# GAMES-UChile/mogptk

Measured on AMD Instinct MI355X. Metric: log-marginal-likelihood+grad evals/sec, MOSM C=4 N=8192; 1/2/4/8 GPU, higher is better.
Workload: dtype f64

## Files before the change

mogptk_amd/csrc/exact.hip:

```cpp
#include "mogp_model.h"
#include <cstdlib>
#include <limits>

using namespace mogp;

static int wait_stream(hipStream_t st) {
    static const bool spin = !(std::getenv("MOGP_SPIN_WAIT") && std::atoi(std::getenv("MOGP_SPIN_WAIT")) == 0);
    if (!spin) { HIP_TRY(hipStreamSynchronize(st)); return 0; }
    for (;;) {
        const hipError_t e = hipStreamQuery(st);
        if (e == hipSuccess) return 0;
        if (e != hipErrorNotReady) return hip_fail(e, "hipStreamQuery", __FILE__, __LINE__);
    }
}

static hipEvent_t prof_event(mogp_model* m, int idx) {
    if (!m->profiling) return nullptr;
    while ((int)m->ev.size() <= idx) { hipEvent_t e; if (hipEventCreate(&e) != hipSuccess) return nullptr; m->ev.push_back(e); }
    return m->ev[idx];
}

static void kinv_block_ranges(mogp_model* m) {
    std::vector<int> blk;
    tile_blocks(m->sx.off, m->C, blk);
    const int nblk = (int)blk.size() / 2, D = m->D;
    m->blk_cen.assign((size_t)D * nblk, 0.0); m->blk_half.assign((size_t)D * nblk, 0.0);
    for (int b = 0; b < nblk; ++b)
        for (int d = 0; d < D; ++d) {
            const double* x = m->sx.xs.data() + (size_t)d * m->sx.Mpad + blk[2 * b];
            double lo = x[0], hi = x[0];
            for (int i = 1; i < blk[2 * b + 1]; ++i) { lo = std::fmin(lo, x[i]); hi = std::fmax(hi, x[i]); }
            m->blk_cen[(size_t)d * nblk + b] = 0.5 * (lo + hi); m->blk_half[(size_t)d * nblk + b] = 0.5 * (hi - lo);
        }
}

static int kinv_plan(mogp_model* m, bool want) {
    static const bool full = std::getenv("MOGP_FULL_INVERSE") && std::atoi(std::getenv("MOGP_FULL_INVERSE")) != 0;
    m->kinv_sparse = false; m->kinv_fraction = 1.0;
    if (!want || full || m->sh_n > 1 || m->tiles.empty() || m->radial) return 0;
    const int nb = m->nb, D = m->D, T = m->T, W = m->Wt;
    const int64_t ld = m->Npad;
    if (m->blk_cen.empty()) kinv_block_ranges(m);
    const int nblk = (int)(m->blk_cen.size() / std::max(D, 1));
    std::vector<char> need((size_t)nb * nb, 0);
    for (const GTile& t : m->tiles) {
        const double* tab = m->table.data() + (size_t)t.pair * T * W;
        bool read = false;
        for (int k = 0; k < T && !read; ++k) {
            const double* row = tab + (size_t)k * W;
            double emin = 0.0;
            for (int d = 0; d < D; ++d) {
                const double sd = (m->blk_cen[(size_t)d * nblk + t.rb] - m->blk_cen[(size_t)d * nblk + t.cb]) + row[2 + 2 * D + d];
                const double mu = std::fmax(0.0, std::fabs(sd) - m->blk_half[(size_t)d * nblk + t.rb] - m->blk_half[(size_t)d * nblk + t.cb]);
                emin += row[2 + d] * mu * mu;
            }
            read = !(0.5 * emin > 52.0);
        }
        if (!read) continue;
        const int i0 = t.r0 / MOGP_TILE, i1 = (t.r0 + t.nr - 1) / MOGP_TILE, j0 = t.c0 / MOGP_TILE, j1 = (t.c0 + t.nc - 1) / MOGP_TILE;
        for (int i = i0; i <= i1; ++i) for (int j = j0; j <= j1; ++j) if (j <= i) need[(size_t)i * nb + j] = 1;
    }
    for (int i = 0; i < nb; ++i) need[(size_t)i * nb + i] = 1;
    std::vector<GemmTask> acc, lau;
    std::vector<int> prefix(nb + 1, 0);
    for (int i = 0; i < nb; ++i) {
        for (int j = 0; j <= i; ++j) {
            if (!need[(size_t)i * nb + j]) continue;
            GemmTask a;
            a.a_off = (int64_t)i * MOGP_TILE; a.b_off = (int64_t)j * MOGP_TILE; a.c_off = (int64_t)i * MOGP_TILE * ld + (int64_t)j * MOGP_TILE;
            a.kt = 4 * MOGP_TILE / 16; a.pad = i + 1;
            acc.push_back(a);
            GemmTask l;
            l.a_off = (int64_t)i * MOGP_TILE * ld + (int64_t)i * MOGP_TILE; l.b_off = (int64_t)i * MOGP_TILE * ld + (int64_t)j * MOGP_TILE;
            l.c_off = a.c_off; l.kt = (int)((ld - (int64_t)i * MOGP_TILE) / 16); l.pad = 0;
            lau.push_back(l);
        }
        prefix[i + 1] = (int)acc.size();
    }
    const double frac = (double)acc.size() / ((double)nb * (nb + 1) / 2);
    m->kinv_fraction = frac;
    if (frac > 0.85) return 0;
    const bool same = acc.size() == m->kinv_acc_tasks.size() && (acc.empty() || std::memcmp(acc.data(), m->kinv_acc_tasks.data(), acc.size() * sizeof(GemmTask)) == 0);
    if (!same || m->d_kinv_acc.n < acc.size()) {
        int rc;
        if ((rc = m->d_kinv_acc.ensure(std::max<size_t>(acc.size(), 1)))) return rc;
        if ((rc = m->d_kinv_lauum.ensure(std::max<size_t>(lau.size(), 1)))) return rc;
        HIP_TRY(hipMemcpyAsync(m->d_kinv_acc.p, acc.data(), acc.size() * sizeof(GemmTask), hipMemcpyHostToDevice, m->st));
        HIP_TRY(hipMemcpyAsync(m->d_kinv_lauum.p, lau.data(), lau.size() * sizeof(GemmTask), hipMemcpyHostToDevice, m->st));
        HIP_TRY(hipStreamSynchronize(m->st));
        m->kinv_acc_tasks.swap(acc); m->kinv_lauum_tasks.swap(lau);
    }
    m->kinv_prefix.swap(prefix);
    m->kinv_sparse = true;
    return 0;
}

static int pin_ensure(mogp_model* m, size_t n) {
    if (n <= m->h_pin_n) return 0;
    if (m->h_pin) { hipError_t e = hipHostFree(m->h_pin); (void)e; m->h_pin = nullptr; m->h_pin_n = 0; }
    HIP_TRY(hipHostMalloc(reinterpret_cast<void**>(&m->h_pin), n * sizeof(double), hipHostMallocDefault));
    m->h_pin_n = n;
    return 0;
}
struct PinLayout {
    size_t nzz, logdet = 0, zz, info, moments, diagG, pivots, total;
    PinLayout(int nb, int64_t Npad, int C, int T, int Wt) : nzz((size_t)((Npad + 3) / 4)) {
        zz = (size_t)nb; info = zz + nzz; moments = info + 1; diagG = moments + (size_t)(C * (C + 1) / 2) * T * Wt; pivots = diagG + C; total = pivots + 2;
    }
    explicit PinLayout(const mogp_model* m) : PinLayout(m->nb, m->Npad, m->C, m->T, m->Wt) {}
};

namespace mogp {
int begin_call(mogp_model* m, int64_t* info, bool one_gpu) {
    m->mean_w = nullptr;
    if (int rc = use_device(m->ctx)) return rc;
    if (info) *info = 0;
    if (one_gpu) one_gpu_call(m);
    return 0;
}

int exact_begin(mogp_model* m, const double* noise_var, const double* data_var, double jitter, GramArgs& ga, double& jabs) {
    const int C = m->C;
    const int64_t N = m->N, Npad = m->Npad;
    if (m->T <= 0) return fail(MOGP_EINVAL, "mogp_model_set_terms must be called before an evaluation");
    if (!noise_var) return fail(MOGP_EINVAL, "noise_var is null");
    { int r__ = ensure_system(m); if (r__) return r__; }
    m->have_W = m->have_Kinv = false;
    m->gemm_ev_used = 0; m->gemm_launches = 0; m->gemm_flops = 0.0;

    double dsum = 0.0;
    if (!m->point_diag.empty()) {
        for (int c = 0; c < C; ++c)
            for (int k = m->sx.off[c]; k < m->sx.off[c + 1]; ++k) dsum += m->point_diag[k] + noise_var[c];
    } else if (m->radial && m->point_kinds) {
        dsum = table_diag_points(m, m->sx);
        for (int c = 0; c < C; ++c) dsum += (double)(m->sx.off[c + 1] - m->sx.off[c]) * noise_var[c];
    } else
    for (int c = 0; c < C; ++c) dsum += (double)(m->sx.off[c + 1] - m->sx.off[c]) * (table_diag(m, c) + noise_var[c]);
    if (data_var) {
        std::vector<double> dv(Npad, 0.0);
        for (int64_t pos = 0; pos < N; ++pos) { dv[pos] = data_var[m->sx.perm[pos]]; dsum += dv[pos]; }
        { int r__ = m->d_dvar.ensure(Npad); if (r__) return r__; }
        HIP_TRY(hipMemcpyAsync(m->d_dvar.p, dv.data(), Npad * sizeof(double), hipMemcpyHostToDevice, m->st));
    }
    jabs = jitter * dsum / (double)N;
    HIP_TRY(hipMemcpyAsync(m->d_noise.p, noise_var, C * sizeof(double), hipMemcpyHostToDevice, m->st));
    static const unsigned long long big = std::numeric_limits<unsigned long long>::max();
    HIP_TRY(hipMemcpyAsync(m->d_info.p, &big, sizeof(big), hipMemcpyHostToDevice, m->st));
    int rc;
    if ((rc = mark(m, 0))) return rc;
    ga = GramArgs{};
    ga.tiles = m->d_tiles.p; ga.xr = m->d_x.p; ga.xc = m->d_x.p; ga.ldxr = ga.ldxc = Npad; ga.nrows = ga.ncols = N;
    if ((rc = m->ph_xx.prepare(m->sx.off, m->sx.off, C, m->T, Npad, Npad, m->st, ga.ph))) return rc;
    ga.table = m->d_table.p; ga.T = m->T; ga.D = m->D; ga.C = C; ga.W = m->Wt;
    ga.out = m->k.A.p; ga.ldo = Npad; ga.noise = m->d_noise.p; ga.dvar = data_var ? m->d_dvar.p : nullptr;
    ga.jitter_abs = jabs; ga.mirror = 0;
    if (m->radial) { ga.kind = m->d_kind.p; ga.shape = m->d_shape.p; }
    return 0;
}
}

namespace mogp { int chain_fallback(mogp_model* m) {
    if (m->flow_ran) {
        m->no_flow = true; m->flow_ran = false;
        m->flow_timeouts++;
        m->flow_retry_at = m->n_fact + m->flow_backoff;
        m->flow_backoff = std::min(m->flow_backoff * 4, 16384);
        for (hipStream_t q : {m->st, m->st2, m->st3, m->st4, m->ctx->st5, m->st_priv}) if (q) HIP_TRY(hipStreamSynchronize(q));
        static bool said_flow = false;
        if (!said_flow) {
            said_flow = true;
            unsigned code = 0;
            if (m->k.flow_flags.p && m->k.flow_cur && m->k.flow_cur->base_err > 0) { hipError_t e = hipMemcpy(&code, m->k.flow_flags.p + m->k.flow_cur->base_err, sizeof(code), hipMemcpyDeviceToHost); (void)e; }
            fprintf(stderr, "mogp: the dataflow kernel timed out (wait 0x%x; GPU shared with another process?); using the stream schedule for the next %d evaluations (said once)\n", code, (int)(m->flow_retry_at - m->n_fact));
            fprintf(stderr, "mogp: the host enqueued that evaluation in %.0f us (longest so far %.0f us)\n", m->flow_enqueue_us, m->flow_enqueue_us_max);
        }
        if (std::getenv("MOGP_FLOW_DEBUG")) { fprintf(stderr, "mogp: dataflow time-out %d of this model\n", m->flow_timeouts); flow_debug_dump(m); }
        return 0;
    }
    if (m->no_chain) return fail(MOGP_EHIP, "chain kernel: a hand-off timed out although the model is on the launch-per-step chain");
    m->no_chain = true;
    for (hipStream_t q : {m->st, m->st2, m->st3, m->st4, m->ctx->st5, m->st_priv}) if (q) HIP_TRY(hipStreamSynchronize(q));
    static bool said = false;
    if (!said) { said = true; fprintf(stderr, "mogp: the persistent chain kernel timed out (GPU shared with another process?); using the launch-per-step chain\n"); }
    return 0;
} }

template <typename F> static int retry_on_streams(mogp_model* m, int rc, F again) {
    if (rc != MOGP_RETRY_NO_CHAIN) return rc;
    if ((rc = chain_fallback(m))) return rc;
    return again();
}

namespace mogp { int report_not_pd(unsigned long long hinfo, int64_t* info) {
    if (info) *info = (int64_t)hinfo;
    return fail(MOGP_ENOTPD, "linalg.cholesky: The factorization could not be completed because the input is not "
                             "positive-definite (the leading minor of order " + std::to_string(hinfo) + " is not positive-definite).");
} }

static int factorize_finish(mogp_model* m, const GramArgs& ga, double* lml, int64_t* info) {
    const int64_t N = m->N, Npad = m->Npad;
    const PinLayout pl(m);
    const unsigned long long big = std::numeric_limits<unsigned long long>::max();
    unsigned long long hinfo = 0;
    std::memcpy(&hinfo, m->h_pin + pl.info, sizeof(hinfo));
    int rc;
    if (hinfo == MOGP_INFO_CHAIN_TIMEOUT) return MOGP_RETRY_NO_CHAIN;
    static const bool fake = std::getenv("MOGP_FAKE_K") && std::atoi(std::getenv("MOGP_FAKE_K")) > 1;
    if (hinfo != big && !fake) {
        if (info) *info = (int64_t)hinfo;
        int flag = 0;
        HIP_TRY(hipMemsetAsync(m->d_flag.p, 0, sizeof(int), m->st));
        if ((rc = launch_gram(ga, (int)m->tiles.size(), m->st))) return rc;
        if ((rc = launch_nonfinite_scan(m->k.A.p, Npad, N, m->d_flag.p, m->st))) return rc;
        HIP_TRY(hipMemcpyAsync(&flag, m->d_flag.p, sizeof(int), hipMemcpyDeviceToHost, m->st));
        HIP_TRY(hipStreamSynchronize(m->st));
        if (flag & 1) return fail(MOGP_ENONFINITE, "linalg.cholesky: kernel matrix has NaNs!");
        if (flag & 2) return fail(MOGP_ENONFINITE, "linalg.cholesky: kernel matrix has infinities!");
        return report_not_pd(hinfo, info);
    }
    m->pivot_min = m->h_pin[pl.pivots]; m->pivot_max = m->h_pin[pl.pivots + 1];
    double logdet = 0.0, zz = 0.0;
    for (int i = 0; i < m->nb; ++i) logdet += m->h_pin[pl.logdet + i];
    for (size_t i = 0; i < pl.nzz; ++i) zz += m->h_pin[pl.zz + i];
    if (lml) *lml = -0.5 * (double)N * std::log(2.0 * M_PI) - logdet - 0.5 * zz;
    m->have_W = !m->factor_only && !m->accurate_ran;
    return 0;
}

struct FactorPlan {
    enum Schedule { Fused, Phases, FactorOnly } schedule = Phases;
    bool defer = false;
    bool want_inverse = true;
    bool refine = false;
};

static int factorize(mogp_model* m, const double* noise_var, const double* data_var, double jitter, const FactorPlan& plan,
                     double* lml, double* jitter_abs, int64_t* info, GramArgs* ga_out = nullptr) {
    const bool fuse_inverse = plan.schedule == FactorPlan::Fused, factor_only = plan.schedule == FactorPlan::FactorOnly;
    const int64_t N = m->N, Npad = m->Npad;
    GramArgs ga{};
    double jabs = 0.0;
    int rc = exact_begin(m, noise_var, data_var, jitter, ga, jabs);
    if (rc) return rc;
    if (jitter_abs) *jitter_abs = jabs;
    m->n_fact++;
    if (m->no_flow && m->n_fact >= m->flow_retry_at) m->no_flow = false;
    m->factor_only = factor_only;
    ga.ev0 = prof_event(m, 7); ga.ev1 = prof_event(m, 8);
    m->strip.attach(ga);
    static const bool split_on = !(std::getenv("MOGP_GRAM_SPLIT") && std::atoi(std::getenv("MOGP_GRAM_SPLIT")) == 0);
    const bool split = split_on && fuse_inverse && flow_enabled(m, m->k) && !m->tiles_head.empty() && !m->tiles_tail.empty() && m->st2;
    if (split) {
        GramArgs gh = ga, gt = ga;
        gh.tiles = m->d_tiles_head.p; m->strip_head.attach(gh); gh.ev1 = nullptr;
        gt.tiles = m->d_tiles_tail.p; m->strip_tail.attach(gt); gt.ev0 = nullptr; gt.phases_ready = 1;
        if ((rc = launch_gram(gh, (int)m->tiles_head.size(), m->st))) return rc;
        if ((rc = launch_pad_identity(m->k.A.p, Npad, N, Npad, m->st))) return rc;
        if (!m->gram_ev) HIP_TRY(hipEventCreateWithFlags(&m->gram_ev, hipEventDisableTiming));
        HIP_TRY(hipEventRecord(m->gram_ev, m->st));
        HIP_TRY(hipStreamWaitEvent(m->st2, m->gram_ev, 0));
        if ((rc = launch_gram(gt, (int)m->tiles_tail.size(), m->st2))) return rc;
        if (!m->gram_tail_ev) HIP_TRY(hipEventCreateWithFlags(&m->gram_tail_ev, hipEventDisableTiming));
        HIP_TRY(hipEventRecord(m->gram_tail_ev, m->st2));
        m->k.tail_ready = m->gram_tail_ev;
    } else {
        if ((rc = launch_gram(ga, (int)m->tiles.size(), m->st))) return rc;
        if ((rc = launch_pad_identity(m->k.A.p, Npad, N, Npad, m->st))) return rc;
    }
    ga.ev0 = ga.ev1 = nullptr;
    if ((rc = mark(m, 1))) return rc;

    const PinLayout pl(m);
    if ((rc = pin_ensure(m, pl.total))) return rc;
    if ((rc = m->d_pivots.ensure(2))) return rc;
    if (m->accurate && (rc = m->acc_rhs.ensure((size_t)Npad * MOGP_TILE))) return rc;
    m->k.flow_used = false;
    m->flow_ran = false;
    m->k.want_vec = fuse_inverse;
    m->k.vec_y = m->d_y.p; m->k.vec_z = m->d_z.p; m->k.vec_zz = m->d_zz.p; m->k.vec_part = m->d_alpha.p + Npad;
    const bool accurate = m->accurate && plan.schedule == FactorPlan::Phases;
    m->accurate_ran = accurate;
    m->k.keep_L = m->k.refine_panels = plan.refine || accurate;
    if (factor_only && m->rhs_job && flow_enabled(m, m->k)) rc = spd_potri_flow(m, m->k, m->rhs_job);
    else rc = fuse_inverse ? spd_potri_fused(m, m->k) : spd_potrf(m, m->k);
    m->k.keep_L = m->k.refine_panels = false;
    m->k.want_vec = false; m->k.tail_ready = nullptr;
    if (rc) return rc;
    if ((rc = mark(m, 2))) return rc;
    if (accurate) {
        static const bool acc_aside = !(std::getenv("MOGP_ACC_ASIDE") && std::atoi(std::getenv("MOGP_ACC_ASIDE")) == 0);
        hipStream_t ms = (plan.want_inverse && m->st2u && acc_aside) ? m->st2u : m->st;
        if (plan.want_inverse) {
            if (ms != m->st) {
                while ((int)m->k.inv_ev.size() < 4) { hipEvent_t e; HIP_TRY(hipEventCreateWithFlags(&e, hipEventDisableTiming)); m->k.inv_ev.push_back(e); }
                HIP_TRY(hipEventRecord(m->k.inv_ev[0], m->st));
                HIP_TRY(hipStreamWaitEvent(ms, m->k.inv_ev[0], 0));
            }
            if ((rc = m->k.Wm.ensure((size_t)Npad * Npad))) return rc;
            HIP_TRY(hipMemsetAsync(m->k.Wm.p, 0, (size_t)Npad * Npad * sizeof(double), ms));
            if ((rc = launch_add_diag(m->k.Wm.p, Npad, Npad, 1.0, ms))) return rc;
            if ((rc = trsm_lower(m, m->k.A.p, Npad, m->nb, m->k.Wm.p, Npad, Npad, false, ms, true))) return rc;
            GemmArgs g{};
            g.A = m->k.Wm.p; g.lda = Npad; g.a_kmajor = 1; g.B = m->k.Wm.p; g.ldb = Npad; g.b_kmajor = 1;
            g.C = m->k.B.p; g.ldc = Npad; g.alpha = 1.0; g.beta = 0.0; g.mode = GM_LAUUM; g.mt = g.nt = m->nb; g.K = (int)Npad;
            if ((rc = gemm_call(m, g, gemm_flops(g, nullptr), ms))) return rc;
            if (ms != m->st) HIP_TRY(hipEventRecord(m->k.inv_ev[1], ms));
        }
        HIP_TRY(hipMemsetAsync(m->acc_rhs.p, 0, (size_t)Npad * MOGP_TILE * sizeof(double), m->st));
        if ((rc = launch_copy2d(m->acc_rhs.p, MOGP_TILE, m->d_y.p, 1, Npad, 1, 1.0, m->st))) return rc;
        if ((rc = trsm_lower(m, m->k.A.p, Npad, m->nb, m->acc_rhs.p, MOGP_TILE, MOGP_TILE, false))) return rc;
        if ((rc = launch_copy2d(m->d_z.p, 1, m->acc_rhs.p, MOGP_TILE, Npad, 1, 1.0, m->st))) return rc;
        HIP_TRY(hipMemsetAsync(m->d_zz.p, 0, pl.nzz * sizeof(double), m->st));
        if ((rc = launch_gemv_rows(m->d_z.p, Npad, 1, Npad, m->d_z.p, m->d_zz.p, m->st))) return rc;
        if ((rc = trsm_lower(m, m->k.A.p, Npad, m->nb, m->acc_rhs.p, MOGP_TILE, MOGP_TILE, true))) return rc;
        if ((rc = launch_copy2d(m->d_alpha.p, 1, m->acc_rhs.p, MOGP_TILE, Npad, 1, 1.0, m->st))) return rc;
        if (plan.want_inverse && ms != m->st) HIP_TRY(hipStreamWaitEvent(m->st, m->k.inv_ev[1], 0));
    } else if (plan.schedule == FactorPlan::Phases && (rc = spd_trtri(m, m->k))) return rc;
    if ((rc = mark(m, 3))) return rc;

    if (factor_only) {
        HIP_TRY(hipMemsetAsync(m->d_zz.p, 0, pl.nzz * sizeof(double), m->st));
    } else if (!accurate) {
        const double* Wp = fuse_inverse ? m->k.Wm.p : m->k.A.p;
        m->w_in_Wm = fuse_inverse;
        if (fuse_inverse && m->k.flow_used && m->k.vec_done) {
            if ((rc = launch_flow_alpha_sum(m->k, m->d_alpha.p, m->st))) return rc;
        } else {
            if ((rc = launch_trmv_lower(Wp, Npad, Npad, m->d_y.p, m->d_z.p, m->d_zz.p, m->st))) return rc;
            if ((rc = launch_trmv_lower_t(Wp, Npad, Npad, m->d_z.p, m->d_alpha.p, m->st))) return rc;
        }
    }
    if (fuse_inverse && (rc = spd_potri_fused_finish(m, m->k))) return rc;
    if ((rc = mark(m, 4))) return rc;
    {
        static const bool fault = std::getenv("MOGP_FLOW_FAULT") && std::atoi(std::getenv("MOGP_FLOW_FAULT")) != 0;
        static const unsigned long long timed_out = MOGP_INFO_CHAIN_TIMEOUT;
        if (fault && m->k.flow_used) HIP_TRY(hipMemcpyAsync(m->d_info.p, &timed_out, sizeof(timed_out), hipMemcpyHostToDevice, m->st));
    }

    const int nzz = (int)pl.nzz;
    if ((rc = launch_pivot_range(m->k.invd.p, N, m->d_pivots.p, m->st))) return rc;
    HIP_TRY(hipMemcpyAsync(m->h_pin + pl.pivots, m->d_pivots.p, 2 * sizeof(double), hipMemcpyDeviceToHost, m->st));
    HIP_TRY(hipMemcpyAsync(m->h_pin + pl.logdet, m->k.logdet.p, m->nb * sizeof(double), hipMemcpyDeviceToHost, m->st));
    static const int zz_piece = []() { const char* e = std::getenv("MOGP_D2H_CHUNK"); const int v = e ? std::atoi(e) : 2048; return v > 0 ? v : (1 << 30); }();
    for (int o = 0; o < nzz; o += zz_piece)
        HIP_TRY(hipMemcpyAsync(m->h_pin + pl.zz + o, m->d_zz.p + o, std::min(zz_piece, nzz - o) * sizeof(double), hipMemcpyDeviceToHost, m->st));
    HIP_TRY(hipMemcpyAsync(m->h_pin + pl.info, m->d_info.p, sizeof(unsigned long long), hipMemcpyDeviceToHost, m->st));
    if (ga_out) *ga_out = ga;
    if (plan.defer) return 0;
    HIP_TRY(hipStreamSynchronize(m->st));
    return factorize_finish(m, ga, lml, info);
}

namespace mogp { void collect_timing(mogp_model* m, int last_mark) {
    if (!m->profiling) return;
    auto el = [&](int a, int b) { float t = 0.f; if (hipEventElapsedTime(&t, m->ev[a], m->ev[b]) != hipSuccess) t = 0.f; return (double)t; };
    std::fill(m->ms, m->ms + MOGP_ST_COUNT, 0.0);
    m->ms[MOGP_ST_GRAM] = el(0, 1);
    m->ms[MOGP_ST_POTRF] = el(1, 2);
    m->ms[MOGP_ST_TRTRI] = el(2, 3);
    m->ms[MOGP_ST_SOLVE] = el(3, 4);
    if (last_mark >= 6) { m->ms[MOGP_ST_LAUUM] = el(4, 5); m->ms[MOGP_ST_MOMENTS] = el(5, 6); }
    m->ms[MOGP_ST_TOTAL] = el(0, last_mark);
    if ((int)m->ev.size() > 8) m->ms[MOGP_ST_GRAM_KERNEL] = el(7, 8);
    if (last_mark >= 6 && (int)m->ev.size() > 10) m->ms[MOGP_ST_MOMENT_KERNEL] = el(9, 10);
    double gsum = 0.0;
    for (size_t i = 0; i + 1 < m->gemm_ev_used; i += 2) {
        float t = 0.f;
        if (hipEventElapsedTime(&t, m->gemm_ev[i], m->gemm_ev[i + 1]) == hipSuccess) gsum += t;
    }
    m->ms[MOGP_ST_GEMM_KERNEL] = gsum;
}

int moment_pass_device(mogp_model* m, const double* kinv, double ksign) {
    const int C = m->C, D = m->D, W = m->Wt, T = m->T, P = C * (C + 1) / 2;
    const int64_t Npad = m->Npad;
    const int rm = m->sh_n > 1 ? m->sh_n : 0;
    const bool own = m->sh_n > 1 && m->own_n == m->sh_n && m->own_rank == m->sh_rank;
    int rc;
    MomentArgs ma{};
    ma.tiles = own ? m->d_tiles_own.p : m->d_tiles.p; ma.ntiles = (int)(own ? m->tiles_own.size() : m->tiles.size());
    ma.x = m->d_x.p; ma.ldx = Npad; ma.nrows = ma.ncols = m->N;
    if ((rc = m->ph_xx.prepare(m->sx.off, m->sx.off, C, T, Npad, Npad, m->st, ma.ph))) return rc;
    ma.table = m->d_table.p; ma.T = T; ma.D = D; ma.C = C; ma.W = W; ma.kinv = kinv; ma.kinv_sign = ksign; ma.ld = Npad; ma.alpha = m->d_alpha.p;
    ma.row_mod = rm; ma.row_rem = m->sh_rank;
    if (m->radial) { ma.kind = m->d_kind.p; ma.shape = m->d_shape.p; }
    ma.partial = m->d_partial.p;
    ma.phases_ready = 1;
    ma.ev0 = prof_event(m, 9); ma.ev1 = prof_event(m, 10);
    if ((rc = launch_moments(ma, m->st))) return rc;
    if ((rc = launch_moment_reduce(m->d_partial.p, own ? m->d_pair_start_own.p : m->d_pair_start.p, P, T, W, D, m->d_moments.p, m->st))) return rc;
    if ((rc = launch_diagG(kinv, Npad, m->d_alpha.p, m->d_chan_off.p, C, m->d_diagG.p, m->st, ksign, rm, m->sh_rank))) return rc;
    if ((rc = mean_grad_enqueue(m, m->d_alpha.p, -1.0))) return rc;
    return mark(m, 6);
}

int moment_pass(mogp_model* m, const double* kinv, double ksign, double* moments, double* diagG) {
    const int C = m->C, W = m->Wt, T = m->T, P = C * (C + 1) / 2;
    int rc;
    if ((rc = moment_pass_device(m, kinv, ksign))) return rc;
    HIP_TRY(hipMemcpyAsync(moments, m->d_moments.p, (size_t)P * T * W * sizeof(double), hipMemcpyDeviceToHost, m->st));
    HIP_TRY(hipMemcpyAsync(diagG, m->d_diagG.p, C * sizeof(double), hipMemcpyDeviceToHost, m->st));
    HIP_TRY(hipStreamSynchronize(m->st));
    return 0;
}

int test_side(mogp_model* m, int64_t S, const double* Xs, const double* kss_diag, int64_t extra_rows, hipStream_t st, TestSide& ts, GramArgs& ga) {
    const int C = m->C, D = m->D;
    const int64_t Npad = m->Npad;
    SortedX& ss = ts.ss;
    int rc;
    if ((rc = sort_inputs(Xs, S, D, C, MOGP_TILE, ss))) return rc;
    const int64_t Spad = ts.Spad = ss.Mpad, Srow = Spad + extra_rows;
    std::vector<GTile> pt;
    build_rect_tiles(ss.off, m->sx.off, C, pt);
    ts.ntiles = (int)pt.size();
    if ((rc = m->d_xs.ensure((size_t)D * Spad))) return rc;
    if ((rc = m->d_Ksf.ensure((size_t)Srow * Npad))) return rc;
    if ((rc = m->d_mu.ensure(Spad))) return rc;
    if ((rc = m->d_kdiag.ensure(Spad))) return rc;
    if ((rc = m->d_ptiles.ensure(std::max<size_t>(pt.size(), 1)))) return rc;
    std::vector<double> kd(Spad, 0.0);
    const bool per_point = m->Wt > 2 + 3 * D || (m->radial && m->point_kinds);
    for (int c = 0; c < C; ++c)
        for (int pos = ss.off[c]; pos < ss.off[c + 1]; ++pos) kd[pos] = per_point ? kss_diag[ss.perm[pos]] : kss_diag[c];
    HIP_TRY(hipMemcpyAsync(m->d_xs.p, ss.xs.data(), (size_t)D * Spad * sizeof(double), hipMemcpyHostToDevice, st));
    HIP_TRY(hipMemcpyAsync(m->d_kdiag.p, kd.data(), Spad * sizeof(double), hipMemcpyHostToDevice, st));
    HIP_TRY(hipMemcpyAsync(m->d_ptiles.p, pt.data(), pt.size() * sizeof(GTile), hipMemcpyHostToDevice, st));
    HIP_TRY(hipMemsetAsync(m->d_Ksf.p, 0, (size_t)Srow * Npad * sizeof(double), st));
    ga = GramArgs{};
    ga.tiles = m->d_ptiles.p; ga.xr = m->d_xs.p; ga.ldxr = Spad; ga.xc = m->d_x.p; ga.ldxc = Npad; ga.nrows = S; ga.ncols = m->N;
    if ((rc = m->ph_sx.prepare(ss.off, m->sx.off, C, m->T, Spad, Npad, st, ga.ph))) return rc;
    ga.table = m->d_table.p; ga.T = m->T; ga.D = D; ga.C = C; ga.W = m->Wt; ga.out = m->d_Ksf.p; ga.ldo = Npad;
    ga.noise = nullptr; ga.dvar = nullptr; ga.jitter_abs = 0.0; ga.mirror = 0;
    if (m->radial) { ga.kind = m->d_kind.p; ga.shape = m->d_shape.p; }
    return 0;
}
}

extern "C" {

int mogp_exact_eval(mogp_model* m, const double* noise_var, const double* data_var, double jitter, int flags,
                    double* lml, double* moments, double* diagG, double* trG, double* jitter_abs, int64_t* info) {
    if (!m) return fail(MOGP_EINVAL, "mogp_exact_eval: model is null");
    int rc;
    if ((rc = begin_call(m, info, true))) return rc;
    static const std::string grad_path = []() { const char* e = std::getenv("MOGP_GRAD_PATH"); return std::string(e ? e : ""); }();
    const bool sweep = grad_path == "sweep" && (flags & MOGP_EVAL_GRAD);
    const bool grad = (flags & MOGP_EVAL_GRAD) != 0;
    GramArgs ga{};
    if ((rc = ensure_system(m))) return rc;
    if ((rc = kinv_plan(m, grad && !sweep && !m->accurate))) return rc;
    const int fused_max = flow_enabled(m, m->k) ? 112 : 80;
    const bool fused = !sweep && grad && !m->accurate && (grad_path == "fused" || (grad_path != "phases" && m->nb <= fused_max));
    auto again = [&]() { return mogp_exact_eval(m, noise_var, data_var, jitter, flags, lml, moments, diagG, trG, jitter_abs, info); };
    FactorPlan plan;
    plan.schedule = fused ? FactorPlan::Fused : FactorPlan::Phases; plan.defer = grad; plan.want_inverse = grad;
    if (sweep) {
        m->pivot_min = m->pivot_max = 0.0;
        if ((rc = eval_sweep(m, noise_var, data_var, jitter, lml, jitter_abs, info))) return retry_on_streams(m, rc, again);
    }
    else if ((rc = factorize(m, noise_var, data_var, jitter, plan, lml, jitter_abs, info, &ga))) return retry_on_streams(m, rc, again);
    if (!grad) { collect_timing(m, 4); return MOGP_OK; }
    if (!moments || !diagG || !trG) return fail(MOGP_EINVAL, "mogp_exact_eval: gradient outputs are null");

    const int C = m->C, W = m->Wt, T = m->T, P = C * (C + 1) / 2;

    if (!sweep && !fused && !m->accurate_ran && (rc = spd_lauum(m, m->k))) return rc;
    const double* kinv = sweep ? m->k.A.p : m->k.B.p;
    const double ksign = sweep ? -1.0 : 1.0;
    if ((rc = mark(m, 5))) return rc;
    if (sweep) {
        if ((rc = moment_pass(m, kinv, ksign, moments, diagG))) return rc;
    } else {
        if ((rc = moment_pass_device(m, kinv, ksign))) return rc;
        const PinLayout pl(m);
        HIP_TRY(hipMemcpyAsync(m->h_pin + pl.moments, m->d_moments.p, (size_t)P * T * W * sizeof(double), hipMemcpyDeviceToHost, m->st));
        HIP_TRY(hipMemcpyAsync(m->h_pin + pl.diagG, m->d_diagG.p, C * sizeof(double), hipMemcpyDeviceToHost, m->st));
        if ((rc = wait_stream(m->st))) return rc;
        if ((rc = factorize_finish(m, ga, lml, info))) return retry_on_streams(m, rc, again);
        std::memcpy(moments, m->h_pin + pl.moments, (size_t)P * T * W * sizeof(double));
        std::memcpy(diagG, m->h_pin + pl.diagG, C * sizeof(double));
    }
    double tr = 0.0;
    for (int c = 0; c < C; ++c) tr += diagG[c];
    *trG = tr;
    m->have_Kinv = true;
    m->kinv_in_A = sweep;
    mean_grad_collect(m);
    collect_timing(m, 6);
    return MOGP_OK;
}

static int predict_core(mogp_model* m, const double* noise_var, const double* data_var, double jitter,
                        const double* kss_diag, int64_t S, const double* Xs, int full,
                        double* mu, double* var, int64_t* info, const double* mean_w) {
    int rc;
    if ((rc = begin_call(m, info, true))) return rc;
    const int C = m->C, nb = m->nb;
    const int64_t Npad = m->Npad;
    hipStream_t sv = m->st3 ? m->st3 : m->st;
    for (auto& e : m->pred_ev) if (!e) HIP_TRY(hipEventCreateWithFlags(&e, hipEventDisableTiming));
    HIP_TRY(hipEventRecord(m->pred_ev[0], m->st));
    HIP_TRY(hipStreamWaitEvent(sv, m->pred_ev[0], 0));
    TestSide ts; GramArgs ga{};
    if ((rc = test_side(m, S, Xs, kss_diag, MOGP_TILE, sv, ts, ga))) return rc;
    const SortedX& ss = ts.ss;
    const int64_t Spad = ts.Spad, Srow = Spad + MOGP_TILE;
    if ((rc = m->d_Vt.ensure((size_t)Srow * Npad))) return rc;
    if ((rc = m->d_var.ensure(Spad))) return rc;
    HIP_TRY(hipMemcpyAsync(m->d_Ksf.p + Spad * Npad, m->d_y.p, Npad * sizeof(double), hipMemcpyDeviceToDevice, sv));
    if ((rc = launch_gram(ga, ts.ntiles, sv))) return rc;
    if (mean_w) {
        std::vector<double> hw(Npad, 0.0);
        for (int64_t pos = 0; pos < m->N; ++pos) hw[pos] = mean_w[m->sx.perm[pos]];
        if ((rc = m->d_z.ensure(Npad))) return rc;
        HIP_TRY(dev_upload(m->d_z.p, hw.data(), Npad * sizeof(double)));
        if ((rc = launch_gemv_rows(m->d_Ksf.p, Npad, Spad, Npad, m->d_z.p, m->d_mu.p, sv))) return rc;
    }

    if ((rc = ensure_system(m))) return rc;
    const char* fpe = std::getenv("MOGP_FLOW_PREDICT");
    int fp_lo = 48, fp_hi = 160;
    if (fpe && std::strchr(fpe, ':')) { fp_lo = std::atoi(fpe); fp_hi = std::atoi(std::strchr(fpe, ':') + 1); }
    else if (fpe) fp_hi = std::atoi(fpe);
    const bool acc = m->accurate;
    const bool as_flow = !acc && fp_hi > 0 && nb >= fp_lo && nb <= fp_hi && Srow / MOGP_TILE <= 4096 && flow_enabled(m, m->k) && !m->kinv_sparse;
    FlowRhs job{m->d_Ksf.p, m->d_Vt.p, (int)(Srow / MOGP_TILE), nullptr};
    if (as_flow) {
        HIP_TRY(hipEventRecord(m->pred_ev[1], sv));
        job.ready = m->pred_ev[1];
        m->rhs_job = &job;
    }
    GramArgs gaK{};
    FactorPlan plan;
    plan.schedule = FactorPlan::FactorOnly; plan.defer = true; plan.refine = acc;
    rc = factorize(m, noise_var, data_var, jitter, plan, nullptr, nullptr, info, &gaK);
    m->rhs_job = nullptr;
    if (rc) return rc;
    const bool flowed = as_flow && m->k.flow_used;

    if (!flowed) {
        constexpr int OB = 4, KD = OB * MOGP_TILE;
        const int nouter = (nb + OB - 1) / OB, mt = (int)(Srow / MOGP_TILE);
        Spd& w = m->k;
        const bool streamed = g_outer == OB && (int)w.sync_ev.size() >= 2 * nouter;
        if (!streamed) {
            HIP_TRY(hipEventRecord(m->pred_ev[1], m->st));
            HIP_TRY(hipStreamWaitEvent(sv, m->pred_ev[1], 0));
        }
        if (w.Wd.n < (size_t)nouter * KD * KD) {
            if ((rc = w.Wd.ensure((size_t)nouter * KD * KD))) return rc;
            HIP_TRY(hipMemsetAsync(w.Wd.p, 0, (size_t)nouter * KD * KD * sizeof(double), sv));
        }
        for (int kb = 0; kb < nouter; ++kb) {
            const int k0 = kb * OB, nk = std::min(OB, nb - k0), k1 = k0 + nk, rem = nb - k1;
            const int64_t c0 = (int64_t)k0 * MOGP_TILE;
            if (streamed) HIP_TRY(hipStreamWaitEvent(sv, w.sync_ev[2 * kb], 0));
            double* Wk = w.Wd.p + (int64_t)kb * KD * KD;
            if ((rc = launch_wkk(w.A.p + c0 * (Npad + 1), Npad, w.invd.p + (int64_t)k0 * MOGP_TILE * MOGP_TILE, nk, Wk, KD, sv))) return rc;
            GemmArgs g{};
            g.A = m->d_Ksf.p + c0; g.lda = Npad; g.a_kmajor = 0; g.B = Wk; g.ldb = KD; g.b_kmajor = 0;
// ... 82 lines not shown
```

mogptk_amd/csrc/flow.hip:

```cpp
#include "mogp_model.h"
#include <unistd.h>
#include <chrono>
#include <set>

#include <cstdio>
#include <cstdlib>

namespace mogp {

typedef double d4_t __attribute__((ext_vector_type(4)));
typedef double d2_t __attribute__((ext_vector_type(2)));

#define FL_BK 16
#define FL_ROWK 18
#define FL_WTM 4
#define FL_WTN 2
#define FL_NWJ 4
#define FL_NWI 2
#define FL_NT 512
#define FL_COLK (MOGP_TILE + 16)
#define FL_OPER (MOGP_TILE * FL_ROWK)
#define FL_LDS_DOUBLES (2 * 2 * FL_OPER)
#define FL_LDS_BYTES (FL_LDS_DOUBLES * 8 + 16 + 3 * 64 * 4 + 16)
static_assert(MOGP_TILE * FL_ROWK == 16 * FL_COLK, "one LDS operand slot serves both layouts");
// ... 628 lines not shown
    }
    std::vector<const std::vector<FlowTask>*> order = {&q[Q_LOOK2], &q[Q_SEMI], &q[Q_INVCRIT], &vec};
    for (int d = 2; d < no + 3; ++d) {
        if (d < no && !into[d].empty()) order.push_back(&into[d]);
        if (d - 3 >= 0 && d - 3 < no && !trail[d - 3].empty()) order.push_back(&trail[d - 3]);
    }
    order.push_back(rhs_nt > 0 ? &rrest : &acc);
    for (size_t k = order.size(); k-- > 1;) if (order[k]->empty()) order.erase(order.begin() + (long)k);
    if ((int)order.size() > FLOW_MAXQ) {
        std::vector<FlowTask> rest;
        std::vector<const std::vector<FlowTask>*> tail(order.begin() + (FLOW_MAXQ - 2), order.end() - 1);
        for (auto* v : tail) rest.insert(rest.end(), v->begin(), v->end());
        std::stable_sort(rest.begin(), rest.end(), [](const FlowTask& x, const FlowTask& y) { return x.key < y.key; });
        p.folded = rest;
        order.erase(order.begin() + (FLOW_MAXQ - 2), order.end() - 1);
        order.insert(order.end() - 1, &p.folded);
    }
    p.nq = (int)order.size();
    for (int qi = 0; qi < p.nq; ++qi) {
        p.qbase[qi] = (int)p.tasks.size(); p.qsize[qi] = (int)order[qi]->size();
        p.tasks.insert(p.tasks.end(), order[qi]->begin(), order[qi]->end());
    }
    p.flops = 2.0 * MOGP_TILE * MOGP_TILE * FL_BK * tiles_k;
}

__global__ void k_alpha_sum(const double* __restrict__ part, int64_t npad, int no, int ob, double* __restrict__ out) {
    const int64_t col = (int64_t)blockIdx.x * blockDim.x + threadIdx.x;
    if (col >= npad) return;
    double s = 0.0;
    for (int r = (int)(col / MOGP_TILE) / ob; r < no; ++r) s += part[(int64_t)r * npad + col];
    out[col] = s;
}
int launch_flow_alpha_sum(const Spd& w, double* alpha, hipStream_t st) {
    const FlowPlan& p = w.flow_cur ? *w.flow_cur : w.flow;
    hipLaunchKernelGGL(k_alpha_sum, dim3((unsigned)((w.Npad + 255) / 256)), dim3(256), 0, st, w.vec_part, w.Npad, p.nouter, p.ob, alpha);
    HIP_TRY(hipGetLastError());
    return 0;
}

bool flow_enabled(const mogp_model* m, const Spd& w) {
    const char* eo = std::getenv("MOGP_FLOW");
    const char* en = std::getenv("MOGP_FLOW_MIN");
    const int on = eo ? std::atoi(eo) : 1, nmin = en ? std::atoi(en) : 8;
    if (!on || (m->no_flow && m->n_fact < m->flow_retry_at) || !chain_enabled(m) || !m->ctx->st_priv) return false;
    if (m->kinv_sparse && &w == &m->k) return false;
    return w.nb >= nmin && w.nb <= 0xfff0;
}

int spd_potri_flow(mogp_model* m, Spd& w, const FlowRhs* rhs) {
    const int nb = w.nb, ob = 4;
    const int64_t ld = w.Npad;
    int rc;
    const auto host_t0 = std::chrono::steady_clock::now();
    hipStream_t crit = m->st, priv = m->st_priv, bulk = m->st2;
    if (w.Wm.n < (size_t)ld * ld) {
        if ((rc = w.Wm.ensure((size_t)ld * ld))) return rc;
        HIP_TRY(hipMemsetAsync(w.Wm.p, 0, (size_t)ld * ld * sizeof(double), crit));
    }
    if ((rc = w.Lm.ensure((size_t)ld * ld))) return rc;
    if (!rhs && (rc = w.Wt.ensure((size_t)ld * ld))) return rc;
    const bool replay = m->replay_flow && !rhs && &w == &m->k;
    FlowPlan& plan = rhs ? w.flow_rhs : replay ? w.flow_replay : w.flow;
    DevBuf<FlowTask>& d_tasks = rhs ? w.flow_tasks_rhs : replay ? w.flow_tasks_replay : w.flow_tasks;
    DevBuf<int>& d_qmeta = rhs ? w.flow_qmeta_rhs : replay ? w.flow_qmeta_replay : w.flow_qmeta;
    const int rhs_nt = rhs ? rhs->nt : 0;
    if (plan.nb != nb || plan.ob != ob || plan.rhs_nt != rhs_nt) {
        flow_build(nb, ob, plan, rhs_nt, replay);
        if ((rc = d_tasks.ensure(plan.tasks.size()))) return rc;
        if ((rc = d_qmeta.ensure(2 * FLOW_MAXQ))) return rc;
        int qm[2 * FLOW_MAXQ] = {0};
        for (int q = 0; q < plan.nq; ++q) { qm[2 * q] = plan.qbase[q]; qm[2 * q + 1] = plan.qsize[q]; }
        HIP_TRY(hipStreamSynchronize(crit));
        HIP_TRY(dev_upload(d_tasks.p, plan.tasks.data(), plan.tasks.size() * sizeof(FlowTask)));
        HIP_TRY(dev_upload(d_qmeta.p, qm, sizeof(qm)));
    }
    if ((rc = w.flow_flags.ensure((size_t)plan.nflags))) return rc;
    if (!w.flow_diag.p) {
        if ((rc = w.flow_diag.ensure(FLOW_DIAG_WORDS))) return rc;
        HIP_TRY(hipMemsetAsync(w.flow_diag.p, 0, FLOW_DIAG_WORDS * sizeof(unsigned), crit));
    }
    w.flow_cur = &plan;
    const FlowPlan& p = plan;
    const int nouter = p.nouter;
    if ((rc = w.chain_flags.ensure((size_t)(nouter + 1) * MOGP_CHAIN_FLAGS))) return rc;
    HIP_TRY(hipMemsetAsync(w.chain_flags.p, 0, (size_t)(nouter + 1) * MOGP_CHAIN_FLAGS * sizeof(unsigned), crit));
    HIP_TRY(hipMemsetAsync(w.flow_flags.p, 0, (size_t)p.nflags * sizeof(unsigned), crit));
    if (replay) {
        std::vector<unsigned> preset((size_t)p.nflags, 0u);
        for (const FlowPlan::Chain& c : p.chain) preset[c.done_idx] = c.expect;
        HIP_TRY(hipMemcpyAsync(w.flow_flags.p, preset.data(), preset.size() * sizeof(unsigned), hipMemcpyHostToDevice, crit));
        HIP_TRY(hipStreamSynchronize(crit));
    }
    if (!rhs && w.want_vec && w.vec_zz) HIP_TRY(hipMemsetAsync(w.vec_zz, 0, (size_t)((ld + 3) / 4) * sizeof(double), crit));
    static const bool want_trace = std::getenv("MOGP_FLOW_TRACE") && std::atoi(std::getenv("MOGP_FLOW_TRACE")) != 0;
    if (want_trace) {
        if ((rc = w.flow_trace.ensure(FLOW_TRACE_W * p.tasks.size() + 4 * (size_t)nouter))) return rc;
        HIP_TRY(hipMemsetAsync(w.flow_trace.p, 0, w.flow_trace.n * sizeof(unsigned long long), crit));
    }
    while ((int)w.inv_ev.size() < 4) {
        hipEvent_t e;
        HIP_TRY(hipEventCreateWithFlags(&e, hipEventDisableTiming));
        w.inv_ev.push_back(e);
    }
    hipEvent_t start = w.inv_ev[0], e_flow = w.inv_ev[1], e_chain = w.inv_ev[2];
    HIP_TRY(hipEventRecord(start, crit));
    HIP_TRY(hipStreamWaitEvent(bulk, start, 0));
    HIP_TRY(hipStreamWaitEvent(priv, start, 0));

    static std::atomic<unsigned long long> attr_done{0ull};
    static std::atomic<unsigned long long> attr_done_dbg{0ull};
    { int r__ = set_max_dynamic_lds(reinterpret_cast<const void*>(k_flow<false>), FL_LDS_BYTES, attr_done); if (r__) return r__; }
    { int r__ = set_max_dynamic_lds(reinterpret_cast<const void*>(k_flow<true>), FL_LDS_BYTES, attr_done_dbg); if (r__) return r__; }
    static const int wg_per_cu = std::getenv("MOGP_FLOW_WGS") ? std::max(1, std::atoi(std::getenv("MOGP_FLOW_WGS"))) : 2;
    int cus = (m->ctx->ncu > 0 ? m->ctx->ncu : 256) - m->ctx->ncu_reserved;
    { static const int drop = std::getenv("MOGP_FLOW_DROP_CUS") ? std::atoi(std::getenv("MOGP_FLOW_DROP_CUS")) : 16;
      if (drop > 0 && drop < cus) cus -= drop; }
    FlowArgs g{};
    g.bA = w.A.p; g.bL = w.Lm.p; g.bWt = rhs ? rhs->T : w.Wt.p; g.bWm = w.Wm.p; g.bB = rhs ? rhs->X : w.B.p; g.ld = ld;
    g.tasks = d_tasks.p; g.qmeta = d_qmeta.p; g.flags = w.flow_flags.p;
    g.nq = p.nq; g.ncas = FLOW_NCAS; g.base_heads = p.base_heads; g.base_err = p.base_err; g.info = m->d_info.p;
    g.trace = want_trace ? w.flow_trace.p : nullptr;
    g.diag = w.flow_diag.p;
    static const bool want_post = std::getenv("MOGP_FLOW_DEBUG") && std::atoi(std::getenv("MOGP_FLOW_DEBUG")) != 0;
    if (want_post) {
        const size_t nwg = (size_t)wg_per_cu * ((size_t)cus + (size_t)m->ctx->ncu_reserved);
        if ((rc = w.flow_post.ensure(nwg * FLOW_POST_W))) return rc;
        HIP_TRY(hipMemsetAsync(w.flow_post.p, 0, w.flow_post.n * sizeof(unsigned), bulk));
        g.post = w.flow_post.p;
        if ((rc = w.flow_done.ensure(p.tasks.size()))) return rc;
        HIP_TRY(hipMemsetAsync(w.flow_done.p, 0, p.tasks.size(), bulk));
        g.done = w.flow_done.p;
    }
    g.npad = ld;
    { const char* e = std::getenv("MOGP_FLOW_REFILL"); g.refill = e ? std::atoi(e) : 0; }
    { const char* e = std::getenv("MOGP_FLOW_CLAIM1"); g.claim_one = e ? std::atoi(e) : 0; }
    { const char* e = std::getenv("MOGP_FLOW_NHI"); g.nhi = e ? std::atoi(e) : 0; }
    { const char* e = std::getenv("MOGP_FLOW_NAP"); g.nap_max = e ? (unsigned)std::max(0, std::atoi(e)) : 4u; }
    { const char* e = std::getenv("MOGP_FLOW_NAP_CALM"); g.nap_calm = e ? (unsigned)std::max(0, std::atoi(e)) : 0u; if (g.nap_calm < g.nap_max) g.nap_calm = g.nap_max; }
    w.vec_done = false;
    if (!rhs && w.want_vec && w.vec_y && w.vec_z && w.vec_zz && w.vec_part) {
        g.vy = w.vec_y; g.vz = w.vec_z; g.vzz = w.vec_zz; g.vpart = w.vec_part;
        w.vec_done = true;
    }
    hipEvent_t pe0 = nullptr, pe1 = nullptr;
    if (m->profiling) {
        if (m->gemm_ev_used + 2 > m->gemm_ev.size())
            for (int i = 0; i < 64; ++i) { hipEvent_t e; HIP_TRY(hipEventCreate(&e)); m->gemm_ev.push_back(e); }
        pe0 = m->gemm_ev[m->gemm_ev_used++]; pe1 = m->gemm_ev[m->gemm_ev_used++];
        HIP_TRY(hipEventRecord(pe0, bulk));
    }
    if (rhs && rhs->ready) HIP_TRY(hipStreamWaitEvent(bulk, rhs->ready, 0));
    const bool dbg_kernel = g.post != nullptr || g.trace != nullptr;
    static_assert(sizeof(FlowArgs) <= 512, "Spd::flow_args slots");
    if ((rc = w.flow_args.ensure(1024))) return rc;
    if (w.flow_args_h.size() != 2048) w.flow_args_h.assign(2048, (char)0xff);
    auto upload = [&](size_t slot, const FlowArgs& a, hipStream_t st) -> int {
        char* held = w.flow_args_h.data() + slot;
        char* fresh_ = w.flow_args_h.data() + 1024 + slot;
        std::memset(fresh_, 0, 512);
        std::memcpy(fresh_, &a, sizeof(a));
        if (std::memcmp(held, fresh_, 512) == 0) return 0;
        HIP_TRY(hipStreamSynchronize(st));
        HIP_TRY(dev_upload(w.flow_args.p + slot, fresh_, 512));
        std::memcpy(held, fresh_, 512);
        return 0;
    };
    if ((rc = upload(0, g, bulk))) return rc;
    const FlowArgs* d_g = reinterpret_cast<const FlowArgs*>(w.flow_args.p);
    FlowHot hot{};
    hot.bA = g.bA; hot.bL = g.bL; hot.bWt = g.bWt; hot.bWm = g.bWm; hot.bB = g.bB; hot.ld = g.ld; hot.tasks = g.tasks; hot.qmeta = g.qmeta; hot.flags = g.flags;
    hot.nq = g.nq; hot.ncas = g.ncas; hot.base_heads = g.base_heads; hot.base_err = g.base_err; hot.nap_max = g.nap_max; hot.nap_calm = g.nap_calm;
    if (dbg_kernel) hipLaunchKernelGGL(k_flow<true>, dim3(wg_per_cu * cus), dim3(FL_NT), FL_LDS_BYTES, bulk, d_g, hot);
    else hipLaunchKernelGGL(k_flow<false>, dim3(wg_per_cu * cus), dim3(FL_NT), FL_LDS_BYTES, bulk, d_g, hot);
    HIP_TRY(hipGetLastError());
    if (pe1) HIP_TRY(hipEventRecord(pe1, bulk));
    HIP_TRY(hipEventRecord(e_flow, bulk));
    m->gemm_launches += 1;
    m->gemm_flops += p.flops;

    unsigned* ferr = w.flow_flags.p + p.base_err;
    for (int kb = 0; kb < nouter && !replay; ++kb) {
        const int k0 = kb * ob, k1 = std::min(k0 + ob, nb), nk = k1 - k0, na = std::min(ob, nb - k1);
        const FlowPlan::Chain& pc = p.chain[kb];
        ChainFlow cf{};
        cf.done_flag = w.flow_flags.p + pc.done_idx; cf.write_through = 1;
        cf.trace = want_trace ? w.flow_trace.p + FLOW_TRACE_W * p.tasks.size() + 4 * (size_t)kb : nullptr;
        cf.diag = w.flow_diag.p;
        if ((rc = launch_chain(w.A.p, ld, k0, nk, w.invd.p, w.logdet.p, m->d_info.p, 0, w.Wm.p + (int64_t)k0 * MOGP_TILE * (ld + 1), ld,
                               w.chain_flags.p + (size_t)kb * MOGP_CHAIN_FLAGS, ferr, priv, &cf))) return rc;
        if (na <= 0) continue;
        GemmArgs t1{};
        t1.A = w.A.p + (int64_t)k1 * MOGP_TILE * ld + (int64_t)k0 * MOGP_TILE; t1.lda = ld; t1.a_kmajor = 0;
        t1.B = w.Wm.p + (int64_t)k0 * MOGP_TILE * (ld + 1); t1.ldb = ld; t1.b_kmajor = 0;
        t1.C = w.Lm.p + (int64_t)k1 * MOGP_TILE * ld + (int64_t)k0 * MOGP_TILE; t1.ldc = ld; t1.alpha = 1.0; t1.beta = 0.0;
        t1.mode = GM_KHI_J; t1.small = 1; t1.mt = 2 * na; t1.nt = nk; t1.K = nk * MOGP_TILE;
        t1.fl_flags = w.flow_flags.p; t1.fl_nwait = pc.t1_nwait;
        for (int k = 0; k < pc.t1_nwait; ++k) { t1.fl_widx[k] = pc.t1_widx[k]; t1.fl_wval[k] = pc.t1_wval[k]; }
        static const unsigned hook_spins = std::getenv("MOGP_FLOW_HOOK_SPINS") ? (unsigned)std::atoll(std::getenv("MOGP_FLOW_HOOK_SPINS")) : 0u;
        t1.fl_spins = hook_spins; t1.fl_diag = w.flow_diag.p;
        t1.fl_wt = 1; t1.fl_sig = 1; t1.fl_sig_base = pc.t1_sig_base; t1.fl_sig_shift = 1; t1.fl_err = ferr; t1.sk_info = m->d_info.p;
        if ((rc = launch_gemm(t1, priv))) return rc;
        if (kb == 0 && w.tail_ready) HIP_TRY(hipStreamWaitEvent(priv, w.tail_ready, 0));
        GemmArgs t2{};
        t2.A = t1.C; t2.lda = ld; t2.a_kmajor = 0; t2.B = t1.C; t2.ldb = ld; t2.b_kmajor = 0;
        t2.C = w.A.p + (int64_t)k1 * MOGP_TILE * (ld + 1); t2.ldc = ld; t2.alpha = -1.0; t2.beta = 1.0;
        t2.mode = GM_RECT_LOWER; t2.small = 2; t2.mt = 2 * na; t2.nt = 2 * na; t2.K = nk * MOGP_TILE;
        t2.fl_flags = w.flow_flags.p; t2.fl_nwait = pc.t2_wval ? 1 : 0; t2.fl_widx[0] = pc.t2_widx; t2.fl_wval[0] = pc.t2_wval;
        t2.fl_err = ferr; t2.sk_info = m->d_info.p; t2.fl_spins = hook_spins; t2.fl_diag = w.flow_diag.p;
        if ((rc = launch_gemm(t2, priv))) return rc;
        m->gemm_flops += gemm_flops(t1, nullptr) + gemm_flops(t2, nullptr);
    }
    static const bool tail_on = !(std::getenv("MOGP_FLOW_TAIL") && std::atoi(std::getenv("MOGP_FLOW_TAIL")) == 0);
    if (tail_on && m->ctx->ncu_reserved > 0 && !replay) {
        if (rhs && rhs->ready) HIP_TRY(hipStreamWaitEvent(priv, rhs->ready, 0));
        g.post_base = wg_per_cu * cus;
        if ((rc = upload(512, g, priv))) return rc;
        const FlowArgs* d_g2 = reinterpret_cast<const FlowArgs*>(w.flow_args.p + 512);
        if (dbg_kernel) hipLaunchKernelGGL(k_flow<true>, dim3(wg_per_cu * m->ctx->ncu_reserved), dim3(FL_NT), FL_LDS_BYTES, priv, d_g2, hot);
        else hipLaunchKernelGGL(k_flow<false>, dim3(wg_per_cu * m->ctx->ncu_reserved), dim3(FL_NT), FL_LDS_BYTES, priv, d_g2, hot);
        HIP_TRY(hipGetLastError());
    }
    HIP_TRY(hipEventRecord(e_chain, priv));
    HIP_TRY(hipStreamWaitEvent(crit, e_flow, 0));
    HIP_TRY(hipStreamWaitEvent(crit, e_chain, 0));
    w.fused_last_inv = nullptr; w.fused_last_wt = nullptr;
    w.flow_used = true;
    m->flow_ran = true;
    m->flow_enqueue_us = std::chrono::duration<double, std::micro>(std::chrono::steady_clock::now() - host_t0).count();
    m->flow_enqueue_us_max = std::max(m->flow_enqueue_us_max, m->flow_enqueue_us);
    { const char* e = std::getenv("MOGP_FLOW_DEBUG");
      if (e && std::atoi(e) == 2 && &w == &m->k) { usleep(60000); fprintf(stderr, "mogp: dataflow state 60 ms after the evaluation was enqueued\n"); flow_debug_dump(m); } }
    return 0;
}

}

namespace mogp { void flow_debug_dump(mogp_model* m) {
    if (!m->k.flow_flags.p || !m->k.flow_cur) return;
    const FlowPlan& p = *m->k.flow_cur;
    std::vector<unsigned> fl((size_t)p.nflags);
    hipError_t e = hipMemcpy(fl.data(), m->k.flow_flags.p, fl.size() * sizeof(unsigned), hipMemcpyDeviceToHost); (void)e;
    std::vector<unsigned long long> tr;
    if (m->k.flow_trace.p && m->k.flow_trace.n >= FLOW_TRACE_W * p.tasks.size()) {
        tr.resize(FLOW_TRACE_W * p.tasks.size());
        e = hipMemcpy(tr.data(), m->k.flow_trace.p, tr.size() * sizeof(unsigned long long), hipMemcpyDeviceToHost); (void)e;
    }
    fprintf(stderr, "  error word 0x%x\n", fl[p.base_err]);
    std::set<unsigned> holders;
    for (int q = 0; q < p.nq; ++q) {
        const unsigned h = fl[p.base_heads + q];
        const unsigned claimed = std::min<unsigned>(h, (unsigned)p.qsize[q]);
        unsigned done = 0, shown = 0;
        fprintf(stderr, "  queue %2d: head %u of %d", q, h, p.qsize[q]);
        for (unsigned hh = 0; hh < (unsigned)p.qsize[q]; ++hh) {
            const size_t ti = (size_t)p.qbase[q] + hh;
            const FlowTask& t = p.tasks[ti];
            const bool fin = !tr.empty() && tr[FLOW_TRACE_W * ti + 4] != 0;
            if (fin) { ++done; continue; }
            if (tr.empty() && hh + 4 < claimed) continue;
            if (hh > claimed || shown >= 6) continue;
            ++shown;
            fprintf(stderr, "\n      %s task %u key %u C(buf %d %d,%d) A(buf %d %d,%d) B(buf %d %d,%d) kt %d var %d:", hh < claimed ? "CLAIMED" : "head   ", hh, t.key,
                    t.cbuf, t.cr, t.cc, t.abuf, t.ar, t.ac, t.bbuf, t.br, t.bc, t.kt, t.var);
            for (int d = 0; d < t.ndep; ++d) fprintf(stderr, " flag[%u]=%u/%u", t.dep[d], fl[t.dep[d]], (unsigned)t.need[d]);
            if (!tr.empty()) {
                const unsigned long long w5 = tr[FLOW_TRACE_W * ti + 5];
                if (w5 >> 63) { fprintf(stderr, "  (HELD by wg %llu%s)", w5 & 0xffff, tr[FLOW_TRACE_W * ti + 1] ? ": STARTED, not finished" : ""); holders.insert((unsigned)(w5 & 0xffff)); }
                else fprintf(stderr, "  (taken by wg %llu: %s)", w5 & 0xffff, tr[FLOW_TRACE_W * ti + 1] ? "running" : "not started");
            }
        }
        if (!tr.empty()) fprintf(stderr, "\n      finished %u", done);
        fprintf(stderr, "\n");
    }
    if (!tr.empty() && !holders.empty()) {
        unsigned long long t0 = ~0ull, tmax = 0;
        for (size_t i = 0; i < p.tasks.size(); ++i) {
            const unsigned long long s1 = tr[FLOW_TRACE_W * i + 1];
            if (s1) { t0 = std::min(t0, s1); tmax = std::max(tmax, std::max(s1, tr[FLOW_TRACE_W * i + 4])); }
        }
        fprintf(stderr, "  last time stamp of the evaluation: %.1f us after its first task\n", (double)(tmax - t0) / 100.0);
        int shown = 0;
        for (unsigned wg : holders) {
            size_t last = (size_t)-1, held = 0;
            for (size_t i = 0; i < p.tasks.size(); ++i) {
                const unsigned long long w5 = tr[FLOW_TRACE_W * i + 5];
                if ((unsigned)(w5 & 0xffff) != wg) continue;
                if (w5 >> 63) { ++held; if (!tr[FLOW_TRACE_W * i + 1]) continue; }
                if (tr[FLOW_TRACE_W * i + 1] && (last == (size_t)-1 || tr[FLOW_TRACE_W * i + 1] > tr[FLOW_TRACE_W * last + 1])) last = i;
            }
            if (shown++ >= 24) break;
            if (last == (size_t)-1) { fprintf(stderr, "  holder wg %u: holds %zu, has started NO task\n", wg, held); continue; }
            const FlowTask& t = p.tasks[last];
            fprintf(stderr, "  holder wg %u (xcc %llu): holds %zu; its last task %zu var %d kt %d: looked %.1f taken %.1f k loop %.1f .. %.1f signalled %.1f us%s\n", wg,
                    (tr[FLOW_TRACE_W * last + 5] >> 16) & 0xff, held, last, t.var, t.kt,
                    (double)((long long)(tr[FLOW_TRACE_W * last + 0] - t0)) / 100.0, (double)((long long)(tr[FLOW_TRACE_W * last + 1] - t0)) / 100.0,
                    (double)((long long)(tr[FLOW_TRACE_W * last + 2] - t0)) / 100.0, (double)((long long)(tr[FLOW_TRACE_W * last + 3] - t0)) / 100.0,
                    tr[FLOW_TRACE_W * last + 4] ? (double)((long long)(tr[FLOW_TRACE_W * last + 4] - t0)) / 100.0 : -1.0, tr[FLOW_TRACE_W * last + 4] ? "" : "  <- NOT FINISHED");
        }
    }
    if (!tr.empty()) {
        unsigned long long t0 = ~0ull;
        for (size_t i = 0; i < p.tasks.size(); ++i) if (tr[FLOW_TRACE_W * i + 1] && tr[FLOW_TRACE_W * i + 1] < t0) t0 = tr[FLOW_TRACE_W * i + 1];
        std::map<long, std::pair<int, std::set<unsigned>>> win;
        for (size_t i = 0; i < p.tasks.size(); ++i) {
            const unsigned long long en = tr[FLOW_TRACE_W * i + 4];
            if (!en) continue;
            auto& w = win[(long)((en - t0) / 500000ull)];
            ++w.first; w.second.insert((unsigned)(tr[FLOW_TRACE_W * i + 5] & 0xffff));
        }
        for (auto& kv : win) fprintf(stderr, "  %4ld ms: %6d tasks done by %3zu workgroups\n", kv.first * 5, kv.second.first, kv.second.second.size());
    }
    if (m->k.flow_post.p) {
        std::vector<unsigned> po(m->k.flow_post.n);
        e = hipMemcpy(po.data(), m->k.flow_post.p, po.size() * sizeof(unsigned), hipMemcpyDeviceToHost); (void)e;
// ... 140 lines not shown
```

mogptk_amd/csrc/gram.hip:

```cpp
#include "mogp_internal.h"

#include <algorithm>
#include <vector>
#include <cstdlib>

#ifdef MOGP_GRAM_DEBUG
#define GRAM_DBG(a, bit) ((a).dbg & (bit))
#else
#define GRAM_DBG(a, bit) 0
#endif

namespace mogp {

typedef double d2_t __attribute__((ext_vector_type(2)));

__device__ __forceinline__ double frac_turn(double p) { return p - rint(p); }

#define GT_SKIP (-1)
#define GT_GENERAL 0
#define GT_SKIP_EXPONENT 50.0
#define GT_DEGREE(zmax) ((zmax) <= 1.19e-3 ? 4 : (zmax) <= 4.93e-3 ? 5 : (zmax) <= 0.0139 ? 6 : (zmax) <= 0.0308 ? 7 : (zmax) <= 0.0578 ? 8 : (zmax) <= 0.0968 ? 9 : \
                         (zmax) <= 0.149 ? 10 : (zmax) <= 0.2147 ? 11 : (zmax) <= 0.294 ? 12 : 14)
#define GT_DEGREE_CASES(X) X(4) X(5) X(6) X(7) X(8) X(9) X(10) X(11) X(12) X(14)

__device__ __forceinline__ double fast_exp(double x) {
    const double n = rint(x * 1.44269504088896338700e+00);
    double r = fma(-n, 6.93147180369123816490e-01, x);
    r = fma(-n, 1.90821492927058770002e-10, r);
    double p = 1.6059043836821613e-10;
    p = fma(p, r, 2.08767569878681e-09);
    p = fma(p, r, 2.505210838544172e-08);
    p = fma(p, r, 2.755731922398589e-07);
    p = fma(p, r, 2.7557319223985893e-06);
    p = fma(p, r, 2.48015873015873e-05);
    p = fma(p, r, 1.984126984126984e-04);
    p = fma(p, r, 1.388888888888889e-03);
    p = fma(p, r, 8.333333333333333e-03);
    p = fma(p, r, 4.1666666666666664e-02);
    p = fma(p, r, 1.6666666666666666e-01);
    p = fma(p, r, 0.5);
    p = fma(p, r, 1.0);
    p = fma(p, r, 1.0);
    return ldexp(p, (int)n);
}

template <int N>
__device__ __forceinline__ double exp_taylor(double z) {
    constexpr double c[15] = {1.0, 1.0, 0.5, 1.6666666666666666e-01, 4.1666666666666664e-02, 8.333333333333333e-03,
                              1.388888888888889e-03, 1.984126984126984e-04, 2.48015873015873e-05, 2.7557319223985893e-06,
                              2.755731922398589e-07, 2.505210838544172e-08, 2.08767569878681e-09, 1.6059043836821613e-10,
                              1.1470745597729725e-11};
    double p = c[N];
#pragma unroll
    for (int k = N - 1; k >= 0; --k) p = fma(p, z, c[k]);
    return p;
}

struct PhaseArgs {
    const double* x; int64_t ld; const int* off; const double* table; int T, D, C, W, role; double* cs; double* sn;
};
__global__ __launch_bounds__(256) void k_phase_table(PhaseArgs a) {
    const int64_t pt = (int64_t)blockIdx.x * 256 + threadIdx.x;
    if (pt >= a.off[a.C]) return;
    const int o = blockIdx.y, t = blockIdx.z, D = a.D, W = a.W;
    int c = 0;
    while (pt >= a.off[c + 1]) ++c;
    const int pair = a.role == 0 ? c * a.C + o : o * a.C + c;
    const double* row = a.table + ((size_t)pair * a.T + t) * W;
    double ph = a.role == 0 ? row[1] : 0.0;
    for (int d = 0; d < D; ++d) {
        const double m = row[2 + D + d], xv = a.x[(size_t)d * a.ld + pt];
        ph = a.role == 0 ? fma(m, xv + row[2 + 2 * D + d], ph) : fma(m, xv, ph);
    }
    double sn, cs;
    sincospi(2.0 * frac_turn(ph), &sn, &cs);
    const size_t idx = ((size_t)o * a.T + t) * a.ld + pt;
    a.cs[idx] = cs;
    a.sn[idx] = sn;
}

struct CentreArgs { const double* x; int64_t ld; const int* off; int C, D; double* cen; double* half; };
__global__ __launch_bounds__(64) void k_block_centres(CentreArgs a) {
    int b = blockIdx.x, c = 0;
    for (; c < a.C; ++c) {
        const int nb = (a.off[c + 1] - a.off[c] + MOGP_GT - 1) / MOGP_GT;
        if (b < nb) break;
        b -= nb;
    }
    if (c >= a.C) return;
    const int start = a.off[c] + b * MOGP_GT, n = min(MOGP_GT, a.off[c + 1] - start), lane = threadIdx.x;
    for (int d = 0; d < a.D; ++d) {
        const double v = a.x[(size_t)d * a.ld + start + (lane < n ? lane : 0)];
        double lo = v, hi = v;
#pragma unroll
        for (int off = 32; off > 0; off >>= 1) { lo = fmin(lo, __shfl_xor(lo, off, 64)); hi = fmax(hi, __shfl_xor(hi, off, 64)); }
        if (lane == 0) { a.cen[(size_t)d * a.ld + start] = 0.5 * (lo + hi); a.half[(size_t)d * a.ld + start] = 0.5 * (hi - lo); }
    }
}

size_t phase_ws_doubles(int C, int T, int64_t ldr, int64_t ldc) { return (size_t)2 * (C * T + MOGP_MAXD) * (size_t)(ldr + ldc); }

struct PhaseView {
    const double *rcs, *rsn, *ccs, *csn, *rcen, *rhalf, *ccen, *chalf;
};
__host__ __device__ static inline PhaseView phase_view(double* ws, int C, int T, int D, int64_t ldr, int64_t ldc) {
    PhaseView v;
    double* p = ws;
    v.rcs = p; p += (size_t)C * T * ldr; v.rsn = p; p += (size_t)C * T * ldr;
    v.ccs = p; p += (size_t)C * T * ldc; v.csn = p; p += (size_t)C * T * ldc;
    v.rcen = p; p += (size_t)D * ldr; v.rhalf = p; p += (size_t)D * ldr;
    v.ccen = p; p += (size_t)D * ldc; v.chalf = p;
    return v;
}

static int launch_phase_tables(const PhaseRef& ph, const double* xr, int64_t ldxr, int64_t nr, const double* xc, int64_t ldxc, int64_t nc,
                               const double* table, int T, int D, int C, int W, hipStream_t s) {
    if (!ph.ws || !ph.offr || !ph.offc) { set_error("Gram / moment launch without a phase workspace"); return -1; }
    const PhaseView v = phase_view(ph.ws, C, T, D, ldxr, ldxc);
    PhaseArgs a;
    a.table = table; a.T = T; a.D = D; a.C = C; a.W = W;
    a.x = xr; a.ld = ldxr; a.off = ph.offr; a.role = 0; a.cs = const_cast<double*>(v.rcs); a.sn = const_cast<double*>(v.rsn);
    if (nr > 0) hipLaunchKernelGGL(k_phase_table, dim3((unsigned)((nr + 255) / 256), C, T), dim3(256), 0, s, a);
    a.x = xc; a.ld = ldxc; a.off = ph.offc; a.role = 1; a.cs = const_cast<double*>(v.ccs); a.sn = const_cast<double*>(v.csn);
    if (nc > 0) hipLaunchKernelGGL(k_phase_table, dim3((unsigned)((nc + 255) / 256), C, T), dim3(256), 0, s, a);
    CentreArgs c;
    c.C = C; c.D = D;
    c.x = xr; c.ld = ldxr; c.off = ph.offr; c.cen = const_cast<double*>(v.rcen); c.half = const_cast<double*>(v.rhalf);
    if (nr > 0) hipLaunchKernelGGL(k_block_centres, dim3((unsigned)((nr + MOGP_GT - 1) / MOGP_GT + C)), dim3(64), 0, s, c);
    c.x = xc; c.ld = ldxc; c.off = ph.offc; c.cen = const_cast<double*>(v.ccen); c.half = const_cast<double*>(v.chalf);
    if (nc > 0) hipLaunchKernelGGL(k_block_centres, dim3((unsigned)((nc + MOGP_GT - 1) / MOGP_GT + C)), dim3(64), 0, s, c);
    HIP_TRY(hipGetLastError());
    return 0;
}

template <int DM>
struct TileLds {
    double cu[MOGP_TC][MOGP_GT], su[MOGP_TC][MOGP_GT], cw[MOGP_TC][MOGP_GT], sw[MOGP_TC][MOGP_GT];
    double V[MOGP_TC][DM], s[MOGP_TC][DM], M[MOGP_TC][DM], A[MOGP_TC];
    double Kp[MOGP_TC][DM];
    double L[MOGP_TC][DM], e[MOGP_TC][DM];
    int deg[MOGP_TC];
};
template <int DM>
struct TileCtx { double cr[DM], cc[DM], hr[DM], hc[DM]; };

template <int DM>
__device__ __forceinline__ void tile_centres(TileCtx<DM>& X, const GTile& tl, int D, const PhaseView& v, int64_t ldxr, int64_t ldxc) {
    for (int d = 0; d < D; ++d) {
        X.cr[d] = v.rcen[(size_t)d * ldxr + tl.r0]; X.hr[d] = v.rhalf[(size_t)d * ldxr + tl.r0];
        X.cc[d] = v.ccen[(size_t)d * ldxc + tl.c0]; X.hc[d] = v.chalf[(size_t)d * ldxc + tl.c0];
    }
}

template <int DM>
__device__ __forceinline__ void tile_context(TileCtx<DM>& X, double (&p)[4][DM], double (&q)[4][DM], const GTile& tl, int D,
                                             const PhaseView& v, const double* __restrict__ xr, int64_t ldxr,
                                             const double* __restrict__ xc, int64_t ldxc, int rg, int cg) {
    tile_centres<DM>(X, tl, D, v, ldxr, ldxc);
#pragma unroll
    for (int m = 0; m < 4; ++m)
        for (int d = 0; d < D; ++d) {
            p[m][d] = xr[(size_t)d * ldxr + tl.r0 + min(rg * 4 + m, tl.nr - 1)] - X.cr[d];
            q[m][d] = xc[(size_t)d * ldxc + tl.c0 + min(cg * 4 + m, tl.nc - 1)] - X.cc[d];
        }
}

constexpr int STAGE_ITEMS = MOGP_TC * MOGP_GT * 2 / 256;
template <int DM>
struct StageItem { double x[DM], cs, sn; };

template <int DM>
__device__ __forceinline__ void stage_item_load(StageItem<DM>& I, int which, int t, int pnt, const GTile& tl, int D, int C, int T, int t0,
                                                const PhaseView& v, const double* __restrict__ xr, int64_t ldxr,
                                                const double* __restrict__ xc, int64_t ldxc) {
    const int i = tl.pair / C, j = tl.pair - i * C;
    if (which == 0) {
        const int64_t g = tl.r0 + min(pnt, tl.nr - 1);
        const size_t k = ((size_t)j * T + t0 + t) * ldxr + g;
        I.cs = v.rcs[k]; I.sn = v.rsn[k];
        for (int d = 0; d < D; ++d) I.x[d] = xr[(size_t)d * ldxr + g];
    } else {
        const int64_t g = tl.c0 + min(pnt, tl.nc - 1);
        const size_t k = ((size_t)i * T + t0 + t) * ldxc + g;
        I.cs = v.ccs[k]; I.sn = v.csn[k];
        for (int d = 0; d < D; ++d) I.x[d] = xc[(size_t)d * ldxc + g];
    }
}

template <int DM, bool AMP, bool RAD = false>
__device__ __forceinline__ void stage_item_compute(TileLds<DM>& L, const StageItem<DM>& I, const TileCtx<DM>& X, const double* tab, int W,
                                                   int which, int t, int pnt, int D, int t0, const int* kinds = nullptr) {
    const double* row = tab + (size_t)(t0 + t) * W;
    const double A = row[0];
    if constexpr (RAD) {
        const int kd = kinds[t0 + t] & MOGP_KIND_MASK;
        const bool per = kd == MOGP_KIND_PERIODIC, dot = kd == MOGP_KIND_DOT;
        const int deg = (AMP && A == 0.0 && !dot) ? GT_SKIP : GT_GENERAL;
        if (pnt == 0 && which == 0) {
            L.deg[t] = deg; L.A[t] = A;
            for (int d = 0; d < D; ++d) {
                L.V[t][d] = row[2 + d]; L.M[t][d] = row[2 + D + d];
                L.s[t][d] = (X.cr[d] - X.cc[d]) + row[2 + 2 * D + d];
                L.Kp[t][d] = X.cr[d]; L.L[t][d] = X.cc[d];
            }
            L.e[t][0] = row[1];
        }
        if (deg == GT_SKIP) return;
        if (dot) return;
        const double f = (AMP && !per) ? A : 1.0;
        if (which == 0) { L.cu[t][pnt] = f * I.cs; L.su[t][pnt] = f * I.sn; }
        else { L.cw[t][pnt] = I.cs; L.sw[t][pnt] = I.sn; }
        return;
    }
    const bool env = W > 2 + 3 * D;
    double zmax = 0.0, es = 0.0, emin = 0.0, efac = 0.0, s[DM], V[DM], Lv[DM], er[DM], ec[DM];
// ... 1381 lines not shown
            c += fabs(s) >= fabs(x) ? (s - t) + x : (x - t) + s;
            s = t;
        }
        __syncthreads();
        red[part][pnt] = s; redc[part][pnt] = c;
        __syncthreads();
        if (part == 0 && pnt < n) {
            double hs = 0.0, hc = 0.0;
#pragma unroll
            for (int q = 0; q < 4; ++q) {
                const double x = red[q][pnt];
                const double t = hs + x;
                hc += fabs(hs) >= fabs(x) ? (hs - t) + x : (x - t) + hs;
                hs = t;
                hc += redc[q][pnt];
            }
            out[(size_t)d * ld + first + pnt] += hs + hc;
        }
    }
}

template <bool DENSE, bool ZG, bool ENV>
static int launch_moments_t(const MomentArgs& a, hipStream_t s) {
    switch (a.D) {
        case 1: hipLaunchKernelGGL((k_moments<1, DENSE, ZG, ENV>), dim3(a.ntiles), dim3(256), 0, s, a); break;
        case 2: hipLaunchKernelGGL((k_moments<2, DENSE, ZG, ENV>), dim3(a.ntiles), dim3(256), 0, s, a); break;
        case 3: hipLaunchKernelGGL((k_moments<3, DENSE, ZG, ENV>), dim3(a.ntiles), dim3(256), 0, s, a); break;
        default: hipLaunchKernelGGL((k_moments<0, DENSE, ZG, ENV>), dim3(a.ntiles), dim3(256), 0, s, a); break;
    }
    HIP_TRY(hipGetLastError());
    return 0;
}

int launch_moments(const MomentArgs& a0, hipStream_t s) {
    if (a0.ntiles <= 0) return 0;
    MomentArgs a = a0;
    if (a.W <= 0) a.W = 2 + 3 * a.D;
    const bool env = a.W > 2 + 3 * a.D;
    const double* xc = a.xc ? a.xc : a.x;
    const int64_t ldxc = a.xc ? a.ldxc : a.ldx;
    int rc = a.phases_ready ? 0 : launch_phase_tables(a.ph, a.x, a.ldx, a.nrows, xc, ldxc, a.xc ? a.ncols : a.nrows, a.table, a.T, a.D, a.C, a.W, s);
    if (rc) return rc;
    if (a.kind) {
        if (!a.shape) { set_error("launch_moments: kinds without shapes"); return -1; }
        if (a.G != nullptr || env) { set_error("launch_moments: radial profiles run in exact mode without an envelope only"); return -1; }
        if (a.ev0) HIP_TRY(hipEventRecord(a.ev0, s));
        switch (a.D) {
            case 1: hipLaunchKernelGGL((k_moments<1, false, false, false, true>), dim3(a.ntiles), dim3(256), 0, s, a); break;
            case 2: hipLaunchKernelGGL((k_moments<2, false, false, false, true>), dim3(a.ntiles), dim3(256), 0, s, a); break;
            case 3: hipLaunchKernelGGL((k_moments<3, false, false, false, true>), dim3(a.ntiles), dim3(256), 0, s, a); break;
            default: hipLaunchKernelGGL((k_moments<0, false, false, false, true>), dim3(a.ntiles), dim3(256), 0, s, a); break;
        }
        HIP_TRY(hipGetLastError());
        if (a.ev1) HIP_TRY(hipEventRecord(a.ev1, s));
        return 0;
    }
    if (a.G == nullptr) {
        if (a.ev0) HIP_TRY(hipEventRecord(a.ev0, s));
        static const bool mx_on = !(std::getenv("MOGP_MOM_X") && std::atoi(std::getenv("MOGP_MOM_X")) == 0);
        if (mx_on && !env && a.D == 1 && a.W == 5 && a.T <= 4 && a.row_mod <= 1 && a.xc == nullptr) {
            static const int ncu = []() { int dev = 0; hipDeviceProp_t pr; if (hipGetDevice(&dev) != hipSuccess || hipGetDeviceProperties(&pr, dev) != hipSuccess) return 256; return pr.multiProcessorCount; }();
            if (a.T <= 3) hipLaunchKernelGGL(k_moments_x<3>, dim3(std::min(a.ntiles, ncu)), dim3(512), 0, s, a);
            else hipLaunchKernelGGL(k_moments_x<4>, dim3(std::min(a.ntiles, ncu)), dim3(512), 0, s, a);
            HIP_TRY(hipGetLastError());
            rc = 0;
        } else
        rc = env ? launch_moments_t<false, false, true>(a, s) : launch_moments_t<false, false, false>(a, s);
        if (!rc && a.ev1) HIP_TRY(hipEventRecord(a.ev1, s));
        return rc;
    }
    if (a.gzr || a.gzc) {
        if (!a.gzp || !a.rblk || !a.cblk || a.nrb <= 0 || a.ncb <= 0) { set_error("launch_moments: the input-gradient pass needs its scratch and block tables"); return -1; }
        const size_t half = (size_t)a.nrb * a.ncb * a.D * MOGP_GT;
        HIP_TRY(hipMemsetAsync(a.gzp, 0, 2 * half * sizeof(double), s));
        if ((rc = env ? launch_moments_t<true, true, true>(a, s) : launch_moments_t<true, true, false>(a, s))) return rc;
        if (a.gzr) hipLaunchKernelGGL(k_gz_reduce, dim3(a.nrb), dim3(256), 0, s, a.gzp, a.ncb, a.D, a.rblk, a.gzr, a.ldgz);
        if (a.gzc) hipLaunchKernelGGL(k_gz_reduce, dim3(a.ncb), dim3(256), 0, s, a.gzp + half, a.nrb, a.D, a.cblk, a.gzc, a.ldgz);
        HIP_TRY(hipGetLastError());
        return 0;
    }
    return env ? launch_moments_t<true, false, true>(a, s) : launch_moments_t<true, false, false>(a, s);
}

__global__ __launch_bounds__(256) void k_moment_reduce(const double* __restrict__ partial, const int* __restrict__ pair_start,
                                                       int TW, int W, int D, int lower_pairs, double* __restrict__ out) {
    const int p = blockIdx.x, tw = blockIdx.y;
    const int b = pair_start[p], e = pair_start[p + 1];
    __shared__ double red[256];
    double s = 0.0;
    for (int t = b + threadIdx.x; t < e; t += 256) s += partial[(size_t)t * TW + tw];
    red[threadIdx.x] = s;
    __syncthreads();
    for (int off = 128; off > 0; off >>= 1) {
        if (threadIdx.x < off) red[threadIdx.x] += red[threadIdx.x + off];
        __syncthreads();
    }
    if (threadIdx.x == 0) {
        int i = (int)((sqrt(8.0 * (double)p + 1.0) - 1.0) * 0.5);
        while ((i + 1) * (i + 2) / 2 <= p) ++i;
        while (i * (i + 1) / 2 > p) --i;
        const bool diag = lower_pairs && (p - i * (i + 1) / 2) == i;
        const int w = tw % W;
        double v = red[0];
        if (diag && (w == 1 || (w >= 2 + D && w < 2 + 2 * D))) v = 0.0;
        out[(size_t)p * TW + tw] = v;
    }
}

int launch_moment_reduce(const double* partial, const int* pair_start, int npairs, int T, int W, int D, double* out, hipStream_t s, int lower_pairs) {
    hipLaunchKernelGGL(k_moment_reduce, dim3(npairs, T * W), dim3(256), 0, s, partial, pair_start, T * W, W, D, lower_pairs, out);
    HIP_TRY(hipGetLastError());
    return 0;
}

__global__ void k_diagG(const double* __restrict__ kinv, int64_t ld, const double* __restrict__ alpha,
                        const int* __restrict__ chan_off, double* __restrict__ out, double kinv_sign, int row_mod, int row_rem) {
    const int c = blockIdx.x;
    __shared__ double red[256];
    double s = 0.0;
    for (int64_t k = chan_off[c] + threadIdx.x; k < chan_off[c + 1]; k += 256)
        if (row_mod <= 1 || (int)((k / MOGP_TILE) % row_mod) == row_rem) s += 0.5 * (alpha[k] * alpha[k] - kinv_sign * kinv[k * ld + k]);
    red[threadIdx.x] = s;
    __syncthreads();
    for (int off = 128; off > 0; off >>= 1) {
        if (threadIdx.x < off) red[threadIdx.x] += red[threadIdx.x + off];
        __syncthreads();
    }
    if (threadIdx.x == 0) out[c] = red[0];
}

int launch_diagG(const double* kinv, int64_t ld, const double* alpha, const int* chan_off, int C, double* out, hipStream_t s,
                 double kinv_sign, int row_mod, int row_rem) {
    hipLaunchKernelGGL(k_diagG, dim3(C), dim3(256), 0, s, kinv, ld, alpha, chan_off, out, kinv_sign, row_mod, row_rem);
    HIP_TRY(hipGetLastError());
    return 0;
}

}
```

mogptk_amd/csrc/mogp_api.hip:

```cpp
#include "mogp_model.h"

#include <algorithm>
#include <cmath>
#include <cstring>
#include <cstdlib>

namespace mogp {

static thread_local std::string g_err;
void set_error(const std::string& msg) { g_err = msg; }
int hip_fail(hipError_t e, const char* what, const char* file, int line) {
    g_err = std::string("HIP error '") + hipGetErrorString(e) + "' in " + what + " (" + file + ":" + std::to_string(line) + ")";
    return MOGP_EHIP;
}
int launch_potrf_trtri_tile(double* A, int64_t ld, int t, double* invd, double* logdet, unsigned long long* info, hipStream_t s,
                            long long info_base = 0, int store_L = 0);

int fail(int code, const std::string& msg) { g_err = msg; return code; }

int sort_inputs(const double* X, int64_t M, int D, int C, int64_t pad_to, SortedX& o) {
    o.M = M;
    o.Mpad = round_up(std::max<int64_t>(M, 1), pad_to);
    o.perm.resize(M);
    o.off.assign(C + 1, 0);
// ... 558 lines not shown
        build_sym_tiles(m->sx.off, m->C, m->tiles, m->pair_start);
        if ((rc = m->d_tiles.ensure(m->tiles.size()))) return rc;
        if ((rc = m->d_pair_start.ensure(m->pair_start.size()))) return rc;
        HIP_TRY(dev_upload(m->d_tiles.p, m->tiles.data(), m->tiles.size() * sizeof(GTile)));
        if ((rc = m->strip.build(m->tiles))) return rc;
        for (const GTile& t : m->tiles) (t.c0 < 4 * MOGP_TILE ? m->tiles_head : m->tiles_tail).push_back(t);
        if (!m->tiles_head.empty() && !m->tiles_tail.empty()) {
            if ((rc = m->d_tiles_head.ensure(m->tiles_head.size()))) return rc;
            if ((rc = m->d_tiles_tail.ensure(m->tiles_tail.size()))) return rc;
            HIP_TRY(dev_upload(m->d_tiles_head.p, m->tiles_head.data(), m->tiles_head.size() * sizeof(GTile)));
            HIP_TRY(dev_upload(m->d_tiles_tail.p, m->tiles_tail.data(), m->tiles_tail.size() * sizeof(GTile)));
            if ((rc = m->strip_head.build(m->tiles_head))) return rc;
            if ((rc = m->strip_tail.build(m->tiles_tail))) return rc;
        }
        HIP_TRY(dev_upload(m->d_pair_start.p, m->pair_start.data(), m->pair_start.size() * sizeof(int)));
    }
    if ((rc = m->d_partial.ensure(m->tiles.size() * (size_t)std::max(m->T, 1) * (size_t)std::max(m->Wt, 1)))) return rc;
    if (m->k.Npad == m->Npad) return (m->k.owned_rows && !m->sh_owned) ? spd_make_whole(m->k) : 0;
    return spd_alloc(m->k, m->Npad, m->sh_owned ? m->ctx->device : -1);
} }

extern "C" {

static int ctx_streams(mogp_ctx* ctx) {
    if (ctx->streams_ready) return 0;
    int lo_prio = 0;
    {
        int lo = 0, hi = 0;
        HIP_TRY(hipDeviceGetStreamPriorityRange(&lo, &hi));
        lo_prio = lo;
        HIP_TRY(hipStreamCreateWithPriority(&ctx->st, hipStreamNonBlocking, hi));
        const char* er = std::getenv("MOGP_RESERVE_CUS");
        const int reserve = er ? std::atoi(er) : 2;
        hipDeviceProp_t prop;
        HIP_TRY(hipGetDeviceProperties(&prop, ctx->device));
        const int ncu = prop.multiProcessorCount;
        const bool masked = reserve > 0 && 16 * reserve < ncu;
        ctx->ncu = ncu; ctx->ncu_reserved = masked ? 8 * reserve : 0;
        ctx->chain_ok = !masked || 8 * reserve >= 13;
        if (masked) {
            std::vector<uint32_t> bulk((ncu + 31) / 32, 0u), priv((ncu + 31) / 32, 0u);
            for (int i = 0; i < ncu; ++i) (i < 8 * reserve ? priv : bulk)[i / 32] |= 1u << (i % 32);
            HIP_TRY(hipExtStreamCreateWithCUMask(&ctx->st_priv, (uint32_t)priv.size(), priv.data()));
            HIP_TRY(hipExtStreamCreateWithCUMask(&ctx->st2, (uint32_t)bulk.size(), bulk.data()));
            HIP_TRY(hipExtStreamCreateWithCUMask(&ctx->st3, (uint32_t)bulk.size(), bulk.data()));
            HIP_TRY(hipExtStreamCreateWithCUMask(&ctx->st4, (uint32_t)bulk.size(), bulk.data()));
        } else {
            HIP_TRY(hipStreamCreateWithPriority(&ctx->st2, hipStreamNonBlocking, (lo + hi) / 2));
            HIP_TRY(hipStreamCreateWithPriority(&ctx->st3, hipStreamNonBlocking, lo));
            HIP_TRY(hipStreamCreateWithPriority(&ctx->st4, hipStreamNonBlocking, lo));
        }
    }
    {
        hipDeviceProp_t prop;
        HIP_TRY(hipGetDeviceProperties(&prop, ctx->device));
        std::vector<uint32_t> all((prop.multiProcessorCount + 31) / 32, 0u);
        for (int i = 0; i < prop.multiProcessorCount; ++i) all[i / 32] |= 1u << (i % 32);
        if (ctx->st_priv) HIP_TRY(hipExtStreamCreateWithCUMask(&ctx->st2u, (uint32_t)all.size(), all.data()));
        else HIP_TRY(hipStreamCreateWithPriority(&ctx->st2u, hipStreamNonBlocking, lo_prio));
    }
    ctx->streams_ready = true;
    return 0;
}

int mogp_model_create(mogp_ctx* ctx, int64_t N, int D, int C, const double* X, const double* y, mogp_model** out) {
    if (!ctx || !X || !y || !out) return fail(MOGP_EINVAL, "mogp_model_create: null argument");
    *out = nullptr;
    if (N <= 0 || D <= 0 || D > MOGP_MAXD || C <= 0) return fail(MOGP_EINVAL, "mogp_model_create: need N > 0, 0 < D <= 8, C > 0");
    int rc;
    if ((rc = use_device(ctx))) return rc;
    mogp_model* m = new mogp_model();
    m->ctx = ctx; m->N = N; m->D = D; m->C = C;
    if ((rc = sort_inputs(X, N, D, C, MOGP_TILE, m->sx))) { delete m; return rc; }
    m->Npad = m->sx.Mpad;
    m->nb = (int)(m->Npad / MOGP_TILE);
    const int64_t Npad = m->Npad;
    const int nchunks = (int)((Npad + 511) / 512);
#define TRY_RC(x) do { int r__ = (x); if (r__) { mogp_model_destroy(m); return r__; } } while (0)
#define TRY_HIP(x) do { hipError_t e__ = (x); if (e__ != hipSuccess) { int r__ = hip_fail(e__, #x, __FILE__, __LINE__); mogp_model_destroy(m); return r__; } } while (0)
    TRY_RC(ctx_streams(ctx));
    m->st = ctx->st; m->st2 = ctx->st2; m->st2u = ctx->st2u; m->st3 = ctx->st3; m->st4 = ctx->st4; m->st_priv = ctx->st_priv;
    TRY_RC(m->d_x.ensure((size_t)D * Npad));
    TRY_RC(m->d_y.ensure(Npad));
    TRY_RC(m->d_noise.ensure(C));
    TRY_RC(m->d_z.ensure(Npad));
    TRY_RC(m->d_alpha.ensure((size_t)(1 + nchunks) * Npad));
    TRY_RC(m->d_zz.ensure((Npad + 3) / 4));
    TRY_RC(m->d_diagG.ensure(C));
    TRY_RC(m->d_info.ensure(2));
    TRY_RC(m->d_flag.ensure(1));
    TRY_RC(m->d_chan_off.ensure(C + 1));
    TRY_HIP(dev_upload(m->d_x.p, m->sx.xs.data(), (size_t)D * Npad * sizeof(double)));
    TRY_HIP(dev_upload(m->d_chan_off.p, m->sx.off.data(), (C + 1) * sizeof(int)));
    TRY_RC(mogp_model_set_y(m, y));
#undef TRY_RC
#undef TRY_HIP
    *out = m;
    return MOGP_OK;
}

int mogp_model_destroy(mogp_model* m) {
    if (!m) return MOGP_OK;
    if (m->ctx) { hipError_t e = hipSetDevice(m->ctx->device); (void)e; }
    if (m->st) { hipError_t e = hipStreamSynchronize(m->st); (void)e; }
    for (auto e : m->ev) { hipError_t r = hipEventDestroy(e); (void)r; }
    for (auto e : m->gemm_ev) { hipError_t r = hipEventDestroy(e); (void)r; }
    for (auto& e : m->pred_ev) if (e) { hipError_t r = hipEventDestroy(e); (void)r; e = nullptr; }
    for (hipStream_t q : {m->st2, m->st2u, m->st3, m->st4, m->ctx->st5, m->st_priv}) if (q) { hipError_t e = hipStreamSynchronize(q); (void)e; }
    m->k.release(); m->ws.release(); m->ws_tail.release();
    for (int b = 0; b < 2; ++b) { m->swU[b].release(); m->swUr[b].release(); m->swXr[b].release(); }
    for (auto e : m->sw_ev) { hipError_t r = hipEventDestroy(e); (void)r; }
    for (auto e : m->sh_prof) { hipError_t r = hipEventDestroy(e); (void)r; }
    m->d_symv.release(); m->sh_send.release(); m->sh_recv.release(); m->sh_send1.release(); m->sh_recv1.release(); m->sh_fact.release();
    for (auto e : m->sh_ev) { hipError_t r = hipEventDestroy(e); (void)r; }
    if (m->tw) { m->tw->release(); delete m->tw; m->tw = nullptr; }
    m->oa.release();
    m->d_x.release(); m->d_y.release(); m->d_table.release(); m->d_kind.release(); m->d_shape.release();
    m->d_noise.release(); m->d_dvar.release(); m->d_z.release(); m->d_alpha.release(); m->d_zz.release();
    m->d_partial.release(); m->d_moments.release(); m->d_diagG.release(); m->d_tiles.release(); m->d_pair_start.release(); m->strip.release(); m->strip_own.release();
    m->d_tiles_head.release(); m->d_tiles_tail.release(); m->strip_head.release(); m->strip_tail.release();
    if (m->gram_ev) { hipError_t r = hipEventDestroy(m->gram_ev); (void)r; m->gram_ev = nullptr; }
    if (m->gram_tail_ev) { hipError_t r = hipEventDestroy(m->gram_tail_ev); (void)r; m->gram_tail_ev = nullptr; }
    m->d_chan_off.release(); m->d_flag.release(); m->d_info.release(); m->d_pivots.release(); m->acc_rhs.release();
    m->d_xs.release(); m->d_Ksf.release(); m->d_Vt.release(); m->d_mu.release(); m->d_var.release(); m->d_kdiag.release();
    m->d_Kss.release(); m->d_ptiles.release(); m->d_pred_tasks.release();
    m->ph_xx.release(); m->ph_sx.release(); m->ph_ss.release();
    if (m->h_pin) { hipError_t e = hipHostFree(m->h_pin); (void)e; m->h_pin = nullptr; }
    mean_release(m);

    delete m;
    return MOGP_OK;
}

int mogp_model_set_y(mogp_model* m, const double* y) {
    if (!m || !y) return fail(MOGP_EINVAL, "mogp_model_set_y: null argument");
    int rc;
    if ((rc = use_device(m->ctx))) return rc;
    std::vector<double> ys(m->Npad, 0.0);
    for (int64_t pos = 0; pos < m->N; ++pos) ys[pos] = y[m->sx.perm[pos]];
    if (m->mean_on) {
        HIP_TRY(dev_upload(m->d_y0.p, ys.data(), m->Npad * sizeof(double)));
        m->hy0 = ys;
        m->mean_g_valid = m->mean_g_pending = false;
        return mean_apply(m);
    }
    HIP_TRY(dev_upload(m->d_y.p, ys.data(), m->Npad * sizeof(double)));
    m->hy = ys;
    return MOGP_OK;
}

int mogp_model_set_terms_ex(mogp_model* m, int T, int width, const double* table) {
    if (!m || !table || T <= 0) return fail(MOGP_EINVAL, "mogp_model_set_terms: bad argument");
    if (width != 2 + 3 * m->D && width != 2 + 5 * m->D) return fail(MOGP_EINVAL, "mogp_model_set_terms: the row width must be 2 + 3 D or 2 + 5 D");
    int rc;
    if ((rc = use_device(m->ctx))) return rc;
    const int W = width;
    const size_t n = (size_t)m->C * m->C * T * W;
    for (size_t i = 0; i < n; ++i)
        if (!std::isfinite(table[i])) return fail(MOGP_ENONFINITE, "spectral term table has non-finite entries (kernel parameters diverged)");
    if (T != m->T) m->radial = m->point_kinds = false;
    m->T = T;
    m->Wt = W;
    if (m->tw) m->tw->pred_valid = false;
    m->table.assign(table, table + n);
    if ((rc = m->d_table.ensure(n))) return rc;
    if ((rc = m->d_moments.ensure((size_t)(m->C * (m->C + 1) / 2) * T * W))) return rc;
    HIP_TRY(hipMemcpyAsync(m->d_table.p, m->table.data(), n * sizeof(double), hipMemcpyHostToDevice, m->st));
    return MOGP_OK;
}

int mogp_model_set_terms(mogp_model* m, int T, const double* table) {
    if (!m) return fail(MOGP_EINVAL, "mogp_model_set_terms: bad argument");
    return mogp_model_set_terms_ex(m, T, 2 + 3 * m->D, table);
}

int mogp_model_set_kinds(mogp_model* m, int T, const int* kind, const double* shape) {
    if (!m) return fail(MOGP_EINVAL, "mogp_model_set_kinds: model is null");
    if (T != m->T || T <= 0) return fail(MOGP_EINVAL, "mogp_model_set_kinds: T must be that of the last mogp_model_set_terms");
    const size_t n = (size_t)m->C * m->C * T;
    bool any = false;
    if (const char* bad = check_kinds(kind, shape, m->C, m->D, T, &any)) return fail(MOGP_EINVAL, std::string("mogp_model_set_kinds: ") + bad);
    m->radial = false; m->point_kinds = false;
    if (!any) return MOGP_OK;
    if (m->Wt != 2 + 3 * m->D) return fail(MOGP_EINVAL, "mogp_model_set_kinds: radial profiles do not combine with enveloped term rows");
    m->hkind.assign(kind, kind + n);
    m->hshape.assign(shape, shape + n);
    for (size_t i = 0; i < n; ++i) m->point_kinds |= (kind[i] & MOGP_KIND_MASK) == MOGP_KIND_DOT;
    int rc;
    if ((rc = use_device(m->ctx))) return rc;
    if ((rc = m->d_kind.ensure(n))) return rc;
    if ((rc = m->d_shape.ensure(n))) return rc;
    HIP_TRY(hipMemcpyAsync(m->d_kind.p, kind, n * sizeof(int), hipMemcpyHostToDevice, m->st));
    HIP_TRY(hipMemcpyAsync(m->d_shape.p, shape, n * sizeof(double), hipMemcpyHostToDevice, m->st));
    m->radial = true;
    return MOGP_OK;
}

int mogp_model_set_point_diag(mogp_model* m, const double* kdiag) {
    if (!m) return fail(MOGP_EINVAL, "mogp_model_set_point_diag: model is null");
    m->point_diag.clear();
    if (kdiag) {
        m->point_diag.resize(m->N);
        for (int64_t pos = 0; pos < m->N; ++pos) m->point_diag[pos] = kdiag[m->sx.perm[pos]];
    }
    return MOGP_OK;
}

int mogp_gram(mogp_ctx* ctx, int C, int D, int T, const double* table, int64_t M1, const double* X1,
              int64_t M2, const double* X2, double* K_out) {
    return mogp_gram_ex(ctx, C, D, T, 2 + 3 * D, table, M1, X1, M2, X2, K_out);
}

int mogp_gram_ex(mogp_ctx* ctx, int C, int D, int T, int width, const double* table, int64_t M1, const double* X1,
                 int64_t M2, const double* X2, double* K_out) {
    return mogp_gram_kinds(ctx, C, D, T, width, table, nullptr, nullptr, M1, X1, M2, X2, K_out);
}

int mogp_gram_kinds(mogp_ctx* ctx, int C, int D, int T, int width, const double* table, const int* kind, const double* shape,
                    int64_t M1, const double* X1, int64_t M2, const double* X2, double* K_out) {
    if (!ctx || !table || !X1 || !K_out || M1 <= 0 || T <= 0 || C <= 0 || D <= 0 || D > MOGP_MAXD || (width != 2 + 3 * D && width != 2 + 5 * D))
        return fail(MOGP_EINVAL, "mogp_gram: bad argument");
    bool radial = false;
    if (const char* bad = check_kinds(kind, shape, C, D, T, &radial)) return fail(MOGP_EINVAL, std::string("mogp_gram_kinds: ") + bad);
    if (radial && width != 2 + 3 * D) return fail(MOGP_EINVAL, "mogp_gram_kinds: kinds need shapes and rows of width 2 + 3 D");
    int rc;
    if ((rc = use_device(ctx))) return rc;
    const bool sym = (X2 == nullptr);
    SortedX s1, s2;
    if ((rc = sort_inputs(X1, M1, D, C, 1, s1))) return rc;
    if (!sym && (rc = sort_inputs(X2, M2, D, C, 1, s2))) return rc;
    const SortedX& sc = sym ? s1 : s2;
    const int64_t R = s1.M, Cc = sc.M;
    std::vector<GTile> tiles;
    std::vector<int> ps;
    if (sym) build_sym_tiles(s1.off, C, tiles, ps); else build_rect_tiles(s1.off, s2.off, C, tiles);
    const int W = width;
    DevBuf<double> dx1, dx2, dtab, dout;
    DevBuf<GTile> dt;
    DevBuf<int> dkind;
    DevBuf<double> dshape;
    PhaseWs ph;
    auto cleanup = [&]() { dx1.release(); dx2.release(); dtab.release(); dout.release(); dt.release(); dkind.release(); dshape.release(); ph.release(); };
#define G_TRY(x) do { int r__ = (x); if (r__) { cleanup(); return r__; } } while (0)
#define G_HIP(x) do { hipError_t e__ = (x); if (e__ != hipSuccess) { cleanup(); return hip_fail(e__, #x, __FILE__, __LINE__); } } while (0)
    G_TRY(dx1.ensure((size_t)D * s1.Mpad));
    G_TRY(dtab.ensure((size_t)C * C * T * W));
    G_TRY(dout.ensure((size_t)R * Cc));
    G_TRY(dt.ensure(std::max<size_t>(tiles.size(), 1)));
    G_HIP(dev_upload(dx1.p, s1.xs.data(), (size_t)D * s1.Mpad * sizeof(double)));
// ... 180 lines not shown
```

mogptk_amd/csrc/mogp_internal.h:

```cpp
#pragma once
#include <hip/hip_runtime.h>
#include <stdint.h>
#include <atomic>
#include <string>
#include <vector>

#define MOGP_TILE 128
#define MOGP_GT 64
#define MOGP_TC 8
#define MOGP_MAXD 8

#define MOGP_KIND_GAUSS 0
#define MOGP_KIND_RQ 1
#define MOGP_KIND_MATERN12 2
#define MOGP_KIND_MATERN32 3
#define MOGP_KIND_MATERN52 4
#ifndef MOGP_KIND_PERIODIC
#define MOGP_KIND_PERIODIC 5
#endif
#ifndef MOGP_KIND_SINC
#define MOGP_KIND_SINC 6
#define MOGP_KIND_DOT 7
#define MOGP_DOT_DEGREE_MAX 8
#endif
#ifndef MOGP_KIND_TIMES
#define MOGP_KIND_TIMES (1 << 8)
#endif
#define MOGP_KIND_MASK 0xff
#define MOGP_GROUP_MAX 4

namespace mogp {
const char* check_kinds(const int* kind, const double* shape, int C, int D, int T, bool* any);
}

namespace mogp {

void set_error(const std::string& msg);
int hip_fail(hipError_t e, const char* what, const char* file, int line);
#define HIP_TRY(x)                                                        \
    do {                                                                  \
        hipError_t e__ = (x);                                             \
        if (e__ != hipSuccess) return mogp::hip_fail(e__, #x, __FILE__, __LINE__); \
    } while (0)

inline int set_max_dynamic_lds(const void* fn, int bytes, std::atomic<unsigned long long>& done) {
    int dev = 0;
    HIP_TRY(hipGetDevice(&dev));
    const unsigned long long bit = 1ull << (dev & 63);
    if (done.load(std::memory_order_acquire) & bit) return 0;
    HIP_TRY(hipFuncSetAttribute(fn, hipFuncAttributeMaxDynamicSharedMemorySize, bytes));
    done.fetch_or(bit, std::memory_order_release);
    return 0;
}

struct GTile {
    int r0, c0;
    int nr, nc;
    int pair;
    int flags;
    int rb, cb;
};
struct GSeg { int r0, c0, n, pair; int diag, pad[3]; };
enum { GT_MIRROR = 1,
       GT_DIAG = 2 };

struct PhaseRef {
    const int* offr = nullptr;
    const int* offc = nullptr;
    double* ws = nullptr;
};
size_t phase_ws_doubles(int C, int T, int64_t ldr, int64_t ldc);

struct GramArgs {
    const GTile* tiles;
    const double* xr;
    const double* xc;
    int64_t ldxr, ldxc;
    int64_t nrows, ncols;
    PhaseRef ph;
    const double* table;
    int T, D, C;
    int W;
    double* out;
    int64_t ldo;
    double* out2;
    const double* noise;
    const double* dvar;
    double jitter_abs;
    int mirror;
    hipEvent_t ev0, ev1;
    const GSeg* segs; int nsegs;
    const GTile* rest; int nrest;
    int dbg;
    int tab_lds;
    int phases_ready;
    const int* kind;
    const double* shape;
};

struct MomentArgs {
    const GTile* tiles;
    int ntiles;
    const double* x;
    int64_t ldx;
    const double* xc;
    int64_t ldxc;
    int64_t nrows, ncols;
    PhaseRef ph;
    const double* table;
    int T, D, C;
    int W;
    const double* kinv;
    int64_t ld;
    const double* alpha;
    double kinv_sign;
    int row_mod, row_rem;
    const double* G;
    int64_t ldg;
    const double* ru;
    const double* rw;
    double rcoef;
    int sym;
    double* gzr;
    double* gzc;
    int64_t ldgz;
    double* gzp;
    int nrb, ncb;
    const int* rblk;
    const int* cblk;
    double* partial;
    hipEvent_t ev0, ev1;
    int tab_lds;
    int phases_ready;
    const int* kind;
    const double* shape;
};

int launch_gram(const GramArgs& a, int ntiles, hipStream_t s);
void split_strip_tiles(const std::vector<GTile>& tiles, int maxrun, std::vector<GSeg>& segs, std::vector<GTile>& rest);
int launch_moments(const MomentArgs& a, hipStream_t s);
inline size_t gz_scratch_doubles(int nrb, int ncb, int D) { return (size_t)2 * nrb * ncb * D * MOGP_GT; }
void tile_blocks(const std::vector<int>& off, int C, std::vector<int>& blk);
int launch_moment_reduce(const double* partial, const int* pair_start, int npairs, int T, int W, int D, double* out, hipStream_t s,
                         int lower_pairs = 1);
int launch_diagG(const double* kinv, int64_t ld, const double* alpha, const int* chan_off, int C, double* out, hipStream_t s,
                 double kinv_sign = 1.0, int row_mod = 0, int row_rem = 0);

enum GemmMode { GM_RECT = 0,
                GM_LOWER = 1,
                GM_LAUUM = 2,
                GM_KHI_J = 3,
                GM_TASKS = 4,
                GM_RECT_LOWER = 5,
                GM_KHI_I = 6,
                GM_KLO_J = 7,
                GM_KLO_I = 8 };

struct GemmTask {
    int64_t a_off, b_off, c_off;
    int kt;
    int pad;
};

struct GemmArgs {
    const double* A; int64_t lda; int a_kmajor;
    const double* B; int64_t ldb; int b_kmajor;
    double* C; int64_t ldc;
    double alpha, beta;
    int mode, mt, nt, K;
    const GemmTask* tasks; int ntasks;
    int task_chunked;
    int small;
    int beta0_from;
    int ksplit; int64_t c_split;
    int ksplit_xcd;
    int col_major;
    int row_mod, row_rem, row_off, row_shift;
    int sk_hint;
    int sk_spans;
    double* sk_ws;
    unsigned* sk_flags;
    unsigned sk_epoch;
    unsigned long long* sk_info;
    unsigned* fl_flags; int fl_nwait; unsigned fl_widx[4]; unsigned fl_wval[4];
    int fl_wt, fl_sig; unsigned fl_sig_base; int fl_sig_shift; unsigned* fl_err; unsigned fl_spins; unsigned* fl_diag;
};
int launch_gemm(const GemmArgs& a, hipStream_t s);
double gemm_flops(const GemmArgs& a, const std::vector<GemmTask>* host_tasks);

int launch_potrf_tile(double* A, int64_t ld, int t, double* logdet, unsigned long long* info, hipStream_t s);
int launch_trtri_tiles(const double* A, int64_t ld, int t0, int nt, double* invd, hipStream_t s);
int launch_put_diag_tiles(double* A, int64_t ld, int nt, const double* invd, hipStream_t s);
int launch_wkk(const double* Ablk, int64_t ld, const double* invd, int nk, double* Wk, int64_t ldw, hipStream_t s);
#define MOGP_CHAIN_FLAGS 32
#define MOGP_INFO_CHAIN_TIMEOUT 0ull
struct ChainFlow {
    unsigned* wait_flag; unsigned wait_val;
    unsigned* done_flag;
    int write_through;
    unsigned long long* trace;
    unsigned* diag;
};
int launch_chain(double* A, int64_t ld, int t0, int nk, double* invd, double* logdet, unsigned long long* info, long long info_base,
                 double* Wk, int64_t ldw, unsigned* flags, unsigned* err, hipStream_t s, const ChainFlow* flow = nullptr);

#define FLOW_MAXQ 48
#define FLOW_NCAS 1
#define FLOW_TRACE_W 6
#define FLOW_POST_W 96
#define FLOW_KEY_STEP 1024
#define FLOW_NOSIG 0xffffffffu
struct FlowTask {
    uint16_t ar, ac, br, bc, cr, cc;
    uint8_t abuf, bbuf, cbuf, var;
    uint16_t kt, ndep;
    uint32_t dep[4];
    uint16_t need[4];
    uint32_t sig[2];
    uint32_t key;
    uint32_t pad[2];
};
static_assert(sizeof(FlowTask) == 64, "FlowTask layout");
enum { FLOW_DIAG_DEEP = 0, FLOW_DIAG_HEAD_STALE = 1, FLOW_DIAG_DEP_STALE = 2, FLOW_DIAG_WAIT_DEEP = 3, FLOW_DIAG_WAIT_STALE = 4, FLOW_DIAG_LAST = 5, FLOW_DIAG_WORDS = 8 };
struct FlowPlan {
    int nb = 0, ob = 0, nouter = 0, nq = 0, rhs_nt = 0;
    bool replay = false;
    std::vector<FlowTask> tasks;
    std::vector<FlowTask> folded;
    int qbase[FLOW_MAXQ] = {0}, qsize[FLOW_MAXQ] = {0};
// ... 29 lines not shown
```

mogptk_amd/csrc/mogp_model.h:

```cpp
#pragma once
#include "../../include/mogp_hip.h"
#include "mogp_internal.h"

#include <algorithm>
#include <cmath>
#include <cstring>
#include <string>
#include <map>
#include <vector>

namespace mogp {

inline int dev_fill_zero(void* p, size_t bytes) {
    HIP_TRY(hipMemset(p, 0, bytes));
    HIP_TRY(hipStreamSynchronize(nullptr));
    return 0;
}

inline hipError_t dev_upload(void* dst, const void* src, size_t bytes) {
    hipError_t e = hipMemcpy(dst, src, bytes, hipMemcpyHostToDevice);
    return e != hipSuccess ? e : hipStreamSynchronize(nullptr);
}

template <typename T>
struct DevBuf {
    T* p = nullptr;
    size_t n = 0;
    bool borrowed = false;
    int ensure(size_t count) {
        if (count <= n) return 0;
        if (borrowed) { set_error("DevBuf: a borrowed range cannot grow"); return -1; }
        if (p) { hipError_t e = hipFree(p); (void)e; p = nullptr; n = 0; }
        HIP_TRY(hipMalloc(reinterpret_cast<void**>(&p), count * sizeof(T)));
        n = count;
        return 0;
    }
    void release() { if (p && !borrowed) { hipError_t e = hipFree(p); (void)e; } p = nullptr; n = 0; borrowed = false; }
};

struct RowBacked {
    static constexpr size_t GRAN = (size_t)2 << 20;
    char* base = nullptr;
    size_t bytes = 0, gran = GRAN;
    int device = 0;
    std::vector<hipMemGenericAllocationHandle_t> handle;
    std::vector<char> have;
    size_t nbacked = 0;
    int reserve(size_t nbytes, int dev) {
        release();
        bytes = (nbytes + gran - 1) / gran * gran;
        void* q = nullptr;
        HIP_TRY(hipMemAddressReserve(&q, bytes, gran, nullptr, 0));
        base = static_cast<char*>(q); device = dev;
        have.assign(bytes / gran, 0);
        handle.resize(bytes / gran);
        return 0;
    }
    int back(size_t off, size_t len) {
        if (len == 0) return 0;
        if (!base || off + len > bytes) { set_error("RowBacked::back: outside the reserved range"); return -1; }
        const size_t g_lo = off / gran, g_hi = (off + len - 1) / gran;
        hipMemAllocationProp prop{};
        prop.type = hipMemAllocationTypePinned; prop.location.type = hipMemLocationTypeDevice; prop.location.id = device;
        hipMemAccessDesc acc{};
        acc.location.type = hipMemLocationTypeDevice; acc.location.id = device; acc.flags = hipMemAccessFlagsProtReadWrite;
        for (size_t g = g_lo; g <= g_hi;) {
            if (have[g]) { ++g; continue; }
            size_t e = g;
            for (; e <= g_hi && !have[e]; ++e) {
                HIP_TRY(hipMemCreate(&handle[e], gran, &prop, 0));
                hipError_t me = hipMemMap(base + e * gran, gran, 0, handle[e], 0);
                if (me == hipSuccess) me = hipMemSetAccess(base + e * gran, gran, &acc, 1);
                if (me != hipSuccess) { hipError_t x = hipMemUnmap(base + e * gran, gran); x = hipMemRelease(handle[e]); (void)x; HIP_TRY(me); }
                have[e] = 1; ++nbacked;
            }
            { int z__ = dev_fill_zero(base + g * gran, (e - g) * gran); if (z__) return z__; }
            g = e;
        }
        return 0;
    }
    size_t backed_bytes() const { return nbacked * gran; }
    void release() {
        for (size_t g = 0; g < have.size(); ++g)
            if (have[g]) {
                hipError_t e = hipMemUnmap(base + g * gran, gran); (void)e;
                e = hipMemRelease(handle[g]); (void)e;
            }
        have.clear(); handle.clear(); nbacked = 0;
        if (base) { hipError_t e = hipMemAddressFree(base, bytes); (void)e; }
        base = nullptr; bytes = 0;
    }
};

struct PhaseWs {
    DevBuf<double> ws;
    DevBuf<int> offr, offc;
    std::vector<int> hr, hc;
    int prepare(const std::vector<int>& r, const std::vector<int>& c, int C, int T, int64_t ldr, int64_t ldc, hipStream_t s, PhaseRef& out) {
        int rc;
        if ((rc = ws.ensure(phase_ws_doubles(C, T, ldr, ldc)))) return rc;
        if (hr != r) {
            if ((rc = offr.ensure(r.size()))) return rc;
            hr = r;
            HIP_TRY(hipMemcpyAsync(offr.p, hr.data(), hr.size() * sizeof(int), hipMemcpyHostToDevice, s));
        }
        if (hc != c) {
            if ((rc = offc.ensure(c.size()))) return rc;
            hc = c;
            HIP_TRY(hipMemcpyAsync(offc.p, hc.data(), hc.size() * sizeof(int), hipMemcpyHostToDevice, s));
        }
        out.offr = offr.p; out.offc = offc.p; out.ws = ws.p;
        return 0;
    }
    void release() { ws.release(); offr.release(); offc.release(); hr.clear(); hc.clear(); }
};

struct SortedX {
    int64_t M = 0, Mpad = 0;
    std::vector<int64_t> perm;
    std::vector<int> off;
    std::vector<double> xs;
    bool identity = true;
};


int fail(int code, const std::string& msg);
static inline int64_t round_up(int64_t v, int64_t m) { return (v + m - 1) / m * m; }
int sort_inputs(const double* X, int64_t M, int D, int C, int64_t pad_to, SortedX& o);
void build_sym_tiles(const std::vector<int>& off, int C, std::vector<GTile>& tiles, std::vector<int>& pair_start);
void build_rect_tiles(const std::vector<int>& offr, const std::vector<int>& offc, int C, std::vector<GTile>& tiles,
                      std::vector<int>* pair_start = nullptr);

}

using namespace mogp;

enum { MOGP_COMM_NONE = 0, MOGP_COMM_RCCL = 1, MOGP_COMM_EXTERNAL = 2 };
struct mogp_comm {
    int kind = MOGP_COMM_NONE, rank = 0, n = 1;
    void* nccl = nullptr;
    mogp_allgather_cb allgather = nullptr;
    mogp_allreduce_cb allreduce = nullptr;
    void* user = nullptr;
};

struct mogp_ctx {
    int device = 0;
    mogp_comm comm;
    std::string name;
    hipStream_t st = nullptr, st2 = nullptr, st3 = nullptr, st4 = nullptr, st5 = nullptr, st_priv = nullptr, st2u = nullptr;
    bool streams_ready = false;
    bool chain_ok = true;
    struct SkWs { DevBuf<double> ws; DevBuf<unsigned> flags; unsigned epoch = 0; };
    std::map<hipStream_t, SkWs> sk;
    int ncu = 0, ncu_reserved = 0;
};

struct TrtriLevel {
    std::vector<GemmTask> h1, h2;
    DevBuf<GemmTask> d1, d2;
    double flops1 = 0, flops2 = 0;
};

#define MOGP_CHAIN_BOUND_TILES 160
#define MOGP_NPANEL 4
struct Spd {
    int64_t Npad = 0;
    int nb = 0;
    bool keep_L = false;
    bool refine_panels = false;
    DevBuf<double> pscr;
    DevBuf<double> A, B, invd, logdet;
    RowBacked Arows;
    bool owned_rows = false;
    DevBuf<double> Wm;
    std::vector<TrtriLevel> levels;
    std::vector<hipEvent_t> sync_ev;
    std::vector<hipEvent_t> row_ev;
    bool want_row_ev = false;
    std::vector<hipEvent_t> inv_ev;
    hipEvent_t fused_last_inv = nullptr, fused_last_wt = nullptr;
    DevBuf<double> Wd;
    DevBuf<double> Pb[MOGP_NPANEL];
    DevBuf<unsigned> chain_flags;
    DevBuf<double> Lm, Wt;
    FlowPlan flow;
    DevBuf<FlowTask> flow_tasks;
    DevBuf<int> flow_qmeta;
    FlowPlan flow_replay;
    DevBuf<FlowTask> flow_tasks_replay;
    DevBuf<int> flow_qmeta_replay;
    FlowPlan flow_rhs;
    DevBuf<FlowTask> flow_tasks_rhs;
    DevBuf<int> flow_qmeta_rhs;
    const FlowPlan* flow_cur = nullptr;
    DevBuf<unsigned> flow_flags;
    DevBuf<char> flow_args;
    std::vector<char> flow_args_h;
    DevBuf<unsigned char> flow_done;
    DevBuf<unsigned> flow_post;
    DevBuf<unsigned> flow_diag;
    DevBuf<unsigned long long> flow_trace;
    hipEvent_t tail_ready = nullptr;
    bool flow_used = false;
    bool want_vec = false, vec_done = false;
    const double* vec_y = nullptr; double* vec_z = nullptr; double* vec_zz = nullptr; double* vec_part = nullptr;
    void release() {
        for (auto& lv : levels) { lv.d1.release(); lv.d2.release(); }
        for (auto e : sync_ev) { hipError_t r = hipEventDestroy(e); (void)r; }
        for (auto e : row_ev) { hipError_t r = hipEventDestroy(e); (void)r; }
        row_ev.clear();
        for (auto e : inv_ev) { hipError_t r = hipEventDestroy(e); (void)r; }
        inv_ev.clear(); Wm.release(); Wd.release(); chain_flags.release(); for (auto& b : Pb) b.release();
        Lm.release(); Wt.release(); flow_tasks.release(); flow_qmeta.release(); flow_flags.release(); flow_args.release(); flow_args_h.clear(); flow_diag.release(); flow_post.release(); flow_done.release(); flow_trace.release(); flow = FlowPlan();
        flow_tasks_rhs.release(); flow_qmeta_rhs.release(); flow_rhs = FlowPlan(); flow_cur = nullptr;
        flow_tasks_replay.release(); flow_qmeta_replay.release(); flow_replay = FlowPlan();
        levels.clear(); sync_ev.clear();
        A.release(); B.release(); invd.release(); logdet.release(); pscr.release();
        Arows.release(); owned_rows = false;
    }
};

struct StripTiles {
    std::vector<mogp::GSeg> segs;
    std::vector<mogp::GTile> rest;
    mogp::DevBuf<mogp::GSeg> d_segs;
    mogp::DevBuf<mogp::GTile> d_rest;
    int build(const std::vector<mogp::GTile>& tiles);
    void attach(mogp::GramArgs& ga) const { ga.segs = d_segs.p; ga.nsegs = (int)segs.size(); ga.rest = d_rest.p; ga.nrest = (int)rest.size(); }
    void release() { d_segs.release(); d_rest.release(); }
};

struct TitsiasWork {
    int64_t Mpad = 0;
    Spd a, q;
    DevBuf<double> zx, B, v, GB, Qs, E, R, T1, GA, Hm;
    DevBuf<double> vec, scratch, gz, partial_uu, partial_uf, mom_uu, mom_uf, zero_noise;
    DevBuf<GTile> tiles_uu, tiles_uf;
    DevBuf<int> ps_uu, ps_uf;
    StripTiles strip_uf;
    std::vector<int> tile_key;
    size_t n_tuu = 0, n_tuf = 0;
    DevBuf<double> Kus, Aus, Bus;
    DevBuf<double> zero_col;
    DevBuf<double> kslices;
    DevBuf<double> red;
    const double* Wq = nullptr;
    SortedX pred_ss;
    bool pred_valid = false;
    hipEvent_t side_ev[2] = {nullptr, nullptr};
    hipEvent_t prod_ev[2] = {nullptr, nullptr};
    DevBuf<int> blk_z, blk_x;
    std::vector<int> hblk_z, hblk_x;
    DevBuf<double> gzp;
    SortedX sv_sz; bool sv_dense = false, sv_valid = false;
    DevBuf<double> kd_point;
    DevBuf<double> nvec;
    PhaseWs ph_zz, ph_zx, ph_zs;
    void release() {
        ph_zz.release(); ph_zx.release(); ph_zs.release();
        a.release(); q.release();
        zx.release(); B.release(); v.release(); GB.release(); Qs.release(); E.release(); R.release(); T1.release(); GA.release(); Hm.release();
        vec.release(); scratch.release(); gz.release(); partial_uu.release(); partial_uf.release(); mom_uu.release(); mom_uf.release();
        zero_noise.release(); tiles_uu.release(); tiles_uf.release(); ps_uu.release(); ps_uf.release(); strip_uf.release(); tile_key.clear();
        Kus.release(); Aus.release(); Bus.release(); zero_col.release(); kslices.release(); nvec.release(); kd_point.release(); red.release();
        blk_z.release(); blk_x.release(); gzp.release(); hblk_z.clear(); hblk_x.clear();
        for (auto& e : side_ev) if (e) { hipError_t r = hipEventDestroy(e); (void)r; e = nullptr; }
        for (auto& e : prod_ev) if (e) { hipError_t r = hipEventDestroy(e); (void)r; e = nullptr; }
    }
};

struct OaWork {
    mogp::DevBuf<double> K, Sc, Y, vec;
    bool valid = false;
    void release() { K.release(); Sc.release(); Y.release(); vec.release(); valid = false; }
};

struct FlowRhs { double* T; double* X; int nt; hipEvent_t ready; };
struct mogp_model {
    mogp_ctx* ctx = nullptr;
    int64_t N = 0, Npad = 0;
    int nb = 0, D = 0, C = 0, T = 0;
    int Wt = 0;
    std::vector<double> point_diag;
    SortedX sx;
    std::vector<GTile> tiles;
    std::vector<int> pair_start;
    std::vector<double> table;
    bool radial = false;
    mogp::DevBuf<int> d_kind;
    std::vector<int> hkind;
    mogp::DevBuf<double> d_shape;
    std::vector<double> hshape;
    bool point_kinds = false;
    hipStream_t st = nullptr;
    hipStream_t st2 = nullptr;
    hipStream_t st2u = nullptr;
    hipStream_t st3 = nullptr;
    hipStream_t st4 = nullptr;
    hipStream_t st_priv = nullptr;
    Spd k;
    Spd ws, ws_tail;
    DevBuf<double> swU[2], swUr[2];
    DevBuf<double> swXr[2];
    std::vector<hipEvent_t> sw_ev;
    int sh_rank = 0, sh_n = 1;
    bool sh_owned = false;
    int backed_rank = -1, backed_n = 0;
    std::vector<GTile> tiles_own;
    std::vector<int> pair_start_own;
    DevBuf<GTile> d_tiles_own;
    bool factor_only = false;
    hipEvent_t pred_ev[2] = {nullptr, nullptr};
    StripTiles strip, strip_own;
    std::vector<GTile> tiles_head, tiles_tail;
    DevBuf<GTile> d_tiles_head, d_tiles_tail;
    StripTiles strip_head, strip_tail;
    hipEvent_t gram_ev = nullptr, gram_tail_ev = nullptr;
    DevBuf<int> d_pair_start_own;
    int own_rank = -1, own_n = 0;
    DevBuf<double> sh_send, sh_recv;
    DevBuf<double> sh_send1, sh_recv1;
    DevBuf<double> sh_fact;
    bool sh_factor_once = false;
    bool sh_split = false;
    std::vector<hipEvent_t> sh_ev;
    std::vector<hipEvent_t> sh_prof;
    double sh_ms[6] = {0, 0, 0, 0, 0, 0};
    int sh_prof_blocks = 0;
    double sh_jabs = 0.0;
    bool sh_dvar = false;

    std::vector<double> hy;
    DevBuf<double> d_symv;
    DevBuf<double> d_x, d_y, d_table, d_noise, d_dvar, d_z, d_alpha, d_zz, d_partial, d_moments, d_diagG;
    DevBuf<GTile> d_tiles;
    std::vector<GemmTask> kinv_acc_tasks, kinv_lauum_tasks;
    std::vector<int> kinv_prefix;
    DevBuf<GemmTask> d_kinv_acc, d_kinv_lauum;
    std::vector<double> blk_cen, blk_half;
    bool kinv_sparse = false;
    double kinv_fraction = 1.0;
    DevBuf<int> d_pair_start, d_chan_off, d_flag;
    DevBuf<double> d_pivots;
    bool accurate = false, accurate_ran = false;
    DevBuf<double> acc_rhs;
    double pivot_min = 0.0, pivot_max = 0.0;
    DevBuf<unsigned long long> d_info;

    DevBuf<double> d_xs, d_Ksf, d_Vt, d_mu, d_var, d_kdiag, d_Kss;
    DevBuf<GTile> d_ptiles;
    DevBuf<GemmTask> d_pred_tasks;
    PhaseWs ph_xx, ph_sx, ph_ss;

    double* h_pin = nullptr;
    size_t h_pin_n = 0;

    bool profiling = false;
    std::vector<hipEvent_t> ev;
    std::vector<hipEvent_t> gemm_ev;
    size_t gemm_ev_used = 0;
    double ms[MOGP_ST_COUNT] = {0};
    int64_t gemm_launches = 0;
    double gemm_flops = 0.0;
    bool have_W = false, have_Kinv = false, kinv_in_A = false, w_in_Wm = false;
    bool flow_ran = false;
    const FlowRhs* rhs_job = nullptr;
    bool replay_flow = false;
    bool no_flow = false;
    long long n_fact = 0, flow_retry_at = 0;
    int flow_backoff = 64, flow_timeouts = 0;
    double flow_enqueue_us = 0.0, flow_enqueue_us_max = 0.0;
    bool no_chain = false;
    TitsiasWork* tw = nullptr;
    OaWork oa;

    bool mean_on = false, mean_g_valid = false, mean_g_pending = false;
    std::vector<double> mean_coef, mean_g, hy0;
    DevBuf<double> d_y0, d_mean_coef, d_mean_part, d_mean_g;
    double* h_mean_pin = nullptr;
    hipEvent_t mean_ev = nullptr;
    const double* mean_w = nullptr;
    double mean_w_scale = 0.0;
};


namespace mogp {
int use_device(mogp_ctx* c);
int gemm_call(mogp_model* m, const GemmArgs& g, double flops, hipStream_t st = nullptr);
int mark(mogp_model* m, int idx);
double table_diag(const mogp_model* m, int c);
double table_diag_points(const mogp_model* m, const SortedX& pts);
int mean_apply(mogp_model* m);
int mean_grad_enqueue(mogp_model* m, const double* w, double scale);
void mean_grad_collect(mogp_model* m);
void mean_release(mogp_model* m);
int spd_alloc(Spd& w, int64_t Npad, int owned_rows_device = -1);
int spd_make_whole(Spd& w);
inline GemmArgs make_gemm(const double* A, int64_t lda, int akm, const double* B, int64_t ldb, int bkm, double* C, int64_t ldc,
                          double alpha, int mode, int mt, int nt, int64_t K) {
    GemmArgs g{};
    g.A = A; g.lda = lda; g.a_kmajor = akm; g.B = B; g.ldb = ldb; g.b_kmajor = bkm; g.C = C; g.ldc = ldc;
    g.alpha = alpha; g.beta = 0.0; g.mode = mode; g.mt = mt; g.nt = nt; g.K = (int)K;
    return g;
}
int side_fork(mogp_model* m, TitsiasWork& t, hipStream_t* side);
int side_join(mogp_model* m, TitsiasWork& t, hipStream_t side);
int gz_prepare(mogp_model* m, TitsiasWork& t, const std::vector<int>& offz, int D);
void gz_attach(const TitsiasWork& t, MomentArgs& ma, bool zx);
int spd_check_info(mogp_model* m, const char* which, int64_t* info);
int spd_info_verdict(mogp_model* m, const char* which, unsigned long long hinfo, int64_t* info);
int sparse_timeout_check(mogp_model* m);
bool chain_enabled(const mogp_model* m);
int chain_fallback(mogp_model* m);
int spd_invert(mogp_model* m, Spd& w, const char* which, int64_t* info, const double** W, bool defer_check = false);
int mm_lower_splitk(mogp_model* m, TitsiasWork& t, const double* A, const double* B, double* out, int mt, int64_t Mpad, int64_t ldk, int64_t K,
                    double alpha = 1.0);
int launch_scale_cols(const double* in, double* out, int64_t ld, int64_t rows, int64_t n, const double* s, hipStream_t st);
int sparse_workspace(mogp_model* m, TitsiasWork& t, int64_t Mpad);
int sparse_tiles(mogp_model* m, TitsiasWork& t, const SortedX& sz, bool want_uf);
int sparse_kuu(mogp_model* m, int64_t M, const double* Z, double jitter, bool want_uf, SortedX& sz, double* jit, const char* need_grouped = nullptr);
int sparse_kuf(mogp_model* m, TitsiasWork& t, const SortedX& sz, hipStream_t stream, bool use_strips, double* out2);
int refined_apply(mogp_model* m, TitsiasWork& t, const double* P, const double* Q, const double* rhs, double* out);
int allreduce_vec_scalars(mogp_model* m, TitsiasWork& t, double* vec, int64_t n, double* hs, int k);
int adjoint_GA(mogp_model* m, TitsiasWork& t, double scale, hipStream_t stream);
int solve_with_rider(mogp_model* m, TitsiasWork& t, double* panel, const double* r, double* beta);
struct MomentSpec { const double* G; int64_t ldg; const double* ru; const double* rw; double rcoef; bool dz; };
int sparse_moments(mogp_model* m, TitsiasWork& t, const SortedX& sz, const MomentSpec* uf, const MomentSpec& uu, bool sharded, hipStream_t side);
int sparse_predict_panels(mogp_model* m, TitsiasWork& t, const SortedX& sz, int64_t S, const double* Xs, SortedX& ss);
int sparse_point_stats(mogp_model* m, TitsiasWork& t, const SortedX& pts, const double* a, const double* b, const double* mu_panel,
                       const double* mu_vec, double mu_div, const double* kdiag, double* mu, double* var);
int sparse_predict_finish(mogp_model* m, TitsiasWork& t, const SortedX& ss, const double* mu_panel, const double* mu_vec, double mu_div,
                          const double* kss_diag, double* mu, double* var);
#define MOGP_RETRY_NO_CHAIN 0x7e7e
extern int g_outer;
int begin_call(mogp_model* m, int64_t* info, bool one_gpu);
int exact_begin(mogp_model* m, const double* noise_var, const double* data_var, double jitter, GramArgs& ga, double& jabs);
int report_not_pd(unsigned long long hinfo, int64_t* info);
struct TestSide { SortedX ss; int64_t Spad = 0; int ntiles = 0; };
int test_side(mogp_model* m, int64_t S, const double* Xs, const double* kss_diag, int64_t extra_rows, hipStream_t st, TestSide& ts, GramArgs& ga);
inline void scatter_by_perm(const SortedX& ss, const double* sorted, double* out) { for (int64_t pos = 0; pos < ss.M; ++pos) out[ss.perm[pos]] = sorted[pos]; }
int moment_pass_device(mogp_model* m, const double* kinv, double ksign);
int moment_pass(mogp_model* m, const double* kinv, double ksign, double* moments, double* diagG);
void collect_timing(mogp_model* m, int last_mark);
int eval_sweep(mogp_model* m, const double* noise_var, const double* data_var, double jitter, double* lml, double* jitter_abs, int64_t* info);
void one_gpu_call(mogp_model* m);
int ensure_system(mogp_model* m);
int spd_potrf(mogp_model* m, Spd& w, long long info_base = 0);
int spd_potri_fused(mogp_model* m, Spd& w);
bool flow_enabled(const mogp_model* m, const Spd& w);
int launch_flow_alpha_sum(const Spd& w, double* alpha, hipStream_t st);
int spd_potri_flow(mogp_model* m, Spd& w, const FlowRhs* rhs = nullptr);
void flow_debug_dump(mogp_model* m);
int spd_potri_fused_finish(mogp_model* m, Spd& w);
int spd_trtri(mogp_model* m, Spd& w);
int spd_lauum(mogp_model* m, Spd& w);
int spd_sweep(mogp_model* m, Spd& w);
int sweep_prepare(mogp_model* m, Spd& w);
int sweep_nblocks(const Spd& w);
int sweep_block(mogp_model* m, Spd& w, int kb, hipEvent_t* prof = nullptr, hipEvent_t panel_ready = nullptr, hipEvent_t* stall = nullptr);
int sweep_finish(mogp_model* m, Spd& w);
int trsm_lower(mogp_model* m, const double* L, int64_t ldl, int nb, double* B, int64_t ldb, int64_t ncols, bool trans, hipStream_t st = nullptr, bool tri = false,
               const hipEvent_t* row_ready = nullptr);
int launch_transpose(double* dst, const double* src, int64_t ld, int64_t n, hipStream_t s);
int launch_sym_lower_avg(double* A, int64_t ld, int64_t n, double scale, hipStream_t s);
int comm_allgather(mogp_ctx* ctx, const double* send, double* recv, int64_t count, hipStream_t st);
int comm_allreduce(mogp_ctx* ctx, double* buf, int64_t count, hipStream_t st);
int shard_pack(mogp_model* m, Spd& w, int kb, double** send, double** recv, int64_t* count);
int shard_unpack(mogp_model* m, Spd& w, int kb);
int shard_pack_part(mogp_model* m, Spd& w, int kb, int part, DevBuf<double>& sendb, DevBuf<double>& recvb, int64_t* count, hipStream_t st);
int shard_unpack_part(mogp_model* m, Spd& w, int kb, int part, DevBuf<double>& recvb, hipStream_t st);
int shard_factor_bcast(mogp_model* m, Spd& w, Spd& s, int k0, int nk, bool mine, hipStream_t st);
}
```

mogptk_amd/csrc/potri.hip:

```cpp
#include "mogp_model.h"

#include <algorithm>
#include <chrono>
#include <cstdio>
#include <cstdlib>

using namespace mogp;

namespace mogp {
int launch_potrf_trtri_tile(double* A, int64_t ld, int t, double* invd, double* logdet, unsigned long long* info, hipStream_t s,
                            long long info_base = 0, int store_L = 0);
}

#define RC(x) do { int r__ = (x); if (r__) return r__; } while (0)
#define FZ_OB 4
#define FZ_KD (FZ_OB * MOGP_TILE)

namespace {

enum { EV_BLK = 0, EV_DIAG = 1, EV_PANEL = 2, EV_BULK = 3, EV_INV = 4, EV_REST = 5, EV_WROW = 6, EV_ACC = 7, EV_PER_BLOCK = 8 };

int intra_block_chain(mogp_model* m, Spd& w, double* Wk, int k0, int k1, hipStream_t q, int kb) {
    const int64_t ld = w.Npad;
    if (chain_enabled(m)) {
// ... 22 lines not shown
}

int panel_rows(mogp_model* m, Spd& w, double* P, const double* Wk, int k0, int nk, int r0, int nr, bool small, hipStream_t q) {
    const int64_t ld = w.Npad;
    GemmArgs g{};
    g.A = w.A.p + (int64_t)r0 * MOGP_TILE * ld + (int64_t)k0 * MOGP_TILE; g.lda = ld; g.a_kmajor = 0;
    g.B = Wk; g.ldb = FZ_KD; g.b_kmajor = 0;
    g.C = P + (int64_t)r0 * MOGP_TILE * FZ_KD; g.ldc = FZ_KD; g.alpha = 1.0; g.beta = 0.0;
    g.mode = GM_KHI_J; g.small = small ? 1 : 0; g.mt = small ? 2 * nr : nr; g.nt = nk; g.K = nk * MOGP_TILE;
    return gemm_call(m, g, gemm_flops(g, nullptr), q);
}

int inverse_step(mogp_model* m, Spd& w, const double* Wkk, int k0, int k1, const double* Lp, hipStream_t q, hipStream_t qacc, hipEvent_t w_row,
                 hipEvent_t w_final) {
    const int64_t ld = w.Npad;
    const int nk = k1 - k0, rem = w.nb - k1;
    const int64_t Kd = (int64_t)nk * MOGP_TILE, c0 = (int64_t)k0 * MOGP_TILE;
    double* Wrow = w.Wm.p + c0 * ld;
    double* Brow = w.B.p + c0 * ld;
    if (k0 > 0) {
        GemmArgs g{};
        g.A = Wkk; g.lda = FZ_KD; g.a_kmajor = 0; g.B = Wrow; g.ldb = ld; g.b_kmajor = 1;
        g.C = Brow; g.ldc = ld; g.alpha = 1.0; g.beta = 0.0;
        g.mode = GM_KHI_I; g.small = 1; g.mt = 2 * nk; g.nt = k0; g.K = (int)Kd;
        RC(gemm_call(m, g, gemm_flops(g, nullptr), q));
        RC(launch_copy2d(Wrow, ld, Brow, ld, Kd, c0, 1.0, q));
    }
    RC(launch_copy2d(Wrow + c0, ld, Wkk, FZ_KD, Kd, Kd, 1.0, q));
    if (w_final) HIP_TRY(hipEventRecord(w_final, q));
    HIP_TRY(hipEventRecord(w_row, q));
    if (rem > 0) {
        double* Wt = w.Wm.p + (int64_t)k1 * MOGP_TILE * ld;
        GemmArgs g{};
        g.A = Lp; g.lda = FZ_KD; g.a_kmajor = 0; g.B = Wkk; g.ldb = FZ_KD; g.b_kmajor = 1;
        g.C = Wt + c0; g.ldc = ld; g.alpha = -1.0; g.beta = 0.0;
        g.mode = GM_KLO_J; g.mt = rem; g.nt = nk; g.K = (int)Kd;
        RC(gemm_call(m, g, gemm_flops(g, nullptr), q));
        if (k0 > 0) {
            GemmArgs u{};
            u.A = Lp; u.lda = FZ_KD; u.a_kmajor = 0; u.B = Wrow; u.ldb = ld; u.b_kmajor = 1;
            u.C = Wt; u.ldc = ld; u.alpha = -1.0; u.beta = 1.0;
            u.mode = GM_RECT; u.mt = rem; u.nt = k0; u.K = (int)Kd;
            RC(gemm_call(m, u, gemm_flops(u, nullptr), q));
        }
    }
    HIP_TRY(hipStreamWaitEvent(qacc, w_row, 0));
    GemmArgs g{};
    g.A = Wrow; g.lda = ld; g.a_kmajor = 1; g.B = Wrow; g.ldb = ld; g.b_kmajor = 1;
    g.C = w.B.p; g.ldc = ld; g.alpha = 1.0; g.beta = 1.0;
    g.mode = GM_LOWER; g.mt = g.nt = k1; g.K = (int)Kd;
    g.beta0_from = k0 + 1;
    if (m->kinv_sparse && &w == &m->k && Kd == 4 * MOGP_TILE && k1 < (int)m->kinv_prefix.size()) {
        g.mode = GM_TASKS; g.tasks = m->d_kinv_acc.p; g.ntasks = m->kinv_prefix[k1]; g.task_chunked = 1; g.mt = g.nt = 0;
        return gemm_call(m, g, 2.0 * MOGP_TILE * MOGP_TILE * (double)Kd * g.ntasks, qacc);
    }
    return gemm_call(m, g, gemm_flops(g, nullptr), qacc);
}

}

namespace mogp {

int spd_potri_fused(mogp_model* m, Spd& w) {
    w.flow_used = false;
    if (flow_enabled(m, w)) return spd_potri_flow(m, w);
    const int nb = w.nb;
    const int64_t ld = w.Npad;
    const int nouter = (nb + FZ_OB - 1) / FZ_OB;
    const auto t_host0 = std::chrono::steady_clock::now();
    hipStream_t crit = m->st, priv = m->st_priv ? m->st_priv : m->st, bulk = m->st2, inv = m->st3;
    static const bool split_acc = !(std::getenv("MOGP_ACC_STREAM") && std::atoi(std::getenv("MOGP_ACC_STREAM")) == 0);
    hipStream_t acc = (m->st4 && split_acc) ? m->st4 : m->st3;

    if (w.Wm.n < (size_t)ld * ld) {
        RC(w.Wm.ensure((size_t)ld * ld));
        HIP_TRY(hipMemsetAsync(w.Wm.p, 0, (size_t)ld * ld * sizeof(double), crit));
    }
    for (auto& b : w.Pb) RC(b.ensure((size_t)ld * FZ_KD));
    if (w.Wd.n < (size_t)nouter * FZ_KD * FZ_KD) {
        RC(w.Wd.ensure((size_t)nouter * FZ_KD * FZ_KD));
        HIP_TRY(hipMemsetAsync(w.Wd.p, 0, (size_t)nouter * FZ_KD * FZ_KD * sizeof(double), crit));
    }
    RC(w.chain_flags.ensure((size_t)(nouter + 1) * MOGP_CHAIN_FLAGS));
    HIP_TRY(hipMemsetAsync(w.chain_flags.p, 0, (size_t)(nouter + 1) * MOGP_CHAIN_FLAGS * sizeof(unsigned), crit));
    auto Wk = [&](int kb) { return w.Wd.p + (int64_t)kb * FZ_KD * FZ_KD; };
    while ((int)w.inv_ev.size() < EV_PER_BLOCK * nouter + 2) {
        hipEvent_t e;
        HIP_TRY(hipEventCreateWithFlags(&e, hipEventDisableTiming));
        w.inv_ev.push_back(e);
    }
    auto ev = [&](int kb, int which) { return w.inv_ev[EV_PER_BLOCK * kb + which]; };
    hipEvent_t start = w.inv_ev[EV_PER_BLOCK * nouter], w_ready = w.inv_ev[EV_PER_BLOCK * nouter + 1];
    HIP_TRY(hipEventRecord(start, crit));

    auto geom = [&](int kb, int& k0, int& k1, int& nk, int& rem, int& na, int& k2) {
        k0 = kb * FZ_OB; k1 = std::min(k0 + FZ_OB, nb); nk = k1 - k0; rem = nb - k1; na = std::min(FZ_OB, rem); k2 = k1 + na;
    };
    auto chain = [&](int kb) -> int {
        int k0, k1, nk, rem, na, k2; geom(kb, k0, k1, nk, rem, na, k2);
        RC(intra_block_chain(m, w, Wk(kb), k0, k1, priv, kb));
        HIP_TRY(hipEventRecord(ev(kb, EV_BLK), priv));
        return 0;
    };
    auto next_diag = [&](int kb) -> int {
        int k0, k1, nk, rem, na, k2; geom(kb, k0, k1, nk, rem, na, k2);
        if (rem <= 0) return 0;
        double* P = w.Pb[kb % MOGP_NPANEL].p;
        if (kb >= MOGP_NPANEL) HIP_TRY(hipStreamWaitEvent(priv, ev(kb - MOGP_NPANEL, EV_INV), 0));
        if (kb >= 1) HIP_TRY(hipStreamWaitEvent(priv, ev(kb - 1, EV_BULK), 0));
        if (kb >= 1) HIP_TRY(hipStreamWaitEvent(priv, ev(kb - 1, EV_PANEL), 0));
        RC(panel_rows(m, w, P, Wk(kb), k0, nk, k1, na, true, priv));
        const double* Pn = P + (int64_t)k1 * MOGP_TILE * FZ_KD;
        GemmArgs u{};
        u.A = Pn; u.lda = FZ_KD; u.a_kmajor = 0; u.B = Pn; u.ldb = FZ_KD; u.b_kmajor = 0;
        u.C = w.A.p + (int64_t)k1 * MOGP_TILE * (ld + 1); u.ldc = ld; u.alpha = -1.0; u.beta = 1.0;
        u.mode = GM_RECT_LOWER; u.small = 2; u.mt = 2 * na; u.nt = 2 * na; u.K = nk * MOGP_TILE;
        RC(gemm_call(m, u, gemm_flops(u, nullptr), priv));
        HIP_TRY(hipEventRecord(ev(kb, EV_DIAG), priv));
        return 0;
    };
    HIP_TRY(hipStreamWaitEvent(priv, start, 0));
    RC(chain(0));
    RC(next_diag(0));
    for (int kb = 0; kb < nouter; ++kb) {
        int k0, k1, nk, rem, na, k2; geom(kb, k0, k1, nk, rem, na, k2);
        const int Kd = nk * MOGP_TILE;
        double* P = w.Pb[kb % MOGP_NPANEL].p;
        const double* Pn = P + (int64_t)k1 * MOGP_TILE * FZ_KD;
        const double* Pr = P + (int64_t)k2 * MOGP_TILE * FZ_KD;
        const int nr = rem - na, n1 = std::min(FZ_OB, std::max(nr, 0));
        if (kb + 1 < nouter) RC(chain(kb + 1));
        if (rem > 0) {
            HIP_TRY(hipStreamWaitEvent(crit, ev(kb, EV_DIAG), 0));
            if (nr > 0) RC(panel_rows(m, w, P, Wk(kb), k0, nk, k2, nr, false, crit));
            HIP_TRY(hipEventRecord(ev(kb, EV_REST), crit));
            if (nr > 0) {
                GemmArgs u{};
                u.A = Pr; u.lda = FZ_KD; u.a_kmajor = 0; u.B = Pn; u.ldb = FZ_KD; u.b_kmajor = 0;
                u.C = w.A.p + (int64_t)k2 * MOGP_TILE * ld + (int64_t)k1 * MOGP_TILE; u.ldc = ld; u.alpha = -1.0; u.beta = 1.0;
                u.mode = GM_RECT; u.mt = nr; u.nt = na; u.K = Kd;
                RC(gemm_call(m, u, gemm_flops(u, nullptr), crit));
            }
            HIP_TRY(hipEventRecord(ev(kb, EV_PANEL), crit));
        }
        if (nr > 0) {
            HIP_TRY(hipStreamWaitEvent(bulk, ev(kb, EV_REST), 0));
            GemmArgs u{};
            u.A = Pr; u.lda = FZ_KD; u.a_kmajor = 0; u.B = Pr; u.ldb = FZ_KD; u.b_kmajor = 0;
            u.C = w.A.p + (int64_t)k2 * MOGP_TILE * (ld + 1); u.ldc = ld; u.alpha = -1.0; u.beta = 1.0;
            u.mode = GM_RECT_LOWER; u.mt = nr; u.nt = n1; u.K = Kd;
            RC(gemm_call(m, u, gemm_flops(u, nullptr), bulk));
        }
        HIP_TRY(hipEventRecord(ev(kb, EV_BULK), bulk));
        if (kb + 1 < nouter) RC(next_diag(kb + 1));
        if (nr > n1) {
            const double* Pq = Pr + (int64_t)n1 * MOGP_TILE * FZ_KD;
            GemmArgs v{};
            v.A = Pq; v.lda = FZ_KD; v.a_kmajor = 0; v.B = Pq; v.ldb = FZ_KD; v.b_kmajor = 0;
            v.C = w.A.p + (int64_t)(k2 + n1) * MOGP_TILE * (ld + 1); v.ldc = ld; v.alpha = -1.0; v.beta = 1.0;
            v.mode = GM_LOWER; v.mt = v.nt = nr - n1; v.K = Kd;
            RC(gemm_call(m, v, gemm_flops(v, nullptr), bulk));
        }
        HIP_TRY(hipStreamWaitEvent(inv, ev(kb, EV_BLK), 0));
        if (rem > 0) HIP_TRY(hipStreamWaitEvent(inv, ev(kb, EV_REST), 0));
        RC(inverse_step(m, w, Wk(kb), k0, k1, P + (int64_t)k1 * MOGP_TILE * FZ_KD, inv, acc, ev(kb, EV_WROW), kb == nouter - 1 ? w_ready : nullptr));
        HIP_TRY(hipEventRecord(ev(kb, EV_INV), inv));
// ... 24 lines not shown
```

mogptk_amd/csrc/sweep.hip:

```cpp
#include "mogp_model.h"

#include <cstdlib>
#include <limits>

using namespace mogp;

#define RC(x) do { int r__ = (x); if (r__) return r__; } while (0)
#define SW_OB 4

static GemmArgs upd(const double* A, int64_t lda, int akm, const double* B, int64_t ldb, int bkm, double* C, int64_t ldc,
                    int mode, int mt, int nt, int64_t K, int small = 0) {
    GemmArgs g{};
    g.A = A; g.lda = lda; g.a_kmajor = akm; g.B = B; g.ldb = ldb; g.b_kmajor = bkm; g.C = C; g.ldc = ldc;
    g.alpha = -1.0; g.beta = 1.0; g.mode = mode; g.mt = mt; g.nt = nt; g.K = (int)K; g.small = small;
    return g;
}

namespace mogp {

int sweep_prepare(mogp_model* m, Spd& w) {
    const int nb = w.nb;
    const int64_t ld = w.Npad;
    const int nouter = (nb + SW_OB - 1) / SW_OB;
    RC(spd_alloc(m->ws, (int64_t)std::min(SW_OB, nb) * MOGP_TILE));
    if (nb % SW_OB && nb > SW_OB) RC(spd_alloc(m->ws_tail, (int64_t)(nb % SW_OB) * MOGP_TILE));
    for (int b = 0; b < 2; ++b) {
        RC(m->swU[b].ensure((size_t)ld * SW_OB * MOGP_TILE));
        RC(m->swUr[b].ensure((size_t)ld * SW_OB * MOGP_TILE));
        if (m->sh_owned) RC(m->swXr[b].ensure((size_t)ld * SW_OB * MOGP_TILE));
    }
    while ((int)m->sw_ev.size() < 2 * nouter) {
        hipEvent_t e;
        HIP_TRY(hipEventCreateWithFlags(&e, hipEventDisableTiming));
        m->sw_ev.push_back(e);
    }
    return 0;
}

int sweep_nblocks(const Spd& w) { return (w.nb + SW_OB - 1) / SW_OB; }

int sweep_block(mogp_model* m, Spd& w, int kb, hipEvent_t* prof, hipEvent_t panel_ready, hipEvent_t* stall) {
    const int nb = w.nb;
    const int64_t ld = w.Npad;
    const int rm = m->sh_n > 1 ? m->sh_n : 0, rr = m->sh_rank;
    const bool ow = m->sh_owned;
    auto owned = [&](int i) { return rm == 0 || i % rm == rr; };
    static const int force_masked = std::getenv("MOGP_SWEEP_MASKED") ? std::atoi(std::getenv("MOGP_SWEEP_MASKED")) : 0;
    hipStream_t q1 = m->st, q2 = (rm == 0 && !force_masked && w.nb > MOGP_CHAIN_BOUND_TILES && m->st2u) ? m->st2u : m->st2;
    double* A = w.A.p;
    const int k0 = kb * SW_OB, k1 = std::min(k0 + SW_OB, nb), nk = k1 - k0;
    const int64_t Kd = (int64_t)nk * MOGP_TILE;
    const int below = nb - k1;
    Spd& s = (nk == m->ws.nb) ? m->ws : m->ws_tail;
    double* Akk = A + (int64_t)k0 * MOGP_TILE * (ld + 1);
    double* Acol = A + (int64_t)k1 * MOGP_TILE * ld + (int64_t)k0 * MOGP_TILE;
    double* Arow = A + (int64_t)k0 * MOGP_TILE * ld;
    const bool chain = chain_enabled(m) && q2 == m->st2 && m->st_priv && m->ctx->comm.kind != MOGP_COMM_EXTERNAL;
    const bool once = rm > 0 && m->sh_factor_once;
    const bool mine = !once || (k0 % rm) == rr;
    if (chain && kb == 0) {
        const int nouter = (nb + SW_OB - 1) / SW_OB;
        RC(w.chain_flags.ensure((size_t)(nouter + 1) * MOGP_CHAIN_FLAGS));
        HIP_TRY(hipMemsetAsync(w.chain_flags.p, 0, (size_t)(nouter + 1) * MOGP_CHAIN_FLAGS * sizeof(unsigned), q1));
    }
    if (!mine) {
        HIP_TRY(hipMemsetAsync(s.B.p, 0, (size_t)Kd * Kd * sizeof(double), q1));
    } else if (chain) {
        const int nouter = (nb + SW_OB - 1) / SW_OB;
        if (s.Wm.n < (size_t)Kd * Kd) {
            RC(s.Wm.ensure((size_t)Kd * Kd));
            HIP_TRY(hipMemsetAsync(s.Wm.p, 0, (size_t)Kd * Kd * sizeof(double), q1));
        }
        double* cA = ow ? s.A.p - (int64_t)k0 * MOGP_TILE * (Kd + 1) : A;
        RC(launch_chain(cA, ow ? Kd : ld, k0, nk, w.invd.p, w.logdet.p, m->d_info.p, 0, s.Wm.p, Kd, w.chain_flags.p + (size_t)kb * MOGP_CHAIN_FLAGS,
                        w.chain_flags.p + (size_t)nouter * MOGP_CHAIN_FLAGS, q1));
        GemmArgs g{};
        g.A = s.Wm.p; g.lda = Kd; g.a_kmajor = 1; g.B = s.Wm.p; g.ldb = Kd; g.b_kmajor = 1;
        g.C = s.B.p; g.ldc = Kd; g.alpha = 1.0; g.beta = 0.0;
        g.mode = GM_LAUUM; g.mt = g.nt = nk; g.K = (int)Kd;
        RC(gemm_call(m, g, gemm_flops(g, nullptr), q1));
    } else {
        if (!ow) RC(launch_copy2d(s.A.p, Kd, Akk, ld, Kd, Kd, 1.0, q1));
        RC(spd_potrf(m, s, (long long)k0 * MOGP_TILE));
        HIP_TRY(hipMemcpyAsync(w.logdet.p + k0, s.logdet.p, nk * sizeof(double), hipMemcpyDeviceToDevice, q1));
        RC(spd_trtri(m, s));
        RC(spd_lauum(m, s));
    }
    if (mine) RC(launch_symmetrize(s.B.p, Kd, Kd, q1));
    if (once) RC(shard_factor_bcast(m, w, s, k0, nk, mine, q1));
    const double* P = s.B.p;
    if (stall) HIP_TRY(hipEventRecord(stall[0], q1));
    if (panel_ready) HIP_TRY(hipStreamWaitEvent(q1, panel_ready, 0));
    if (stall) HIP_TRY(hipEventRecord(stall[1], q1));
    double* Uc = m->swU[kb & 1].p;
    double* Ur = m->swUr[kb & 1].p;
    double* Xrow = ow ? m->swXr[kb & 1].p : Arow;
    if (!ow) {
        RC(launch_copy2d(Uc, Kd, Acol, ld, (int64_t)below * MOGP_TILE, Kd, 1.0, q1));
        RC(launch_copy2d(Ur, ld, Arow, ld, Kd, (int64_t)k0 * MOGP_TILE, 1.0, q1));
    }
    if (below > 0) {
        GemmArgs g = upd(Uc, Kd, 0, P, Kd, 0, Acol, ld, GM_RECT, 2 * below, nk, Kd, 1);
        g.alpha = 1.0; g.beta = 0.0;
        g.row_mod = rm; g.row_rem = rr; g.row_off = k1; g.row_shift = 1;
        RC(gemm_call(m, g, gemm_flops(g, nullptr), q1));
    }
    if (k0 > 0) {
        GemmArgs g = upd(P, Kd, 0, Ur, ld, 1, Xrow, ld, GM_RECT, nk, k0, Kd);
        g.alpha = 1.0; g.beta = 0.0;
        RC(gemm_call(m, g, gemm_flops(g, nullptr), q1));
    }
    if (!ow) RC(launch_copy2d(Akk, ld, P, Kd, Kd, Kd, -1.0, q1));
    else
        for (int i = k0; i < k1; ++i) {
            if (!owned(i)) continue;
            const int64_t r = (int64_t)(i - k0) * MOGP_TILE;
            if (k0 > 0) RC(launch_copy2d(A + (int64_t)i * MOGP_TILE * ld, ld, Xrow + r * ld, ld, MOGP_TILE, (int64_t)k0 * MOGP_TILE, 1.0, q1));
            RC(launch_copy2d(A + (int64_t)i * MOGP_TILE * ld + (int64_t)k0 * MOGP_TILE, ld, P + r * Kd, Kd, MOGP_TILE, Kd, -1.0, q1));
        }
    HIP_TRY(hipEventRecord(m->sw_ev[2 * kb], q1));
    if (prof) HIP_TRY(hipEventRecord(prof[0], q1));
    const int nk2 = std::min(SW_OB, below);
    if (kb > 0) HIP_TRY(hipStreamWaitEvent(q1, m->sw_ev[2 * (kb - 1) + 1], 0));
    if (nk2 > 0) {
        GemmArgs a1 = upd(Acol, ld, 0, Uc, Kd, 0, A + (int64_t)k1 * MOGP_TILE * (ld + 1), ld, GM_RECT_LOWER, below, nk2, Kd);
        a1.row_mod = rm; a1.row_rem = rr; a1.row_off = k1;
        RC(gemm_call(m, a1, gemm_flops(a1, nullptr), q1));
        if (k0 > 0) {
            GemmArgs b1 = upd(Acol, ld, 0, Ur, ld, 1, A + (int64_t)k1 * MOGP_TILE * ld, ld, GM_RECT, nk2, k0, Kd);
            b1.row_mod = rm; b1.row_rem = rr; b1.row_off = k1;
            RC(gemm_call(m, b1, gemm_flops(b1, nullptr), q1));
        }
    }
    if (prof) HIP_TRY(hipEventRecord(prof[1], q1));
    HIP_TRY(hipStreamWaitEvent(q2, m->sw_ev[2 * kb], 0));
    if (prof) HIP_TRY(hipEventRecord(prof[2], q2));
    const int rest = below - nk2;
    if (rest > 0) {
        const int64_t r0 = (int64_t)(k1 + nk2) * MOGP_TILE;
        const double* Xr2 = A + r0 * ld + (int64_t)k0 * MOGP_TILE;
        GemmArgs a2 = upd(Xr2, ld, 0, Uc + (int64_t)nk2 * MOGP_TILE * Kd, Kd, 0, A + r0 * (ld + 1), ld, GM_LOWER, rest, rest, Kd);
        a2.row_mod = rm; a2.row_rem = rr; a2.row_off = k1 + nk2;
        RC(gemm_call(m, a2, gemm_flops(a2, nullptr), q2));
        if (k0 > 0) {
            GemmArgs b2 = upd(Xr2, ld, 0, Ur, ld, 1, A + r0 * ld, ld, GM_RECT, rest, k0, Kd);
// ... 188 lines not shown
```

Measured before the change: 94.59.

## Trim per-evaluation launches, memsets and host syncs around the dataflow factorization

Several changes aim to cut per-evaluation host overhead and small launches. The dataflow flag and zz buffers are now zeroed after the results copy, off the critical path, so the next call can skip its memsets. Noise and info uploads are merged into one copy, and moments plus diagG come back in a single D2H transfer from a contiguous buffer. The host waits on an event instead of the whole stream. Moment reduction and diagG are fused into one kernel, block centres are cached across calls, and phase/centre kernels handle both sides in one launch. The cost is extra bookkeeping for clean-state validity, which could go stale if another path touches those flags.

Result: no change. 94.73 (median of 3 runs) (+0.2%).

```diff
diff --git a/mogptk_amd/csrc/exact.hip b/mogptk_amd/csrc/exact.hip
--- a/mogptk_amd/csrc/exact.hip
+++ b/mogptk_amd/csrc/exact.hip
@@ -4,13 +4,13 @@
 
 using namespace mogp;
 
-static int wait_stream(hipStream_t st) {
+static int wait_event(hipEvent_t ev) {
     static const bool spin = !(std::getenv("MOGP_SPIN_WAIT") && std::atoi(std::getenv("MOGP_SPIN_WAIT")) == 0);
-    if (!spin) { HIP_TRY(hipStreamSynchronize(st)); return 0; }
+    if (!spin) { HIP_TRY(hipEventSynchronize(ev)); return 0; }
     for (;;) {
-        const hipError_t e = hipStreamQuery(st);
+        const hipError_t e = hipEventQuery(ev);
         if (e == hipSuccess) return 0;
-        if (e != hipErrorNotReady) return hip_fail(e, "hipStreamQuery", __FILE__, __LINE__);
+        if (e != hipErrorNotReady) return hip_fail(e, "hipEventQuery", __FILE__, __LINE__);
     }
 }
 
@@ -103,9 +103,9 @@
     return 0;
 }
 struct PinLayout {
-    size_t nzz, logdet = 0, zz, info, moments, diagG, pivots, total;
+    size_t nzz, logdet = 0, zz, info, moments, diagG, pivots, flow_err, total;
     PinLayout(int nb, int64_t Npad, int C, int T, int Wt) : nzz((size_t)((Npad + 3) / 4)) {
-        zz = (size_t)nb; info = zz + nzz; moments = info + 1; diagG = moments + (size_t)(C * (C + 1) / 2) * T * Wt; pivots = diagG + C; total = pivots + 2;
+        zz = (size_t)nb; info = zz + nzz; moments = info + 1; diagG = moments + (size_t)(C * (C + 1) / 2) * T * Wt; pivots = diagG + C; flow_err = pivots + 2; total = flow_err + 1;
     }
     explicit PinLayout(const mogp_model* m) : PinLayout(m->nb, m->Npad, m->C, m->T, m->Wt) {}
 };
@@ -144,14 +144,21 @@
         HIP_TRY(hipMemcpyAsync(m->d_dvar.p, dv.data(), Npad * sizeof(double), hipMemcpyHostToDevice, m->st));
     }
     jabs = jitter * dsum / (double)N;
-    HIP_TRY(hipMemcpyAsync(m->d_noise.p, noise_var, C * sizeof(double), hipMemcpyHostToDevice, m->st));
     static const unsigned long long big = std::numeric_limits<unsigned long long>::max();
-    HIP_TRY(hipMemcpyAsync(m->d_info.p, &big, sizeof(big), hipMemcpyHostToDevice, m->st));
+    m->h_step.resize((size_t)C + 1);
+    std::memcpy(m->h_step.data(), noise_var, C * sizeof(double));
+    std::memcpy(m->h_step.data() + C, &big, sizeof(big));
+    HIP_TRY(hipMemcpyAsync(m->d_step.p, m->h_step.data(), ((size_t)C + 1) * sizeof(double), hipMemcpyHostToDevice, m->st));
     int rc;
     if ((rc = mark(m, 0))) return rc;
     ga = GramArgs{};
     ga.tiles = m->d_tiles.p; ga.xr = m->d_x.p; ga.xc = m->d_x.p; ga.ldxr = ga.ldxc = Npad; ga.nrows = ga.ncols = N;
     if ((rc = m->ph_xx.prepare(m->sx.off, m->sx.off, C, m->T, Npad, Npad, m->st, ga.ph))) return rc;
+    if (!m->ph_xx.centres_held(m->d_x.p, m->d_x.p, m->T, m->D)) {
+        if ((rc = launch_block_centres(ga.ph, m->d_x.p, Npad, N, m->d_x.p, Npad, N, C, m->T, m->D, m->st))) return rc;
+        m->ph_xx.centres_mark(m->d_x.p, m->d_x.p, m->T, m->D);
+    }
+    ga.ph.centres_ready = 1;
     ga.table = m->d_table.p; ga.T = m->T; ga.D = m->D; ga.C = C; ga.W = m->Wt;
     ga.out = m->k.A.p; ga.ldo = Npad; ga.noise = m->d_noise.p; ga.dvar = data_var ? m->d_dvar.p : nullptr;
     ga.jitter_abs = jabs; ga.mirror = 0;
@@ -171,7 +178,8 @@
         if (!said_flow) {
             said_flow = true;
             unsigned code = 0;
-            if (m->k.flow_flags.p && m->k.flow_cur && m->k.flow_cur->base_err > 0) { hipError_t e = hipMemcpy(&code, m->k.flow_flags.p + m->k.flow_cur->base_err, sizeof(code), hipMemcpyDeviceToHost); (void)e; }
+            if (m->k.flow_err_snapped) code = m->k.flow_err_snap;
+            else if (m->k.flow_flags.p && m->k.flow_cur && m->k.flow_cur->base_err > 0) { hipError_t e = hipMemcpy(&code, m->k.flow_flags.p + m->k.flow_cur->base_err, sizeof(code), hipMemcpyDeviceToHost); (void)e; }
             fprintf(stderr, "mogp: the dataflow kernel timed out (wait 0x%x; GPU shared with another process?); using the stream schedule for the next %d evaluations (said once)\n", code, (int)(m->flow_retry_at - m->n_fact));
             fprintf(stderr, "mogp: the host enqueued that evaluation in %.0f us (longest so far %.0f us)\n", m->flow_enqueue_us, m->flow_enqueue_us_max);
         }
@@ -311,6 +319,7 @@
         if ((rc = launch_copy2d(m->acc_rhs.p, MOGP_TILE, m->d_y.p, 1, Npad, 1, 1.0, m->st))) return rc;
         if ((rc = trsm_lower(m, m->k.A.p, Npad, m->nb, m->acc_rhs.p, MOGP_TILE, MOGP_TILE, false))) return rc;
         if ((rc = launch_copy2d(m->d_z.p, 1, m->acc_rhs.p, MOGP_TILE, Npad, 1, 1.0, m->st))) return rc;
+        m->k.flow_clean = false;
         HIP_TRY(hipMemsetAsync(m->d_zz.p, 0, pl.nzz * sizeof(double), m->st));
         if ((rc = launch_gemv_rows(m->d_z.p, Npad, 1, Npad, m->d_z.p, m->d_zz.p, m->st))) return rc;
         if ((rc = trsm_lower(m, m->k.A.p, Npad, m->nb, m->acc_rhs.p, MOGP_TILE, MOGP_TILE, true))) return rc;
@@ -327,6 +336,7 @@
         if (fuse_inverse && m->k.flow_used && m->k.vec_done) {
             if ((rc = launch_flow_alpha_sum(m->k, m->d_alpha.p, m->st))) return rc;
         } else {
+            m->k.flow_clean = false;
             if ((rc = launch_trmv_lower(Wp, Npad, Npad, m->d_y.p, m->d_z.p, m->d_zz.p, m->st))) return rc;
             if ((rc = launch_trmv_lower_t(Wp, Npad, Npad, m->d_z.p, m->d_alpha.p, m->st))) return rc;
         }
@@ -390,8 +400,8 @@
     ma.phases_ready = 1;
     ma.ev0 = prof_event(m, 9); ma.ev1 = prof_event(m, 10);
     if ((rc = launch_moments(ma, m->st))) return rc;
-    if ((rc = launch_moment_reduce(m->d_partial.p, own ? m->d_pair_start_own.p : m->d_pair_start.p, P, T, W, D, m->d_moments.p, m->st))) return rc;
-    if ((rc = launch_diagG(kinv, Npad, m->d_alpha.p, m->d_chan_off.p, C, m->d_diagG.p, m->st, ksign, rm, m->sh_rank))) return rc;
+    if ((rc = launch_moment_tail(m->d_partial.p, own ? m->d_pair_start_own.p : m->d_pair_start.p, P, T, W, D, m->d_moments.p,
+                                 kinv, Npad, m->d_alpha.p, m->d_chan_off.p, C, m->d_diagG.p, m->st, ksign, rm, m->sh_rank))) return rc;
     if ((rc = mean_grad_enqueue(m, m->d_alpha.p, -1.0))) return rc;
     return mark(m, 6);
 }
@@ -476,9 +486,16 @@
     } else {
         if ((rc = moment_pass_device(m, kinv, ksign))) return rc;
         const PinLayout pl(m);
-        HIP_TRY(hipMemcpyAsync(m->h_pin + pl.moments, m->d_moments.p, (size_t)P * T * W * sizeof(double), hipMemcpyDeviceToHost, m->st));
-        HIP_TRY(hipMemcpyAsync(m->h_pin + pl.diagG, m->d_diagG.p, C * sizeof(double), hipMemcpyDeviceToHost, m->st));
-        if ((rc = wait_stream(m->st))) return rc;
+        if (m->d_diagG.p != m->d_moments.p + (size_t)P * T * W || pl.diagG != pl.moments + (size_t)P * T * W) return fail(MOGP_EINVAL, "mogp_exact_eval: the moment block is not contiguous");
+        HIP_TRY(hipMemcpyAsync(m->h_pin + pl.moments, m->d_moments.p, ((size_t)P * T * W + C) * sizeof(double), hipMemcpyDeviceToHost, m->st));
+        bool cleaned = false;
+        unsigned* err_pin = reinterpret_cast<unsigned*>(m->h_pin + pl.flow_err);
+        *err_pin = 0u;
+        if (!m->results_ev) HIP_TRY(hipEventCreateWithFlags(&m->results_ev, hipEventDisableTiming));
+        if ((rc = spd_flow_postclean(m, m->k, err_pin, m->results_ev, &cleaned))) return rc;
+        if (!cleaned) HIP_TRY(hipEventRecord(m->results_ev, m->st));
+        if ((rc = wait_event(m->results_ev))) return rc;
+        if (cleaned) { m->k.flow_err_snap = *err_pin; m->k.flow_err_snapped = true; }
         if ((rc = factorize_finish(m, ga, lml, info))) return retry_on_streams(m, rc, again);
         std::memcpy(moments, m->h_pin + pl.moments, (size_t)P * T * W * sizeof(double));
         std::memcpy(diagG, m->h_pin + pl.diagG, C * sizeof(double));
diff --git a/mogptk_amd/csrc/flow.hip b/mogptk_amd/csrc/flow.hip
--- a/mogptk_amd/csrc/flow.hip
+++ b/mogptk_amd/csrc/flow.hip
@@ -734,16 +734,24 @@
     w.flow_cur = &plan;
     const FlowPlan& p = plan;
     const int nouter = p.nouter;
-    if ((rc = w.chain_flags.ensure((size_t)(nouter + 1) * MOGP_CHAIN_FLAGS))) return rc;
-    HIP_TRY(hipMemsetAsync(w.chain_flags.p, 0, (size_t)(nouter + 1) * MOGP_CHAIN_FLAGS * sizeof(unsigned), crit));
-    HIP_TRY(hipMemsetAsync(w.flow_flags.p, 0, (size_t)p.nflags * sizeof(unsigned), crit));
+    const size_t nchain = (size_t)(nouter + 1) * MOGP_CHAIN_FLAGS, nzz = (size_t)((ld + 3) / 4);
+    if ((rc = w.chain_flags.ensure(nchain))) return rc;
+    const bool zero_zz = !rhs && w.want_vec && w.vec_zz;
+    const bool preclean = w.flow_clean && !replay && w.clean_chain >= nchain && w.clean_flow >= (size_t)p.nflags &&
+                          (!zero_zz || (w.clean_zz == w.vec_zz && w.clean_zz_n >= nzz));
+    w.flow_clean = false;
+    w.flow_err_snapped = false;
+    if (!preclean) {
+        HIP_TRY(hipMemsetAsync(w.chain_flags.p, 0, nchain * sizeof(unsigned), crit));
+        HIP_TRY(hipMemsetAsync(w.flow_flags.p, 0, (size_t)p.nflags * sizeof(unsigned), crit));
+    }
     if (replay) {
         std::vector<unsigned> preset((size_t)p.nflags, 0u);
         for (const FlowPlan::Chain& c : p.chain) preset[c.done_idx] = c.expect;
         HIP_TRY(hipMemcpyAsync(w.flow_flags.p, preset.data(), preset.size() * sizeof(unsigned), hipMemcpyHostToDevice, crit));
         HIP_TRY(hipStreamSynchronize(crit));
     }
-    if (!rhs && w.want_vec && w.vec_zz) HIP_TRY(hipMemsetAsync(w.vec_zz, 0, (size_t)((ld + 3) / 4) * sizeof(double), crit));
+    if (zero_zz && !preclean) HIP_TRY(hipMemsetAsync(w.vec_zz, 0, nzz * sizeof(double), crit));
     static const bool want_trace = std::getenv("MOGP_FLOW_TRACE") && std::atoi(std::getenv("MOGP_FLOW_TRACE")) != 0;
     if (want_trace) {
         if ((rc = w.flow_trace.ensure(FLOW_TRACE_W * p.tasks.size() + 4 * (size_t)nouter))) return rc;
@@ -804,11 +812,12 @@
     if (rhs && rhs->ready) HIP_TRY(hipStreamWaitEvent(bulk, rhs->ready, 0));
     const bool dbg_kernel = g.post != nullptr || g.trace != nullptr;
     static_assert(sizeof(FlowArgs) <= 512, "Spd::flow_args slots");
-    if ((rc = w.flow_args.ensure(1024))) return rc;
-    if (w.flow_args_h.size() != 2048) w.flow_args_h.assign(2048, (char)0xff);
+    constexpr size_t ARG_BYTES = 3 * 1024;
+    if ((rc = w.flow_args.ensure(ARG_BYTES))) return rc;
+    if (w.flow_args_h.size() != 2 * ARG_BYTES) w.flow_args_h.assign(2 * ARG_BYTES, (char)0xff);
     auto upload = [&](size_t slot, const FlowArgs& a, hipStream_t st) -> int {
         char* held = w.flow_args_h.data() + slot;
-        char* fresh_ = w.flow_args_h.data() + 1024 + slot;
+        char* fresh_ = w.flow_args_h.data() + ARG_BYTES + slot;
         std::memset(fresh_, 0, 512);
         std::memcpy(fresh_, &a, sizeof(a));
         if (std::memcmp(held, fresh_, 512) == 0) return 0;
@@ -817,8 +826,16 @@
         std::memcpy(held, fresh_, 512);
         return 0;
     };
-    if ((rc = upload(0, g, bulk))) return rc;
-    const FlowArgs* d_g = reinterpret_cast<const FlowArgs*>(w.flow_args.p);
+    const size_t slot0 = (rhs ? 1 : replay ? 2 : 0) * (size_t)1024, slot1 = slot0 + 512;
+    static const bool tail_on = !(std::getenv("MOGP_FLOW_TAIL") && std::atoi(std::getenv("MOGP_FLOW_TAIL")) == 0);
+    const bool tail = tail_on && m->ctx->ncu_reserved > 0 && !replay;
+    if ((rc = upload(slot0, g, bulk))) return rc;
+    if (tail) {
+        FlowArgs g2 = g;
+        g2.post_base = wg_per_cu * cus;
+        if ((rc = upload(slot1, g2, priv))) return rc;
+    }
+    const FlowArgs* d_g = reinterpret_cast<const FlowArgs*>(w.flow_args.p + slot0);
     FlowHot hot{};
     hot.bA = g.bA; hot.bL = g.bL; hot.bWt = g.bWt; hot.bWm = g.bWm; hot.bB = g.bB; hot.ld = g.ld; hot.tasks = g.tasks; hot.qmeta = g.qmeta; hot.flags = g.flags;
     hot.nq = g.nq; hot.ncas = g.ncas; hot.base_heads = g.base_heads; hot.base_err = g.base_err; hot.nap_max = g.nap_max; hot.nap_calm = g.nap_calm;
@@ -862,12 +879,9 @@
         if ((rc = launch_gemm(t2, priv))) return rc;
         m->gemm_flops += gemm_flops(t1, nullptr) + gemm_flops(t2, nullptr);
     }
-    static const bool tail_on = !(std::getenv("MOGP_FLOW_TAIL") && std::atoi(std::getenv("MOGP_FLOW_TAIL")) == 0);
-    if (tail_on && m->ctx->ncu_reserved > 0 && !replay) {
+    if (tail) {
         if (rhs && rhs->ready) HIP_TRY(hipStreamWaitEvent(priv, rhs->ready, 0));
-        g.post_base = wg_per_cu * cus;
-        if ((rc = upload(512, g, priv))) return rc;
-        const FlowArgs* d_g2 = reinterpret_cast<const FlowArgs*>(w.flow_args.p + 512);
+        const FlowArgs* d_g2 = reinterpret_cast<const FlowArgs*>(w.flow_args.p + slot1);
         if (dbg_kernel) hipLaunchKernelGGL(k_flow<true>, dim3(wg_per_cu * m->ctx->ncu_reserved), dim3(FL_NT), FL_LDS_BYTES, priv, d_g2, hot);
         else hipLaunchKernelGGL(k_flow<false>, dim3(wg_per_cu * m->ctx->ncu_reserved), dim3(FL_NT), FL_LDS_BYTES, priv, d_g2, hot);
         HIP_TRY(hipGetLastError());
@@ -877,11 +891,31 @@
     HIP_TRY(hipStreamWaitEvent(crit, e_chain, 0));
     w.fused_last_inv = nullptr; w.fused_last_wt = nullptr;
     w.flow_used = true;
+    w.flow_postclean_ok = !rhs && !replay && !want_trace && !std::getenv("MOGP_FLOW_DEBUG");
     m->flow_ran = true;
     m->flow_enqueue_us = std::chrono::duration<double, std::micro>(std::chrono::steady_clock::now() - host_t0).count();
     m->flow_enqueue_us_max = std::max(m->flow_enqueue_us_max, m->flow_enqueue_us);
     { const char* e = std::getenv("MOGP_FLOW_DEBUG");
       if (e && std::atoi(e) == 2 && &w == &m->k) { usleep(60000); fprintf(stderr, "mogp: dataflow state 60 ms after the evaluation was enqueued\n"); flow_debug_dump(m); } }
+    return 0;
+}
+
+int spd_flow_postclean(mogp_model* m, Spd& w, unsigned* err_out, hipEvent_t results_ready, bool* enqueued) {
+    if (enqueued) *enqueued = false;
+    if (!w.flow_used || !w.flow_postclean_ok || !w.flow_cur || !w.flow_flags.p || !w.chain_flags.p) return 0;
+    const FlowPlan& p = *w.flow_cur;
+    const size_t nchain = (size_t)(p.nouter + 1) * MOGP_CHAIN_FLAGS, nflags = (size_t)p.nflags, nzz = (size_t)((w.Npad + 3) / 4);
+    if (w.chain_flags.n < nchain || w.flow_flags.n < nflags) return 0;
+    hipStream_t crit = m->st;
+    if (err_out && p.base_err > 0) HIP_TRY(hipMemcpyAsync(err_out, w.flow_flags.p + p.base_err, sizeof(unsigned), hipMemcpyDeviceToHost, crit));
+    if (results_ready) HIP_TRY(hipEventRecord(results_ready, crit));
+    HIP_TRY(hipMemsetAsync(w.chain_flags.p, 0, nchain * sizeof(unsigned), crit));
+    HIP_TRY(hipMemsetAsync(w.flow_flags.p, 0, nflags * sizeof(unsigned), crit));
+    const bool zz = w.vec_done && w.vec_zz;
+    if (zz) HIP_TRY(hipMemsetAsync(w.vec_zz, 0, nzz * sizeof(double), crit));
+    w.clean_chain = nchain; w.clean_flow = nflags; w.clean_zz = zz ? w.vec_zz : nullptr; w.clean_zz_n = zz ? nzz : 0;
+    w.flow_clean = true;
+    if (enqueued) *enqueued = true;
     return 0;
 }
 
diff --git a/mogptk_amd/csrc/gram.hip b/mogptk_amd/csrc/gram.hip
--- a/mogptk_amd/csrc/gram.hip
+++ b/mogptk_amd/csrc/gram.hip
@@ -56,45 +56,49 @@
     return p;
 }
 
-struct PhaseArgs {
-    const double* x; int64_t ld; const int* off; const double* table; int T, D, C, W, role; double* cs; double* sn;
-};
+struct PhaseSide { const double* x; int64_t ld; const int* off; double* cs; double* sn; };
+struct PhaseArgs { PhaseSide side[2]; const double* table; int T, D, C, W; unsigned nbr; };
 __global__ __launch_bounds__(256) void k_phase_table(PhaseArgs a) {
-    const int64_t pt = (int64_t)blockIdx.x * 256 + threadIdx.x;
-    if (pt >= a.off[a.C]) return;
+    const int role = blockIdx.x >= a.nbr ? 1 : 0;
+    const PhaseSide& sd = a.side[role];
+    const int64_t pt = (int64_t)(blockIdx.x - (role ? a.nbr : 0u)) * 256 + threadIdx.x;
+    if (pt >= sd.off[a.C]) return;
     const int o = blockIdx.y, t = blockIdx.z, D = a.D, W = a.W;
     int c = 0;
-    while (pt >= a.off[c + 1]) ++c;
-    const int pair = a.role == 0 ? c * a.C + o : o * a.C + c;
+    while (pt >= sd.off[c + 1]) ++c;
+    const int pair = role == 0 ? c * a.C + o : o * a.C + c;
     const double* row = a.table + ((size_t)pair * a.T + t) * W;
-    double ph = a.role == 0 ? row[1] : 0.0;
+    double ph = role == 0 ? row[1] : 0.0;
     for (int d = 0; d < D; ++d) {
-        const double m = row[2 + D + d], xv = a.x[(size_t)d * a.ld + pt];
-        ph = a.role == 0 ? fma(m, xv + row[2 + 2 * D + d], ph) : fma(m, xv, ph);
+        const double m = row[2 + D + d], xv = sd.x[(size_t)d * sd.ld + pt];
+        ph = role == 0 ? fma(m, xv + row[2 + 2 * D + d], ph) : fma(m, xv, ph);
     }
     double sn, cs;
     sincospi(2.0 * frac_turn(ph), &sn, &cs);
-    const size_t idx = ((size_t)o * a.T + t) * a.ld + pt;
-    a.cs[idx] = cs;
-    a.sn[idx] = sn;
-}
-
-struct CentreArgs { const double* x; int64_t ld; const int* off; int C, D; double* cen; double* half; };
+    const size_t idx = ((size_t)o * a.T + t) * sd.ld + pt;
+    sd.cs[idx] = cs;
+    sd.sn[idx] = sn;
+}
+
+struct CentreSide { const double* x; int64_t ld; const int* off; double* cen; double* half; };
+struct CentreArgs { CentreSide side[2]; int C, D; unsigned nbr; };
 __global__ __launch_bounds__(64) void k_block_centres(CentreArgs a) {
-    int b = blockIdx.x, c = 0;
+    const int role = blockIdx.x >= a.nbr ? 1 : 0;
+    const CentreSide& sd = a.side[role];
+    int b = (int)(blockIdx.x - (role ? a.nbr : 0u)), c = 0;
     for (; c < a.C; ++c) {
-        const int nb = (a.off[c + 1] - a.off[c] + MOGP_GT - 1) / MOGP_GT;
+        const int nb = (sd.off[c + 1] - sd.off[c] + MOGP_GT - 1) / MOGP_GT;
         if (b < nb) break;
         b -= nb;
     }
     if (c >= a.C) return;
-    const int start = a.off[c] + b * MOGP_GT, n = min(MOGP_GT, a.off[c + 1] - start), lane = threadIdx.x;
+    const int start = sd.off[c] + b * MOGP_GT, n = min(MOGP_GT, sd.off[c + 1] - start), lane = threadIdx.x;
     for (int d = 0; d < a.D; ++d) {
-        const double v = a.x[(size_t)d * a.ld + start + (lane < n ? lane : 0)];
+        const double v = sd.x[(size_t)d * sd.ld + start + (lane < n ? lane : 0)];
         double lo = v, hi = v;
 #pragma unroll
         for (int off = 32; off > 0; off >>= 1) { lo = fmin(lo, __shfl_xor(lo, off, 64)); hi = fmax(hi, __shfl_xor(hi, off, 64)); }
-        if (lane == 0) { a.cen[(size_t)d * a.ld + start] = 0.5 * (lo + hi); a.half[(size_t)d * a.ld + start] = 0.5 * (hi - lo); }
+        if (lane == 0) { sd.cen[(size_t)d * sd.ld + start] = 0.5 * (lo + hi); sd.half[(size_t)d * sd.ld + start] = 0.5 * (hi - lo); }
     }
 }
 
@@ -113,24 +117,34 @@
     return v;
 }
 
+int launch_block_centres(const PhaseRef& ph, const double* xr, int64_t ldxr, int64_t nr, const double* xc, int64_t ldxc, int64_t nc, int C, int T, int D, hipStream_t s) {
+    if (!ph.ws || !ph.offr || !ph.offc) { set_error("Gram / moment launch without a phase workspace"); return -1; }
+    const PhaseView v = phase_view(ph.ws, C, T, D, ldxr, ldxc);
+    CentreArgs c;
+    c.C = C; c.D = D;
+    c.side[0] = CentreSide{xr, ldxr, ph.offr, const_cast<double*>(v.rcen), const_cast<double*>(v.rhalf)};
+    c.side[1] = CentreSide{xc, ldxc, ph.offc, const_cast<double*>(v.ccen), const_cast<double*>(v.chalf)};
+    const unsigned gr = nr > 0 ? (unsigned)((nr + MOGP_GT - 1) / MOGP_GT + C) : 0u, gc = nc > 0 ? (unsigned)((nc + MOGP_GT - 1) / MOGP_GT + C) : 0u;
+    c.nbr = gr;
+    if (gr + gc > 0) hipLaunchKernelGGL(k_block_centres, dim3(gr + gc), dim3(64), 0, s, c);
+    HIP_TRY(hipGetLastError());
+    return 0;
+}
+
 static int launch_phase_tables(const PhaseRef& ph, const double* xr, int64_t ldxr, int64_t nr, const double* xc, int64_t ldxc, int64_t nc,
                                const double* table, int T, int D, int C, int W, hipStream_t s) {
     if (!ph.ws || !ph.offr || !ph.offc) { set_error("Gram / moment launch without a phase workspace"); return -1; }
     const PhaseView v = phase_view(ph.ws, C, T, D, ldxr, ldxc);
     PhaseArgs a;
     a.table = table; a.T = T; a.D = D; a.C = C; a.W = W;
-    a.x = xr; a.ld = ldxr; a.off = ph.offr; a.role = 0; a.cs = const_cast<double*>(v.rcs); a.sn = const_cast<double*>(v.rsn);
-    if (nr > 0) hipLaunchKernelGGL(k_phase_table, dim3((unsigned)((nr + 255) / 256), C, T), dim3(256), 0, s, a);
-    a.x = xc; a.ld = ldxc; a.off = ph.offc; a.role = 1; a.cs = const_cast<double*>(v.ccs); a.sn = const_cast<double*>(v.csn);
-    if (nc > 0) hipLaunchKernelGGL(k_phase_table, dim3((unsigned)((nc + 255) / 256), C, T), dim3(256), 0, s, a);
-    CentreArgs c;
-    c.C = C; c.D = D;
-    c.x = xr; c.ld = ldxr; c.off = ph.offr; c.cen = const_cast<double*>(v.rcen); c.half = const_cast<double*>(v.rhalf);
-    if (nr > 0) hipLaunchKernelGGL(k_block_centres, dim3((unsigned)((nr + MOGP_GT - 1) / MOGP_GT + C)), dim3(64), 0, s, c);
-    c.x = xc; c.ld = ldxc; c.off = ph.offc; c.cen = const_cast<double*>(v.ccen); c.half = const_cast<double*>(v.chalf);
-    if (nc > 0) hipLaunchKernelGGL(k_block_centres, dim3((unsigned)((nc + MOGP_GT - 1) / MOGP_GT + C)), dim3(64), 0, s, c);
+    a.side[0] = PhaseSide{xr, ldxr, ph.offr, const_cast<double*>(v.rcs), const_cast<double*>(v.rsn)};
+    a.side[1] = PhaseSide{xc, ldxc, ph.offc, const_cast<double*>(v.ccs), const_cast<double*>(v.csn)};
+    const unsigned gr = nr > 0 ? (unsigned)((nr + 255) / 256) : 0u, gc = nc > 0 ? (unsigned)((nc + 255) / 256) : 0u;
+    a.nbr = gr;
+    if (gr + gc > 0) hipLaunchKernelGGL(k_phase_table, dim3(gr + gc, C, T), dim3(256), 0, s, a);
     HIP_TRY(hipGetLastError());
-    return 0;
+    if (ph.centres_ready) return 0;
+    return launch_block_centres(ph, xr, ldxr, nr, xc, ldxc, nc, C, T, D, s);
 }
 
 template <int DM>
@@ -1678,11 +1692,9 @@
     return env ? launch_moments_t<true, false, true>(a, s) : launch_moments_t<true, false, false>(a, s);
 }
 
-__global__ __launch_bounds__(256) void k_moment_reduce(const double* __restrict__ partial, const int* __restrict__ pair_start,
-                                                       int TW, int W, int D, int lower_pairs, double* __restrict__ out) {
-    const int p = blockIdx.x, tw = blockIdx.y;
+__device__ __forceinline__ void moment_reduce_block(double* red, int p, int tw, const double* __restrict__ partial, const int* __restrict__ pair_start,
+                                                    int TW, int W, int D, int lower_pairs, double* __restrict__ out) {
     const int b = pair_start[p], e = pair_start[p + 1];
-    __shared__ double red[256];
     double s = 0.0;
     for (int t = b + threadIdx.x; t < e; t += 256) s += partial[(size_t)t * TW + tw];
     red[threadIdx.x] = s;
@@ -1702,6 +1714,11 @@
         out[(size_t)p * TW + tw] = v;
     }
 }
+__global__ __launch_bounds__(256) void k_moment_reduce(const double* __restrict__ partial, const int* __restrict__ pair_start,
+                                                       int TW, int W, int D, int lower_pairs, double* __restrict__ out) {
+    __shared__ double red[256];
+    moment_reduce_block(red, blockIdx.x, blockIdx.y, partial, pair_start, TW, W, D, lower_pairs, out);
+}
 
 int launch_moment_reduce(const double* partial, const int* pair_start, int npairs, int T, int W, int D, double* out, hipStream_t s, int lower_pairs) {
     hipLaunchKernelGGL(k_moment_reduce, dim3(npairs, T * W), dim3(256), 0, s, partial, pair_start, T * W, W, D, lower_pairs, out);
@@ -1709,10 +1726,8 @@
     return 0;
 }
 
-__global__ void k_diagG(const double* __restrict__ kinv, int64_t ld, const double* __restrict__ alpha,
-                        const int* __restrict__ chan_off, double* __restrict__ out, double kinv_sign, int row_mod, int row_rem) {
-    const int c = blockIdx.x;
-    __shared__ double red[256];
+__device__ __forceinline__ void diagG_block(double* red, int c, const double* __restrict__ kinv, int64_t ld, const double* __restrict__ alpha,
+                                            const int* __restrict__ chan_off, double* __restrict__ out, double kinv_sign, int row_mod, int row_rem) {
     double s = 0.0;
     for (int64_t k = chan_off[c] + threadIdx.x; k < chan_off[c + 1]; k += 256)
         if (row_mod <= 1 || (int)((k / MOGP_TILE) % row_mod) == row_rem) s += 0.5 * (alpha[k] * alpha[k] - kinv_sign * kinv[k * ld + k]);
@@ -1724,6 +1739,30 @@
     }
     if (threadIdx.x == 0) out[c] = red[0];
 }
+__global__ __launch_bounds__(256) void k_diagG(const double* __restrict__ kinv, int64_t ld, const double* __restrict__ alpha,
+                                               const int* __restrict__ chan_off, double* __restrict__ out, double kinv_sign, int row_mod, int row_rem) {
+    __shared__ double red[256];
+    diagG_block(red, blockIdx.x, kinv, ld, alpha, chan_off, out, kinv_sign, row_mod, row_rem);
+}
+
+struct MomentTailArgs {
+    const double* partial; const int* pair_start; int npairs, TW, W, D; double* moments;
+    const double* kinv; int64_t ld; const double* alpha; const int* chan_off; double* diagG; double kinv_sign; int row_mod, row_rem;
+};
+__global__ __launch_bounds__(256) void k_moment_tail(MomentTailArgs a) {
+    __shared__ double red[256];
+    const int b = blockIdx.x, nred = a.npairs * a.TW;
+    if (b < nred) moment_reduce_block(red, b / a.TW, b % a.TW, a.partial, a.pair_start, a.TW, a.W, a.D, 1, a.moments);
+    else diagG_block(red, b - nred, a.kinv, a.ld, a.alpha, a.chan_off, a.diagG, a.kinv_sign, a.row_mod, a.row_rem);
+}
+int launch_moment_tail(const double* partial, const int* pair_start, int npairs, int T, int W, int D, double* moments,
+                       const double* kinv, int64_t ld, const double* alpha, const int* chan_off, int C, double* diagG, hipStream_t s,
+                       double kinv_sign, int row_mod, int row_rem) {
+    MomentTailArgs a{partial, pair_start, npairs, T * W, W, D, moments, kinv, ld, alpha, chan_off, diagG, kinv_sign, row_mod, row_rem};
+    hipLaunchKernelGGL(k_moment_tail, dim3((unsigned)(npairs * T * W + C)), dim3(256), 0, s, a);
+    HIP_TRY(hipGetLastError());
+    return 0;
+}
 
 int launch_diagG(const double* kinv, int64_t ld, const double* alpha, const int* chan_off, int C, double* out, hipStream_t s,
                  double kinv_sign, int row_mod, int row_rem) {
diff --git a/mogptk_amd/csrc/mogp_api.hip b/mogptk_amd/csrc/mogp_api.hip
--- a/mogptk_amd/csrc/mogp_api.hip
+++ b/mogptk_amd/csrc/mogp_api.hip
@@ -664,12 +664,13 @@
     m->st = ctx->st; m->st2 = ctx->st2; m->st2u = ctx->st2u; m->st3 = ctx->st3; m->st4 = ctx->st4; m->st_priv = ctx->st_priv;
     TRY_RC(m->d_x.ensure((size_t)D * Npad));
     TRY_RC(m->d_y.ensure(Npad));
-    TRY_RC(m->d_noise.ensure(C));
+    TRY_RC(m->d_step.ensure((size_t)C + 2));
+    m->d_noise.p = m->d_step.p; m->d_noise.n = C; m->d_noise.borrowed = true;
+    m->d_info.p = reinterpret_cast<unsigned long long*>(m->d_step.p + C); m->d_info.n = 2; m->d_info.borrowed = true;
+    static_assert(sizeof(unsigned long long) == sizeof(double), "d_step holds both");
     TRY_RC(m->d_z.ensure(Npad));
     TRY_RC(m->d_alpha.ensure((size_t)(1 + nchunks) * Npad));
     TRY_RC(m->d_zz.ensure((Npad + 3) / 4));
-    TRY_RC(m->d_diagG.ensure(C));
-    TRY_RC(m->d_info.ensure(2));
     TRY_RC(m->d_flag.ensure(1));
     TRY_RC(m->d_chan_off.ensure(C + 1));
     TRY_HIP(dev_upload(m->d_x.p, m->sx.xs.data(), (size_t)D * Npad * sizeof(double)));
@@ -698,11 +699,12 @@
     if (m->tw) { m->tw->release(); delete m->tw; m->tw = nullptr; }
     m->oa.release();
     m->d_x.release(); m->d_y.release(); m->d_table.release(); m->d_kind.release(); m->d_shape.release();
-    m->d_noise.release(); m->d_dvar.release(); m->d_z.release(); m->d_alpha.release(); m->d_zz.release();
+    m->d_noise.release(); m->d_step.release(); m->d_dvar.release(); m->d_z.release(); m->d_alpha.release(); m->d_zz.release();
     m->d_partial.release(); m->d_moments.release(); m->d_diagG.release(); m->d_tiles.release(); m->d_pair_start.release(); m->strip.release(); m->strip_own.release();
     m->d_tiles_head.release(); m->d_tiles_tail.release(); m->strip_head.release(); m->strip_tail.release();
     if (m->gram_ev) { hipError_t r = hipEventDestroy(m->gram_ev); (void)r; m->gram_ev = nullptr; }
     if (m->gram_tail_ev) { hipError_t r = hipEventDestroy(m->gram_tail_ev); (void)r; m->gram_tail_ev = nullptr; }
+    if (m->results_ev) { hipError_t r = hipEventDestroy(m->results_ev); (void)r; m->results_ev = nullptr; }
     m->d_chan_off.release(); m->d_flag.release(); m->d_info.release(); m->d_pivots.release(); m->acc_rhs.release();
     m->d_xs.release(); m->d_Ksf.release(); m->d_Vt.release(); m->d_mu.release(); m->d_var.release(); m->d_kdiag.release();
     m->d_Kss.release(); m->d_ptiles.release(); m->d_pred_tasks.release();
@@ -746,7 +748,12 @@
     if (m->tw) m->tw->pred_valid = false;
     m->table.assign(table, table + n);
     if ((rc = m->d_table.ensure(n))) return rc;
-    if ((rc = m->d_moments.ensure((size_t)(m->C * (m->C + 1) / 2) * T * W))) return rc;
+    {
+        const size_t nmom = (size_t)(m->C * (m->C + 1) / 2) * T * W;
+        if (m->d_moments.n < nmom + m->C) HIP_TRY(hipStreamSynchronize(m->st));
+        if ((rc = m->d_moments.ensure(nmom + m->C))) return rc;
+        m->d_diagG.p = m->d_moments.p + nmom; m->d_diagG.n = m->C; m->d_diagG.borrowed = true;
+    }
     HIP_TRY(hipMemcpyAsync(m->d_table.p, m->table.data(), n * sizeof(double), hipMemcpyHostToDevice, m->st));
     return MOGP_OK;
 }
diff --git a/mogptk_amd/csrc/mogp_internal.h b/mogptk_amd/csrc/mogp_internal.h
--- a/mogptk_amd/csrc/mogp_internal.h
+++ b/mogptk_amd/csrc/mogp_internal.h
@@ -68,6 +68,7 @@
     const int* offr = nullptr;
     const int* offc = nullptr;
     double* ws = nullptr;
+    int centres_ready = 0;
 };
 size_t phase_ws_doubles(int C, int T, int64_t ldr, int64_t ldc);
 
@@ -137,6 +138,7 @@
 };
 
 int launch_gram(const GramArgs& a, int ntiles, hipStream_t s);
+int launch_block_centres(const PhaseRef& ph, const double* xr, int64_t ldxr, int64_t nr, const double* xc, int64_t ldxc, int64_t nc, int C, int T, int D, hipStream_t s);
 void split_strip_tiles(const std::vector<GTile>& tiles, int maxrun, std::vector<GSeg>& segs, std::vector<GTile>& rest);
 int launch_moments(const MomentArgs& a, hipStream_t s);
 inline size_t gz_scratch_doubles(int nrb, int ncb, int D) { return (size_t)2 * nrb * ncb * D * MOGP_GT; }
@@ -145,6 +147,9 @@
                          int lower_pairs = 1);
 int launch_diagG(const double* kinv, int64_t ld, const double* alpha, const int* chan_off, int C, double* out, hipStream_t s,
                  double kinv_sign = 1.0, int row_mod = 0, int row_rem = 0);
+int launch_moment_tail(const double* partial, const int* pair_start, int npairs, int T, int W, int D, double* moments,
+                       const double* kinv, int64_t ld, const double* alpha, const int* chan_off, int C, double* diagG, hipStream_t s,
+                       double kinv_sign = 1.0, int row_mod = 0, int row_rem = 0);
 
 enum GemmMode { GM_RECT = 0,
                 GM_LOWER = 1,
diff --git a/mogptk_amd/csrc/mogp_model.h b/mogptk_amd/csrc/mogp_model.h
--- a/mogptk_amd/csrc/mogp_model.h
+++ b/mogptk_amd/csrc/mogp_model.h
@@ -99,6 +99,7 @@
     int prepare(const std::vector<int>& r, const std::vector<int>& c, int C, int T, int64_t ldr, int64_t ldc, hipStream_t s, PhaseRef& out) {
         int rc;
         if ((rc = ws.ensure(phase_ws_doubles(C, T, ldr, ldc)))) return rc;
+        if (T != cen_T) cen_ws = nullptr;
         if (hr != r) {
             if ((rc = offr.ensure(r.size()))) return rc;
             hr = r;
@@ -112,7 +113,14 @@
         out.offr = offr.p; out.offc = offc.p; out.ws = ws.p;
         return 0;
     }
-    void release() { ws.release(); offr.release(); offc.release(); hr.clear(); hc.clear(); }
+    const double *cen_ws = nullptr, *cen_xr = nullptr, *cen_xc = nullptr;
+    int cen_T = -1, cen_D = -1;
+    std::vector<int> cen_hr, cen_hc;
+    bool centres_held(const double* xr, const double* xc, int T, int D) const {
+        return cen_ws && cen_ws == ws.p && cen_xr == xr && cen_xc == xc && cen_T == T && cen_D == D && cen_hr == hr && cen_hc == hc;
+    }
+    void centres_mark(const double* xr, const double* xc, int T, int D) { cen_ws = ws.p; cen_xr = xr; cen_xc = xc; cen_T = T; cen_D = D; cen_hr = hr; cen_hc = hc; }
+    void release() { ws.release(); offr.release(); offc.release(); hr.clear(); hc.clear(); cen_ws = nullptr; cen_hr.clear(); cen_hc.clear(); }
 };
 
 struct SortedX {
@@ -203,6 +211,12 @@
     DevBuf<unsigned long long> flow_trace;
     hipEvent_t tail_ready = nullptr;
     bool flow_used = false;
+    bool flow_clean = false;
+    size_t clean_chain = 0, clean_flow = 0, clean_zz_n = 0;
+    const double* clean_zz = nullptr;
+    bool flow_postclean_ok = false;
+    bool flow_err_snapped = false;
+    unsigned flow_err_snap = 0;
     bool want_vec = false, vec_done = false;
     const double* vec_y = nullptr; double* vec_z = nullptr; double* vec_zz = nullptr; double* vec_part = nullptr;
     void release() {
@@ -218,6 +232,7 @@
         levels.clear(); sync_ev.clear();
         A.release(); B.release(); invd.release(); logdet.release(); pscr.release();
         Arows.release(); owned_rows = false;
+        flow_clean = flow_postclean_ok = flow_err_snapped = false; clean_chain = clean_flow = clean_zz_n = 0; clean_zz = nullptr;
     }
 };
 
@@ -317,6 +332,7 @@
     DevBuf<GTile> d_tiles_head, d_tiles_tail;
     StripTiles strip_head, strip_tail;
     hipEvent_t gram_ev = nullptr, gram_tail_ev = nullptr;
+    hipEvent_t results_ev = nullptr;
     DevBuf<int> d_pair_start_own;
     int own_rank = -1, own_n = 0;
     DevBuf<double> sh_send, sh_recv;
@@ -347,6 +363,8 @@
     DevBuf<double> acc_rhs;
     double pivot_min = 0.0, pivot_max = 0.0;
     DevBuf<unsigned long long> d_info;
+    DevBuf<double> d_step;
+    std::vector<double> h_step;
 
     DevBuf<double> d_xs, d_Ksf, d_Vt, d_mu, d_var, d_kdiag, d_Kss;
     DevBuf<GTile> d_ptiles;
@@ -451,6 +469,7 @@
 bool flow_enabled(const mogp_model* m, const Spd& w);
 int launch_flow_alpha_sum(const Spd& w, double* alpha, hipStream_t st);
 int spd_potri_flow(mogp_model* m, Spd& w, const FlowRhs* rhs = nullptr);
+int spd_flow_postclean(mogp_model* m, Spd& w, unsigned* err_out, hipEvent_t results_ready, bool* enqueued);
 void flow_debug_dump(mogp_model* m);
 int spd_potri_fused_finish(mogp_model* m, Spd& w);
 int spd_trtri(mogp_model* m, Spd& w);
diff --git a/mogptk_amd/csrc/potri.hip b/mogptk_amd/csrc/potri.hip
--- a/mogptk_amd/csrc/potri.hip
+++ b/mogptk_amd/csrc/potri.hip
@@ -128,6 +128,7 @@
         HIP_TRY(hipMemsetAsync(w.Wd.p, 0, (size_t)nouter * FZ_KD * FZ_KD * sizeof(double), crit));
     }
     RC(w.chain_flags.ensure((size_t)(nouter + 1) * MOGP_CHAIN_FLAGS));
+    w.flow_clean = false;
     HIP_TRY(hipMemsetAsync(w.chain_flags.p, 0, (size_t)(nouter + 1) * MOGP_CHAIN_FLAGS * sizeof(unsigned), crit));
     auto Wk = [&](int kb) { return w.Wd.p + (int64_t)kb * FZ_KD * FZ_KD; };
     while ((int)w.inv_ev.size() < EV_PER_BLOCK * nouter + 2) {
diff --git a/mogptk_amd/csrc/sweep.hip b/mogptk_amd/csrc/sweep.hip
--- a/mogptk_amd/csrc/sweep.hip
+++ b/mogptk_amd/csrc/sweep.hip
@@ -61,6 +61,7 @@
     if (chain && kb == 0) {
         const int nouter = (nb + SW_OB - 1) / SW_OB;
         RC(w.chain_flags.ensure((size_t)(nouter + 1) * MOGP_CHAIN_FLAGS));
+        w.flow_clean = false;
         HIP_TRY(hipMemsetAsync(w.chain_flags.p, 0, (size_t)(nouter + 1) * MOGP_CHAIN_FLAGS * sizeof(unsigned), q1));
     }
     if (!mine) {
```
